# burritojustice/reporter

Measured on AMD Instinct MI355X. Metric: GPS points matched/sec (whole node) at 1/2/4/8 MI355X; % segment-ID agreement vs meili, higher is better.
Workload: dtype f32

## Files before the change

### include/otmatch.h

```cpp
#ifndef OTMATCH_H
#define OTMATCH_H

#include <stddef.h>
#include <stdint.h>

#ifdef __cplusplus
extern "C" {
#endif

#define OTM_OK 0
#define OTM_EINVAL (-1)
#define OTM_EIO (-2)
#define OTM_EDEVICE (-3)
#define OTM_ECONFIG (-4)
#define OTM_EAGAIN (-5)
#define OTM_ENOMEM (-6)

typedef struct otm_engine otm_engine;


int otm_engine_create(const char* cfg_path, const int* devices, int ndev,
                      otm_engine** out);
typedef struct otm_meili_params {
  float sigma_z, beta, max_route_distance_factor, breakage_distance, interpolation_distance;
// ... 231 lines not shown
int otm_attributes_size(otm_engine* eng, int64_t* n_traces, int64_t* n_bytes);
int otm_fetch_attributes(otm_engine* eng, char* dst, int64_t cap, int64_t* body_off, int64_t* n_bytes);
int otm_attributes_device(otm_engine* eng, const char** dev, const int64_t** body_off, int64_t* n_traces,
                          int64_t* n_bytes);
int otm_debug_attr_fixed(double x, int decimals, char* out);

int otm_hist_bind(otm_engine* eng, void* dev_counts, int nbins, float bin_kph);
int otm_hist_bind_ex(otm_engine* eng, void* dev_counts, int nbins, float bin_kph,
                     void* dev_speed_sum);


int otm_flush_body_host(const uint32_t* counts, const uint64_t* speed_sum,
                        const uint64_t* segment_ids, int64_t n_segments,
                        int64_t rows, int nbins, float bin_kph, int rank, int world,
                        char** body, size_t* body_len, int64_t* n_records);
int otm_flush_body_device(otm_engine* eng, const void* dev_counts,
                          const void* dev_speed_sum, int64_t rows, int nbins,
                          float bin_kph, int rank, int world, void* stream,
                          char** body, size_t* body_len, int64_t* n_records);

int otm_window_begin(otm_engine* eng, int nbins, float bin_kph);
int otm_window_flush(otm_engine* eng, char** body, size_t* body_len, int64_t* n_records);
int otm_window_end(otm_engine* eng);

typedef struct otm_pairs_cfg {
  int32_t bucket_s;
  int32_t privacy;
  int64_t origin;
  int64_t max_keys;
} otm_pairs_cfg;
typedef struct otm_pairs_stats {
  int64_t reports;
  int64_t keys;
  int64_t records;
  int64_t suppressed_keys;
  int64_t suppressed_reports;
  int64_t out_of_range;
  int64_t dropped;
} otm_pairs_stats;
int otm_pairs_cfg_check(const otm_pairs_cfg* cfg);
int otm_pairs_begin(otm_engine* eng, const otm_pairs_cfg* cfg);
int otm_pairs_add_reports(otm_engine* eng, int64_t n, const otm_report_rec* recs);
int otm_pairs_flush(otm_engine* eng, char** body, size_t* body_len, otm_pairs_stats* stats);
int otm_pairs_end(otm_engine* eng);
int otm_pairs_info(const otm_engine* eng, otm_pairs_cfg* cfg, int64_t* slots);

int otm_graph_info(const otm_engine* eng, int64_t* n_nodes, int64_t* n_edges,
                   int64_t* n_segments);

int otm_index_info(const otm_engine* eng, float* rmax, int64_t* entries,
                   int32_t* incomplete_rows, float* build_ms);

int otm_index_levels(const otm_engine* eng, float* radii, int64_t* entries, int cap);

int otm_index_tables(const otm_engine* eng, int64_t* slots, int64_t* bytes, int32_t* load_pct);

int otm_grid_info(const otm_engine* eng, double* cell_deg, int32_t* rows, int32_t* cols,
                  int64_t* entries, int32_t* mult);

typedef struct otm_work_counters {
  int64_t points, columns, cells_visited, cell_entries_scanned, candidates;
  int64_t searches, nodes_settled, edges_relaxed, transitions;
  int64_t route_searches, route_nodes_settled, route_edges_relaxed, route_edges;
  int64_t segments_out, reports_out;
} otm_work_counters;
int otm_set_counting(otm_engine* eng, int on);
int otm_get_counters(otm_engine* eng, otm_work_counters* out);

int otm_set_timing(otm_engine* eng, int on);
int otm_get_stage_ms(otm_engine* eng, float* ms, int n);

#define OTM_NUM_KERNELS 18
int otm_get_kernel_ms(otm_engine* eng, float* ms, int n);
const char* otm_kernel_name(int k);

typedef struct otm_spill_stats {
  int32_t cand_wave;
  int32_t trans_online, trans_wave, trans_global;
  int32_t route_online, route_wave, route_global;
  int32_t cand_big, trans_huge, route_huge, attempts;
  int32_t resumed;
} otm_spill_stats;
int otm_get_spill_stats(otm_engine* eng, otm_spill_stats* out);

int otm_debug_fetch(otm_engine* eng, int what, void* dst, size_t bytes,
                    size_t* needed);
int otm_kmax(void);
int otm_debug_py_repr(double d, char* out);
int otm_debug_py_round3(double x, double* out);
int otm_debug_arena_stress(int threads, int rounds);
int otm_debug_last_split(const otm_engine* eng);
const char* otm_runtime_info(void);

typedef struct otm_batcher otm_batcher;
typedef struct otm_batcher_cfg {
  int32_t report_dist;
  int32_t report_count;
  int64_t report_time_s;
  int64_t session_gap_ms;
  int32_t max_batch;
  int32_t json_path;
  int64_t max_pending;
  int32_t threads;
  int32_t reserved;
} otm_batcher_cfg;
void otm_batcher_defaults(otm_batcher_cfg* cfg);
typedef int (*otm_report_fn)(void* ctx, int n, const char* const* reqs, const size_t* lens, char** resps,
                             size_t* resp_lens, int* codes);
int otm_batcher_create(otm_engine* eng, const otm_batcher_cfg* cfg, otm_report_fn fn, void* ctx,
                       otm_batcher** out);
void otm_batcher_destroy(otm_batcher* b);
int otm_batcher_process(otm_batcher* b, int n, const char* const* keys, const size_t* key_lens, const float* lat,
                        const float* lon, const int32_t* accuracy, const int64_t* time, const int64_t* ts_ms);
int otm_batcher_flush(otm_batcher* b);
int otm_batcher_close(otm_batcher* b);
typedef struct otm_forward {
  char* key;
  size_t key_len;
  char* body;
  size_t body_len;
  int64_t seq;
} otm_forward;
int otm_batcher_take(otm_batcher* b, otm_forward* out, int max);
typedef struct otm_batcher_stats {
  int64_t records, clean_ops, close_ops, requests, request_points, match_batches, forwarded;
  int64_t null_batch_in_clean;
  int64_t keys, stored_batches, stored_points;
  int64_t us_enqueue, us_run, us_prepare, us_match, us_apply;
  int64_t raw_messages, raw_dropped, us_format;
  int64_t null_responses;
} otm_batcher_stats;
int otm_batcher_get_stats(const otm_batcher* b, otm_batcher_stats* out);
int otm_batcher_batch(const otm_batcher* b, const char* key, size_t key_len, int max, float* lat, float* lon,
                      int32_t* accuracy, int64_t* time, float* max_separation);

typedef struct otm_formatter otm_formatter;
int otm_formatter_create(const char* spec, otm_formatter** out, char* err, size_t err_len);
void otm_formatter_destroy(otm_formatter* f);
typedef struct otm_formatted {
  int32_t n, n_ok;
  uint8_t* ok;
  int64_t* key_off;
  char* keys;
  float* lat;
  float* lon;
  int32_t* accuracy;
  int64_t* time;
} otm_formatted;
int otm_format(const otm_formatter* f, int32_t n, const char* msgs, const int64_t* off, int nthreads,
               otm_formatted* out);
void otm_formatted_free(otm_formatted* r);
int otm_batcher_process_raw(otm_batcher* b, const otm_formatter* f, int32_t n, const char* msgs,
                            const int64_t* off, const int64_t* ts_ms, int nthreads);

void otm_quantize_decimal6(const float* in, float* out, int64_t n);

typedef struct otm_synth_graph_params {
  double center_lat, center_lon;
  double width_m, height_m;
  double block_m;
  double jitter_m;
  int arterial_every;
  int highway_every;
  double unassoc_frac;
  int complex_every;
  double seg_max_m;
// ... 38 lines not shown
```

### reporter_amd/_lib.py

```python
import ctypes as C
import os

import numpy as np

_HERE = os.path.dirname(os.path.abspath(__file__))
LIB_PATH = os.environ.get("OTM_LIB") or os.path.join(_HERE, "lib", "libotmatch.so")

OTM_OK = 0



class Batch(C.Structure):
    _fields_ = [("n_traces", C.c_int32), ("n_points", C.c_int64), ("trace_off", C.c_void_p), ("lat", C.c_void_p),
                ("lon", C.c_void_p), ("time", C.c_void_p), ("accuracy", C.c_void_p)]


class BatchCompact(C.Structure):
    _fields_ = [("n_traces", C.c_int32), ("n_points", C.c_int64), ("trace_off", C.c_void_p),
                ("time_base", C.c_void_p), ("lat", C.c_void_p), ("lon", C.c_void_p), ("time_delta", C.c_void_p),
                ("accuracy", C.c_void_p)]


class Results(C.Structure):
    _fields_ = [("n_traces", C.c_int32), ("n_segments", C.c_int32), ("n_reports", C.c_int32),
# ... 158 lines not shown
    psz = C.POINTER(C.c_size_t)
    sig = {
        "otm_engine_create": (C.c_int, [C.c_char_p, C.POINTER(C.c_int), C.c_int, pp]),
        "otm_engine_members": (C.c_int, [vp]),
        "otm_config_meili": (C.c_int, [C.c_char_p, vp]),
        "otm_config_queue": (C.c_int, [C.c_char_p, C.POINTER(C.c_float)]),
        "otm_queue_info": (C.c_int, [vp, C.POINTER(C.c_float)]),
        "otm_set_points": (C.c_int, [vp, C.c_int]),
        "otm_points_info": (C.c_int, [vp, C.POINTER(C.c_int)]),
        "otm_fetch_points": (C.c_int, [vp, vp, i64, C.POINTER(i64)]),
        "otm_points_device": (C.c_int, [vp, pp, C.POINTER(i64)]),
        "otm_set_traversals": (C.c_int, [vp, C.c_int]),
        "otm_traversals_info": (C.c_int, [vp, C.POINTER(C.c_int)]),
        "otm_traversals_size": (C.c_int, [vp, C.POINTER(i64), C.POINTER(i64)]),
        "otm_fetch_traversals": (C.c_int, [vp, vp, i64, vp, C.POINTER(i64)]),
        "otm_traversals_device": (C.c_int, [vp, pp, pp, C.POINTER(i64)]),
        "otm_set_scores": (C.c_int, [vp, C.c_int]),
        "otm_scores_info": (C.c_int, [vp, C.POINTER(C.c_int)]),
        "otm_fetch_scores": (C.c_int, [vp, vp, i64, C.POINTER(i64)]),
        "otm_scores_device": (C.c_int, [vp, pp, C.POINTER(i64)]),
        "otm_set_shape": (C.c_int, [vp, C.c_int]),
        "otm_shape_info": (C.c_int, [vp, C.POINTER(C.c_int)]),
        "otm_shape_size": (C.c_int, [vp, C.POINTER(ShapeSizes)]),
        "otm_fetch_shape": (C.c_int, [vp, C.POINTER(ShapeOut)]),
        "otm_shape_device": (C.c_int, [vp, C.POINTER(ShapeOut), C.POINTER(ShapeSizes)]),
        "otm_set_attributes": (C.c_int, [vp, C.c_uint32]),
        "otm_attributes_info": (C.c_int, [vp, C.POINTER(C.c_uint32)]),
        "otm_attributes_size": (C.c_int, [vp, C.POINTER(i64), C.POINTER(i64)]),
        "otm_fetch_attributes": (C.c_int, [vp, vp, i64, vp, C.POINTER(i64)]),
        "otm_attributes_device": (C.c_int, [vp, pp, pp, C.POINTER(i64), C.POINTER(i64)]),
        "otm_debug_attr_fixed": (C.c_int, [C.c_double, C.c_int, C.c_char_p]),
        "otm_request_points": (C.c_int, [C.c_char_p, sz, C.c_int, vp, vp, vp, vp, C.c_int, C.c_char_p, sz]),
        "otm_engine_member": (vp, [vp, C.c_int]),
        "otm_engine_destroy": (None, [vp]),
        "otm_last_error": (C.c_char_p, [vp]),
        "otm_free": (None, [vp]),
        "otm_report": (C.c_int, [vp, C.c_char_p, sz, pp, psz]),
        "otm_report_batch": (C.c_int, [vp, C.c_int, C.POINTER(C.c_char_p), psz, pp, psz, C.POINTER(C.c_int)]),
        "otm_match_json": (C.c_int, [vp, C.c_char_p, sz, pp, psz]),
        "otm_report_segments": (C.c_int, [vp, C.c_char_p, sz, C.c_char_p, sz, pp, psz]),
        "otm_submit": (C.c_int, [vp, C.c_char_p, sz, C.c_uint64]),
        "otm_poll": (C.c_int, [vp, C.POINTER(Result), C.c_int, C.c_int]),
        "otm_submit_batch": (C.c_int, [vp, C.c_int, vp, vp, vp]),
        "otm_encode_request": (C.c_int, [C.c_char_p, C.c_int, vp, vp, vp, vp, pp, psz]),
        "otm_match_soa": (C.c_int, [vp, C.POINTER(Batch), C.POINTER(Results)]),
        "otm_match_compact": (C.c_int, [vp, C.POINTER(BatchCompact), C.POINTER(Results)]),
        "otm_request_arena_alloc": (vp, [sz]),
        "otm_request_arena_release": (C.c_int, [vp]),
        "otm_host_alloc": (vp, [sz]),
        "otm_host_free": (None, [vp]),
        "otm_match_device": (C.c_int, [vp, C.POINTER(Batch), vp]),
        "otm_fetch_results": (C.c_int, [vp, C.POINTER(Results)]),
        "otm_hist_bind": (C.c_int, [vp, vp, C.c_int, C.c_float]),
        "otm_hist_bind_ex": (C.c_int, [vp, vp, C.c_int, C.c_float, vp]),
        "otm_flush_body_host": (C.c_int, [vp, vp, vp, i64, i64, C.c_int, C.c_float, C.c_int, C.c_int, pp, psz,
                                          C.POINTER(i64)]),
        "otm_flush_body_device": (C.c_int, [vp, vp, vp, i64, C.c_int, C.c_float, C.c_int, C.c_int, vp, pp, psz,
                                            C.POINTER(i64)]),
        "otm_window_begin": (C.c_int, [vp, C.c_int, C.c_float]),
        "otm_window_flush": (C.c_int, [vp, pp, psz, C.POINTER(i64)]),
        "otm_window_end": (C.c_int, [vp]),
        "otm_pairs_cfg_check": (C.c_int, [vp]),
        "otm_pairs_begin": (C.c_int, [vp, vp]),
        "otm_pairs_add_reports": (C.c_int, [vp, i64, vp]),
        "otm_pairs_flush": (C.c_int, [vp, pp, psz, vp]),
        "otm_pairs_end": (C.c_int, [vp]),
        "otm_pairs_info": (C.c_int, [vp, vp, C.POINTER(i64)]),
        "otm_report_segments_device": (C.c_int, [vp, C.c_int, C.POINTER(C.c_char_p), psz, C.POINTER(C.c_char_p), psz,
                                                 pp, psz, C.POINTER(C.c_int)]),
        "otm_graph_info": (C.c_int, [vp, C.POINTER(i64), C.POINTER(i64), C.POINTER(i64)]),
        "otm_index_info": (C.c_int, [vp, C.POINTER(C.c_float), C.POINTER(i64), C.POINTER(i32),
                                     C.POINTER(C.c_float)]),
        "otm_index_levels": (C.c_int, [vp, C.POINTER(C.c_float), C.POINTER(i64), C.c_int]),
        "otm_index_tables": (C.c_int, [vp, C.POINTER(C.c_int64), C.POINTER(C.c_int64), C.POINTER(C.c_int32)]),
        "otm_grid_info": (C.c_int, [vp, C.POINTER(C.c_double), C.POINTER(i32), C.POINTER(i32), C.POINTER(i64),
                                    C.POINTER(i32)]),
        "otm_set_counting": (C.c_int, [vp, C.c_int]),
        "otm_get_counters": (C.c_int, [vp, C.POINTER(WorkCounters)]),
        "otm_set_timing": (C.c_int, [vp, C.c_int]),
        "otm_get_stage_ms": (C.c_int, [vp, C.POINTER(C.c_float), C.c_int]),
        "otm_get_kernel_ms": (C.c_int, [vp, C.POINTER(C.c_float), C.c_int]),
        "otm_kernel_name": (C.c_char_p, [C.c_int]),
        "otm_get_spill_stats": (C.c_int, [vp, C.POINTER(SpillStats)]),
        "otm_debug_fetch": (C.c_int, [vp, C.c_int, vp, sz, psz]),
        "otm_kmax": (C.c_int, []),
        "otm_debug_py_repr": (C.c_int, [C.c_double, C.c_char_p]),
        "otm_debug_py_round3": (C.c_int, [C.c_double, C.POINTER(C.c_double)]),
        "otm_debug_arena_stress": (C.c_int, [C.c_int, C.c_int]),
        "otm_debug_last_split": (C.c_int, [vp]),
        "otm_batcher_defaults": (None, [C.POINTER(BatcherCfg)]),
        "otm_batcher_create": (C.c_int, [vp, C.POINTER(BatcherCfg), REPORT_FN, vp, pp]),
        "otm_batcher_destroy": (None, [vp]),
        "otm_batcher_process": (C.c_int, [vp, C.c_int, C.POINTER(C.c_char_p), psz, vp, vp, vp, vp, vp]),
        "otm_batcher_flush": (C.c_int, [vp]),
        "otm_batcher_close": (C.c_int, [vp]),
        "otm_batcher_take": (C.c_int, [vp, C.POINTER(Forward), C.c_int]),
        "otm_batcher_get_stats": (C.c_int, [vp, C.POINTER(BatcherStats)]),
        "otm_batcher_batch": (C.c_int, [vp, C.c_char_p, sz, C.c_int, vp, vp, vp, vp, C.POINTER(C.c_float)]),
        "otm_quantize_decimal6": (None, [vp, vp, C.c_int64]),
        "otm_engine_clone": (C.c_int, [vp, C.POINTER(vp)]),
        "otm_formatter_create": (C.c_int, [C.c_char_p, C.POINTER(vp), C.c_char_p, sz]),
        "otm_formatter_destroy": (None, [vp]),
        "otm_format": (C.c_int, [vp, C.c_int32, vp, vp, C.c_int, C.POINTER(Formatted)]),
        "otm_formatted_free": (None, [C.POINTER(Formatted)]),
        "otm_batcher_process_raw": (C.c_int, [vp, vp, C.c_int32, vp, vp, vp, C.c_int]),
        "otm_synth_graph_defaults": (None, [C.POINTER(SynthGraphParams)]),
        "otm_synth_graph": (C.c_int, [C.POINTER(SynthGraphParams), C.c_char_p]),
        "otm_synth_traces": (C.c_int, [C.c_char_p, C.POINTER(SynthTraceParams), vp, vp, vp, vp, vp, vp, vp]),
        "otm_murmur2": (i32, [C.c_char_p, sz]),
        "otm_synth_true_paths": (i64, [C.c_char_p, C.POINTER(SynthTraceParams), vp, vp, i64]),
        "otm_synth_true_paths_timed": (i64, [C.c_char_p, C.POINTER(SynthTraceParams), vp, vp, vp, i64]),
        "otm_tile_id": (i64, [C.c_int, C.c_double, C.c_double]),
        "otm_tile_file": (C.c_int, [i64, C.c_int, C.c_char_p, C.c_char_p, sz]),
        "otm_tile_files_bbox": (C.c_int, [C.c_double, C.c_double, C.c_double, C.c_double, C.c_char_p, pp, psz]),
        "otm_runtime_info": (C.c_char_p, []),
        "otm_stream_create": (vp, [vp, C.c_int]),
        "otm_stream_destroy": (None, [vp]),
    }
    for name, (res, args) in sig.items():
        if os.environ.get("OTM_LIB") and not hasattr(L, name):
            continue
        fn = getattr(L, name)
        fn.restype = res
        fn.argtypes = args
    return sig


EXPORTED = None


def _bind_torch_hip_runtime():
    try:
        import torch
    except Exception:
        pass


def lib():
    global _lib, EXPORTED
    if _lib is None:
        if not os.path.exists(LIB_PATH):
            raise RuntimeError("libotmatch.so not built (%s); run __graft_entry__.build() or "
                               "`make -C reporter_amd/csrc`" % LIB_PATH)
        _bind_torch_hip_runtime()
        L = C.CDLL(LIB_PATH)
        EXPORTED = sorted(_declare(L).keys())
        _lib = L
    return _lib


def malloc_bytes(b):
    libc = C.CDLL(None)
    libc.malloc.restype = C.c_void_p
    libc.malloc.argtypes = [C.c_size_t]
    p = libc.malloc(len(b) + 1)
    C.memmove(p, b + b"\0", len(b) + 1)
    return p


def last_error():
    msg = lib().otm_last_error(None)
    return msg.decode("utf-8", "replace") if msg else ""


def take(ptr, n):
    s = C.string_at(ptr, n)
# ... 15 lines not shown
```

### reporter_amd/csrc/abi.cpp

```cpp
#include <dlfcn.h>

#include <algorithm>
#include <atomic>
#include <chrono>
#include <cmath>
#include <condition_variable>
#include <cstdio>
#include <cstdlib>
#include <cstring>
#include <deque>
#include <fstream>
#include <exception>
#include <functional>
#include <memory>
#include <mutex>
#include <new>
#include <sstream>
#include <thread>

#include "attrfmt.h"
#include "engine.h"
#include "flush.h"
#include "javastr.h"
#include "json.h"
// ... 2315 lines not shown

int otm_index_tables(const otm_engine* E, int64_t* slots, int64_t* bytes, int32_t* load_pct) {
  if (!E) return fail(OTM_EINVAL, "engine is NULL");
  if (!E->members.empty()) E = E->members[0];
  const int64_t n = E->index_slots + E->index_near_slots;
  if (slots) *slots = n;
  if (bytes) *bytes = n * otm::IDX_SLOT_BYTES + E->index_src_bytes;
  if (load_pct) *load_pct = E->idx.rmax > 0.0f ? E->idx.load_pct : 0;
  return OTM_OK;
}

int otm_index_levels(const otm_engine* E, float* radii, int64_t* entries, int cap) {
  if (!E) return fail(OTM_EINVAL, "engine is NULL");
  if (!E->members.empty()) E = E->members[0];
  int n = 0;
  for (int l = 0; l < otm::NEAR_LEVELS; ++l) {
    if (!(E->idxn[l].rmax > 0.0f)) continue;
    if (n < cap) {
      if (radii) radii[n] = E->idxn[l].rmax;
      if (entries) entries[n] = E->index_near_level_entries[l];
    }
    ++n;
  }
  return n;
}

int otm_grid_info(const otm_engine* E, double* cell_deg, int32_t* rows, int32_t* cols, int64_t* entries,
                  int32_t* mult) {
  if (!E) return fail(OTM_EINVAL, "engine is NULL");
  if (!E->members.empty()) E = E->members[0];
  if (cell_deg) *cell_deg = E->g.cell;
  if (rows) *rows = E->grid_rows;
  if (cols) *cols = E->grid_cols;
  if (entries) *entries = E->grid_entries;
  if (mult) *mult = E->grid_mult;
  return OTM_OK;
}

int otm_set_counting(otm_engine* E, int on) {
  if (!E) return fail(OTM_EINVAL, "engine is NULL");
  for (otm_engine* m : E->members) m->counting = on != 0;
  E->counting = on != 0;
  return OTM_OK;
}

int otm_get_counters(otm_engine* E, otm_work_counters* out) {
  if (!E || !out) return fail(OTM_EINVAL, "bad arguments");
  if (!E->members.empty()) E = E->members[0];
  std::lock_guard<std::mutex> lk(E->mu);
  return otm::engine_counters(E, out) ? fail(OTM_EDEVICE, "counter copy failed") : OTM_OK;
}

int otm_set_timing(otm_engine* E, int on) {
  if (!E) return fail(OTM_EINVAL, "engine is NULL");
  for (otm_engine* m : E->members) m->timing = on != 0;
  E->timing = on != 0;
  return OTM_OK;
}

int otm_get_stage_ms(otm_engine* E, float* ms, int n) {
  if (!E || !ms) return fail(OTM_EINVAL, "bad arguments");
  if (!E->members.empty()) E = E->members[0];
  for (int k = 0; k < n && k < 8; ++k) ms[k] = E->stage_ms[k];
  return OTM_OK;
}

int otm_get_kernel_ms(otm_engine* E, float* ms, int n) {
  if (!E || !ms) return fail(OTM_EINVAL, "bad arguments");
  if (!E->members.empty()) E = E->members[0];
  for (int k = 0; k < n && k < otm::KN_COUNT; ++k) ms[k] = E->kernel_ms[k];
  return OTM_OK;
}

static_assert(OTM_NUM_KERNELS == otm::KN_COUNT, "kernel table");
const char* otm_kernel_name(int k) { return k >= 0 && k < otm::KN_COUNT ? otm::kKernelNames[k] : nullptr; }

int otm_get_spill_stats(otm_engine* E, otm_spill_stats* out) {
  if (!E || !out) return fail(OTM_EINVAL, "bad arguments");
  if (!E->members.empty()) E = E->members[0];
  std::lock_guard<std::mutex> lk(E->mu);
  return otm::engine_spill_stats(E, out) ? fail(OTM_EDEVICE, "spill stats copy failed") : OTM_OK;
}

int otm_debug_fetch(otm_engine* E, int what, void* dst, size_t bytes, size_t* needed) {
  if (!E) return fail(OTM_EINVAL, "engine is NULL");
  if (!E->members.empty()) E = E->members[0];
  std::lock_guard<std::mutex> lk(E->mu);
  std::string err;
  int rc = otm::engine_debug_fetch(E, what, dst, bytes, needed, &err);
  return rc ? fail(rc, err) : OTM_OK;
}

int otm_engine_create(const char* cfg_path, const int* devices, int ndev, otm_engine** out) {
  return guarded([&] { return otm_engine_create_impl(cfg_path, devices, ndev, out); });
}

int otm_report_batch(otm_engine* E, int n, const char* const* reqs, const size_t* lens, char** resps,
                     size_t* resp_lens, int* codes) {
  return guarded([&] { return otm_report_batch_impl(E, n, reqs, lens, resps, resp_lens, codes); });
}

int otm_report_segments_device(otm_engine* E, int n, const char* const* reqs, const size_t* lens,
                               const char* const* match_jsons, const size_t* match_lens, char** resps,
                               size_t* resp_lens, int* codes) {
  return guarded(
      [&] { return otm_report_segments_device_impl(E, n, reqs, lens, match_jsons, match_lens, resps, resp_lens, codes); });
}

int otm_submit(otm_engine* E, const char* req, size_t len, uint64_t tag) {
  return guarded([&] { return otm_submit_impl(E, req, len, tag); });
}

int otm_submit_batch(otm_engine* E, int n, const char* const* reqs, const size_t* lens, const uint64_t* tags) {
  return guarded([&] { return otm_submit_batch_impl(E, n, reqs, lens, tags); });
}

int otm_match_soa(otm_engine* E, const otm_batch* in, otm_results* out) {
  return guarded([&] { return otm_match_soa_impl(E, in, out); });
}

int otm_match_compact(otm_engine* E, const otm_batch_compact* in, otm_results* out) {
  return guarded([&] { return otm_match_compact_impl(E, in, out); });
}

int otm_match_device(otm_engine* E, const otm_batch* in, void* stream) {
  return guarded([&] { return otm_match_device_impl(E, in, stream); });
}

int otm_fetch_results(otm_engine* E, otm_results* out) {
  return guarded([&] { return otm_fetch_results_impl(E, out); });
}

int otm_report(otm_engine* E, const char* req, size_t len, char** resp, size_t* resp_len) {
  return guarded_500(resp, resp_len, [&] { return otm_report_impl(E, req, len, resp, resp_len); });
}

int otm_match_json(otm_engine* E, const char* req, size_t len, char** resp, size_t* resp_len) {
  return guarded_500(resp, resp_len, [&] { return otm_match_json_impl(E, req, len, resp, resp_len); });
}

}
```

### reporter_amd/csrc/engine.cpp

```cpp
#include "engine.h"

#include "flush.h"

#include <algorithm>
#include <chrono>
#include <cmath>
#include <cstdlib>

#include <cstring>

namespace otm {

#define HIPCHK(x)                                                              \
  do {                                                                         \
    hipError_t e_ = (x);                                                       \
    if (e_ != hipSuccess) {                                                    \
      *err = std::string(#x) + ": " + hipGetErrorString(e_);                   \
      return OTM_EDEVICE;                                                      \
    }                                                                          \
  } while (0)

#define TRY(x)                    \
  do {                            \
    if (int rc_ = (x)) return rc_; \
// ... 498 lines not shown
  TRY(bind_grow(w.huge_fr, E->huge_fr, n * 2, err));
  TRY(bind_grow(w.huge_ins, E->huge_ins, n ? (size_t)HUGE_SLOTS * huge_limit(E->huge_log2) : 0, err));
  TRY(bind_grow(w.huge_prev, E->huge_prev, n ? (size_t)HUGE_SLOTS : 0, err));
  if (n && E->huge_ready_log2 != E->huge_log2) {
    E->huge_ready_log2 = E->huge_log2;
    HIPCHK(hipMemsetAsync(w.huge_key, 0xFF, n * sizeof *w.huge_key, E->stream));
    HIPCHK(hipMemsetAsync(w.huge_lab, 0xFF, n * sizeof *w.huge_lab, E->stream));
    HIPCHK(hipMemsetAsync(w.huge_inq, 0, n * sizeof *w.huge_inq, E->stream));
    HIPCHK(hipMemsetAsync(w.huge_prev, 0xFF, (size_t)HUGE_SLOTS * sizeof *w.huge_prev, E->stream));
  }
  return OTM_OK;
}

static int ensure_big(otm_engine* E, DevWork& w, std::string* err) {
  const size_t n = (size_t)BIG_SLOTS * BIG_TABLE_CAP;
  bool fresh;
  TRY(bind_buf(w.big_key, E->big_key, n, err));
  TRY(bind_buf(w.big_lab, E->big_lab, n, err));
  TRY(bind_buf(w.big_inq, E->big_inq, n, err));
  TRY(bind_buf(w.big_fr, E->big_fr, n * 2, err));
  TRY(bind_buf(w.big_ins, E->big_ins, (size_t)BIG_SLOTS * SEARCH_LIMIT, err));
  TRY(bind_buf(w.big_prev, E->big_prev, (size_t)BIG_SLOTS, err, &fresh));
  if (fresh) {
    HIPCHK(hipMemsetAsync(w.big_key, 0xFF, n * sizeof *w.big_key, E->stream));
    HIPCHK(hipMemsetAsync(w.big_lab, 0xFF, n * sizeof *w.big_lab, E->stream));
    HIPCHK(hipMemsetAsync(w.big_inq, 0, n * sizeof *w.big_inq, E->stream));
    HIPCHK(hipMemsetAsync(w.big_prev, 0, (size_t)BIG_SLOTS * sizeof *w.big_prev, E->stream));
  }
  return OTM_OK;
}

static int bind_point_work(otm_engine* E, int64_t NP, int32_t NT, DevWork& w, std::string* err) {
  const size_t Pn = (size_t)NP + 1;
  TRY(bind_buf(w.pt_trace, E->pt_trace, Pn, err));
  TRY(bind_buf(w.is_col, E->is_col, Pn, err));
  TRY(bind_buf(w.prevc, E->prevc, Pn, err));
  TRY(bind_buf(w.nextc, E->nextc, Pn, err));
  TRY(bind_buf(w.gc, E->gc, Pn, err));
  TRY(bind_buf(w.ncand, E->ncand, Pn, err));
  TRY(bind_buf(w.cand_eo, E->cand_eo, Pn * KIN, err));
  TRY(bind_buf(w.cand_em, E->cand_em, Pn * KIN, err));
  TRY(bind_buf(w.cand_xeo, E->cand_xeo, Pn * KX, err));
  TRY(bind_buf(w.cand_xem, E->cand_xem, Pn * KX, err));
  TRY(bind_buf(w.probe, E->probe, Pn, err));
  TRY(bind_buf(w.col_prev, E->col_prev, Pn, err));
  TRY(bind_buf(w.kq_prev, E->kq_prev, Pn, err));
  TRY(bind_buf(w.vmeta, E->vmeta, Pn, err));
  TRY(bind_buf(w.colrec, E->colrec, Pn, err));
  TRY(bind_buf(w.colrec_pos, E->colrec_pos, Pn, err));
  TRY(bind_buf(w.trans_off, E->trans_off, Pn, err));
  TRY(bind_buf(w.bp, E->bp, Pn * KMAX, err));
  TRY(bind_buf(w.state, E->state, Pn, err));
  TRY(bind_buf(w.chosen, E->chosen, Pn, err));
  TRY(bind_buf(w.chain_start, E->chain_start, Pn, err));
  TRY(bind_buf(w.route_dist, E->route_dist, Pn, err));
  TRY(bind_buf(w.ipos, E->ipos, Pn, err));
  TRY(bind_buf(w.path_off, E->path_off, Pn, err));
  TRY(bind_buf(w.path_len, E->path_len, Pn, err));
  TRY(bind_buf(w.trace_err, E->trace_err, (size_t)NT + 1, err));
  TRY(bind_buf(w.spill_list1, E->spill_list1, Pn, err));
  TRY(bind_buf(w.spill_list2, E->spill_list2, Pn, err));
  TRY(bind_buf(w.spill_list3, E->spill_list3, Pn, err));
  TRY(bind_buf(w.counters_i32, E->counters_i32, CTR_WORDS, err));
  TRY(E->snap.ensure(1, err));
  w.snap = &E->snap.p->stage[0][0];
  TRY(bind_buf(w.abort, E->abort_flag, 4, err));
  if (!E->caps_read) {
    E->caps_read = true;
    if (const char* v = std::getenv("OTM_TRANS_CAP")) E->trans_cap = std::max<int64_t>(1, std::atoll(v)), E->caps_pinned = true;
    if (const char* v = std::getenv("OTM_POOL_CAP")) E->pool_cap = (int32_t)std::max(1, std::atoi(v)), E->caps_pinned = true;
  }
  if (!E->caps_pinned) {
    E->trans_cap = std::max<int64_t>(E->trans_cap, (int64_t)Pn * 48 + 4096);
    E->pool_cap = std::max<int32_t>(E->pool_cap, (int32_t)std::min<size_t>(Pn * 8, (size_t)1 << 30));
  }
  TRY(E->scan_tmp.ensure(scan_tmp_bytes(NP > NT ? NP : NT) + 256, err));
  TRY(bind_buf(w.path_pool, E->path_pool, (size_t)E->pool_cap, err));
  w.pool_cap = E->pool_cap;
  w.idx = E->idx;
  for (int l = 0; l < NEAR_LEVELS; ++l) w.idxn[l] = E->idxn[l];
  return OTM_OK;
}

static int bind_order(otm_engine* E, int64_t NP, bool ordered, DevOrder& ord, std::string* err) {
  const size_t Pn = (size_t)NP + 1;
  TRY(bind_buf(ord.tile, E->ord_tile, Pn, err));
  TRY(bind_buf(ord.tile_cnt, E->ord_cnt, ORDER_TILES, err));
  TRY(bind_buf(ord.cursor, E->ord_cursor, ORDER_TILES, err));
  TRY(bind_buf(ord.grp, E->ord_grp, ORDER_GROUPS + 1, err));
  TRY(bind_buf(ord.item, E->ord_item, Pn, err));
  if (!ordered) ord.tile_cnt = nullptr;
  return OTM_OK;
}

static int bind_trans(otm_engine* E, DevWork& w, hipStream_t s, std::string* err) {
  bool fresh;
  TRY(bind_buf(w.trans, E->trans, (size_t)E->trans_cap + 1, err, &fresh));
  if (fresh) HIPCHK(hipMemsetAsync(E->trans.p, 0, E->trans.bytes(), s));
  w.trans_cap = E->trans_cap;
  return OTM_OK;
}

static size_t out_region_cap(const otm_engine* E, int64_t NP) { return 2 * (size_t)NP + (size_t)E->pool_cap + 1; }

static int bind_out(otm_engine* E, int32_t NT, int64_t NP, DevOut& o, std::string* err) {
  const size_t Tn = (size_t)NT + 1, cap = out_region_cap(E, NP);
  TRY(bind_buf(o.traces, E->o_traces, Tn, err));
  TRY(bind_buf(o.seg_cnt, E->o_seg_cnt, Tn, err));
  TRY(bind_buf(o.way_cnt, E->o_way_cnt, Tn, err));
  TRY(bind_buf(o.seg_base, E->seg_ub, Tn, err));
  TRY(bind_buf(o.segments, E->o_segments, cap, err));
  TRY(bind_buf(o.seg_gidx, E->o_seg_gidx, cap, err));
  TRY(bind_buf(o.reports, E->o_reports, cap, err));
  TRY(bind_buf(o.way_ids, E->o_way_ids, cap, err));
  TRY(bind_buf(o.rep_cnt, E->o_rep_cnt, Tn, err));
  return OTM_OK;
}

static int bind_trav(otm_engine* E, int32_t NT, int64_t NP, DevTrav& tv, std::string* err) {
  TRY(bind_buf(tv.rec, E->tv_rec, out_region_cap(E, NP), err));
  TRY(bind_buf(tv.cnt, E->tv_cnt, (size_t)NT + 1, err));
  return OTM_OK;
}

static int bind_scores(otm_engine* E, int32_t NT, int64_t NP, DevScores& sc, std::string* err) {
  const size_t Pn = (size_t)NP + 1;
  TRY(bind_buf(sc.rec, E->scores.dev, Pn, err));
  TRY(bind_buf(sc.alpha, E->sc_alpha, Pn * KIN, err));
  TRY(bind_buf(sc.alpha_x, E->sc_alpha_x, Pn * KX, err));
  TRY(bind_buf(sc.rej, E->sc_rej, (size_t)NT + 2, err));
  sc.rej_n = sc.rej + NT + 1;
  return OTM_OK;
}

static int engine_match_once(otm_engine* E, const DevBatch& b, hipStream_t s, std::string* err,
                             int from = RESUME_ALL) {
  const int64_t NP = b.n_points;
  const int32_t NT = b.n_traces;
  end_records(E, REC_BATCH_BEGINS);
  DevWork w{};
  TRY(bind_point_work(E, NP, NT, w, err));

  DevParams dp = E->dp;
  if (NP < E->small_points) {
    dp.order_mask = 0;
    dp.cand_wave_all = 1;
  }
  {
    const char* ce = std::getenv("OTM_CAND_CHUNK");
    const int ch = ce ? std::atoi(ce) : 64;
    dp.cand_chunk = ch < 1 ? 1 : (ch > 64 ? 64 : ch);
  }
  w.ctr = E->counting ? E->ctr.p : nullptr;
  if (E->counting && from == RESUME_ALL) HIPCHK(hipMemsetAsync(E->ctr.p, 0, sizeof(DevCounters), s));
  Marks mk;
  mk.ev = E->timing ? E->kev : nullptr;
  TRY(bind_order(E, NP, dp.order_mask != 0, w.ord, err));
  if (from == RESUME_ALL) {
    launch_columns(E->g, b, dp, w, s, mk);
    if (dp.order_mask) {
      launch_order(b, w, s, mk);
    } else if (E->timing) {
      mk.begin(KN_ORDER, s);
      mk.end(KN_ORDER, s);
    }
  }
  TRY(ensure_cand(E, w, err));
  if (from <= RESUME_CAND_BIG) launch_candidates(E->g, b, dp, w, s, mk, from);
  if (from <= RESUME_CAND_BIG) {
    launch_links(b, dp, w, s, mk);
    mk.begin(KN_SCAN_TRANS, s);
    scan_i64(w.trans_off, NP, E->scan_tmp.p, E->scan_tmp.cap(), s);
    mk.end(KN_SCAN_TRANS, s);
  }
  TRY(bind_trans(E, w, s, err));
  TRY(ensure_big(E, w, err));
  TRY(ensure_huge(E, w, err));
  if (from <= RESUME_TRANS_HUGE) launch_transitions(E->g, b, dp, w, s, mk, E->trans_lanes, from);
  if (from <= RESUME_TRANS_HUGE) launch_viterbi(b, w, s, mk);
  launch_route(E->g, b, dp, w, s, mk, from);

  if (out_region_cap(E, NP) >= (size_t)INT32_MAX) {
    *err = "batch too large for one launch (segment regions exceed 2^31)";
    return OTM_EINVAL;
  }
  DevOut o{};
  TRY(bind_out(E, NT, NP, o, err));
  {
    otm_engine* H = E->parent ? const_cast<otm_engine*>(E->parent) : E;
    std::lock_guard<std::mutex> lk(H->hist_mu);
    o.hist = H->hist;
    o.speed_sum = H->speed_sum;
    o.nbins = H->nbins;
    o.bin_kph = H->bin_kph;
    o.pairs = H->pairs_tab;
  }
  HIPCHK(hipMemsetAsync(o.seg_base, 0, ((size_t)NT + 1) * sizeof *o.seg_base, s));
  launch_seg_bound(E->g, b, dp, w, o.seg_base, s, mk);
  mk.begin(KN_SEG_SCAN, s);
  scan_i64(o.seg_base, NT, E->scan_tmp.p, E->scan_tmp.cap(), s);
  mk.end(KN_SEG_SCAN, s);
  launch_segments(E->g, b, w, o, s, mk);
  if (E->queue_kph > 0.0f) launch_queue(b, w, o, E->queue_kph, s);
  const uint32_t attr = records_wanted(E, E->attrs) ? E->at_mask : 0;
  end_records(E, REC_BATCH_OUTPUTS);
  if (records_wanted(E, E->points) || (attr & OTM_ATTR_POINTS)) {
    TRY(E->points.dev.ensure((size_t)NP + 1, err));
    launch_points(E->g, b, dp, w, E->points.dev.p, s);
    if (records_wanted(E, E->points)) E->points.n = NP;
  }
  if (records_wanted(E, E->scores) || (attr & OTM_ATTR_SCORES)) {
    DevScores sc{};
    TRY(bind_scores(E, NT, NP, sc, err));
    launch_scores(b, w, sc, s);
    if (records_wanted(E, E->scores)) E->scores.n = NP;
  }
  const bool for_route = records_wanted(E, E->route), for_shape = records_wanted(E, E->shape);
  if (for_route || for_shape || (attr & (OTM_ATTR_EDGES | OTM_ATTR_SHAPE))) {
    DevTrav tv{};
    TRY(bind_trav(E, NT, NP, tv, err));
    HIPCHK(hipMemsetAsync(tv.cnt + NT, 0, sizeof *tv.cnt, s));
    launch_traversals(E->g, b, w, o, tv, s);
    if (for_route) E->tv_T = NT;
    if (for_shape) E->sh_T = NT;
  }
  if (attr) {
    E->at_T = NT;
    E->at_P = NP;
    E->at_batch_mask = attr;
  }
  launch_report(b, E->drc, w, o, s, mk);
  HIPCHK(hipGetLastError());
  E->last_T = NT;
  E->last_P = NP;
  E->last_S = -1;
  E->last_W = -1;
  return OTM_OK;
}

int engine_match(otm_engine* E, const DevBatch& b, hipStream_t s, std::string* err) {
  if (!s) s = E->stream;
  const int64_t NP = b.n_points;
  struct OomGuard {
    otm_engine* E;
    bool huge = false, cand = false;
    ~OomGuard() {
      if (huge) E->huge_final = 0;
      if (cand) E->cand_final = 0;
    }
  } oom{E};
  struct FailGuard {
    otm_engine* E;
    bool ok = false;
    ~FailGuard() {
      if (!ok) end_records(E, REC_BATCH_FAILED);
    }
  } failed{E};
  int from = RESUME_ALL;
  DevWork grown{};
  E->last_resumes = 0;
  for (int attempt = 0;; ++attempt) {
    TRY(engine_match_once(E, b, s, err, from));
    TRY(E->h_status.ensure(1, err));
    BatchStatus* dst = &E->snap.p->status;
    launch_status(E->abort_flag.p, E->trans_off.p + NP, E->counters_i32.p, dst, s);
    HIPCHK(hipMemcpyAsync(E->h_status.p, dst, sizeof(BatchStatus), hipMemcpyDeviceToHost, s));
    HIPCHK(wait_batch(E, s, NP));
    const BatchStatus st = *E->h_status.p;
    const int32_t ab = st.abort;
    const int64_t ttotal = st.ttotal;
    E->last_trans = ttotal;
    E->last_attempts = attempt + 1;
    if (!ab) break;
    if (attempt == 16) {
      *err = "batch capacities could not be sized";
      return OTM_EDEVICE;
    }
    if (ttotal > E->trans_cap) E->trans_cap = ttotal + ttotal / 4 + 4096;
    if (st.grow & GROW_HUGE) {
      const int32_t next = E->huge_log2 ? E->huge_log2 + 2 : 19;
      const int32_t prev = E->huge_log2;
      if (next > max_log2("OTM_HUGE_MAX_LOG2", HUGE_MAX_LOG2)) {
        E->huge_final = 1;
      } else {
        E->huge_log2 = next;
        if (ensure_huge(E, grown, err) != OTM_OK) {
          E->huge_log2 = prev;
          E->huge_final = 1;
          oom.huge = true;
          E->huge_ready_log2 = 0;
          err->clear();
        }
      }
    }
    if (st.grow & GROW_CAND) {
      const int32_t next = E->cand_log2 ? E->cand_log2 + 2 : 13;
      const int32_t prev = E->cand_log2;
      if (next > max_log2("OTM_CAND_MAX_LOG2", CAND_MAX_LOG2)) {
        E->cand_final = 1;
      } else {
        E->cand_log2 = next;
        if (ensure_cand(E, grown, err) != OTM_OK) {
          E->cand_log2 = prev;
          E->cand_final = 1;
          oom.cand = true;
          err->clear();
        }
      }
    }
    if (st.pool_over)
      E->pool_cap = (int32_t)std::min<size_t>((size_t)st.pool_used * 2 + 1024, (size_t)INT32_MAX / 2);
    const char* nr = std::getenv("OTM_NO_RESUME");
    const bool whole = ttotal > E->trans_cap || st.pool_over || !(st.grow & (GROW_HUGE | GROW_CAND)) ||
                       (nr && *nr && *nr != '0');
    from = whole ? RESUME_ALL
                 : (st.grow & GROW_CAND) ? RESUME_CAND_BIG : (st.route_huge ? RESUME_ROUTE_HUGE : RESUME_TRANS_HUGE);
    if (from != RESUME_ALL) {
      const SnapId snap = from == RESUME_CAND_BIG ? SNAP_AFTER_CAND
                                                  : (from == RESUME_TRANS_HUGE ? SNAP_AFTER_TRANS : SNAP_AFTER_ROUTE);
      int32_t* ctr = E->counters_i32.p;
      HIPCHK(hipMemcpyAsync(ctr, E->snap.p->stage[snap], CTR_STAGE_WORDS * sizeof(int32_t),
                            hipMemcpyDeviceToDevice, s));
      HIPCHK(hipMemsetAsync(ctr + CTR_GROW_HUGE, 0, 4, s));
      HIPCHK(hipMemsetAsync(ctr + CTR_GROW_CAND, 0, 4, s));
      HIPCHK(hipMemsetAsync(E->abort_flag.p, 0, 4, s));
      E->last_resumes += 1;
    }
  }
  if (E->timing) {
    HIPCHK(hipEventSynchronize(E->kev[2 * KN_REPORT + 1]));
    for (int k = 0; k < KN_COUNT; ++k)
      HIPCHK(hipEventElapsedTime(&E->kernel_ms[k], E->kev[2 * k], E->kev[2 * k + 1]));
    const int first[8] = {KN_COLUMNS, KN_ORDER, KN_LINKS, KN_TRANS_INDEX, KN_VITERBI, KN_ROUTE_INDEX, KN_SEG_BOUND,
                          KN_SEG_WRITE};
    const int last[8] = {KN_COLUMNS, KN_CAND_WAVE, KN_SCAN_TRANS, KN_TRANS_GLOBAL, KN_VITERBI, KN_ROUTE_GLOBAL,
                         KN_SEG_SCAN, KN_REPORT};
    for (int k = 0; k < 8; ++k) {
      E->stage_ms[k] = 0.0f;
      for (int q = first[k]; q <= last[k]; ++q) E->stage_ms[k] += E->kernel_ms[q];
    }
  }
  failed.ok = true;
  return OTM_OK;
}

static hipError_t big_copy(void* dst, const void* src, size_t n, hipMemcpyKind k, hipStream_t s) {
  return hipMemcpyAsync(dst, src, n, k, s);
}

static int validate_offsets(int32_t NT, const int64_t* trace_off, int64_t n_points, std::string* err) {
  const int64_t NP = trace_off[NT];
  if (trace_off[0] != 0 || NP < 0 || (n_points && n_points != NP)) {
    *err = "batch trace_off inconsistent with n_points";
    return OTM_EINVAL;
  }
  for (int32_t t = 0; t < NT; ++t)
    if (trace_off[t + 1] < trace_off[t]) {
      *err = "batch trace_off not monotonic";
      return OTM_EINVAL;
    }
  return OTM_OK;
}

int engine_match_host(otm_engine* E, const otm_batch* in, std::string* err) {
  const int32_t NT = in->n_traces;
  if (NT < 0 || !in->trace_off) {
    *err = "invalid batch";
    return OTM_EINVAL;
  }
  TRY(validate_offsets(NT, in->trace_off, in->n_points, err));
  const int64_t NP = in->trace_off[NT];
  DevBatch b;
  b.n_traces = NT;
  b.n_points = NP;
  TRY(bind_buf(b.trace_off, E->in_off, (size_t)NT + 1, err));
  TRY(bind_buf(b.lat, E->in_lat, (size_t)NP, err));
  TRY(bind_buf(b.lon, E->in_lon, (size_t)NP, err));
  TRY(bind_buf(b.time, E->in_time, (size_t)NP, err));
  TRY(bind_buf(b.acc, E->in_acc, (size_t)NP, err));
  hipStream_t s = E->stream;
  const size_t b_off = ((size_t)NT + 1) * 8, b_pt = (size_t)NP * 4, b_tm = (size_t)NP * 8;
  if (NP <= (int64_t)1 << 18) {
    const size_t total = b_off + b_tm + 3 * b_pt;
    TRY(E->h_in.ensure(total, err));
    TRY(E->in_blob.ensure(total, err));
    char* h = E->h_in.p;
    std::memcpy(h, in->trace_off, b_off);
    if (NP) {
      std::memcpy(h + b_off, in->time, b_tm);
      std::memcpy(h + b_off + b_tm, in->lat, b_pt);
      std::memcpy(h + b_off + b_tm + b_pt, in->lon, b_pt);
      std::memcpy(h + b_off + b_tm + 2 * b_pt, in->accuracy, b_pt);
    }
    HIPCHK(hipMemcpyAsync(E->in_blob.p, h, total, hipMemcpyHostToDevice, s));
    const char* d = E->in_blob.p;
    b.trace_off = (const int64_t*)d;
    b.time = (const double*)(d + b_off);
    b.lat = (const float*)(d + b_off + b_tm);
    b.lon = (const float*)(d + b_off + b_tm + b_pt);
    b.acc = (const float*)(d + b_off + b_tm + 2 * b_pt);
    return engine_match(E, b, s, err);
  }
  const hipMemcpyKind h2d = hipMemcpyHostToDevice;
  HIPCHK(hipMemcpyAsync(E->in_off.p, in->trace_off, b_off, hipMemcpyHostToDevice, s));
  HIPCHK(big_copy(E->in_lat.p, in->lat, b_pt, h2d, s));
  HIPCHK(big_copy(E->in_lon.p, in->lon, b_pt, h2d, s));
  HIPCHK(big_copy(E->in_time.p, in->time, b_tm, h2d, s));
// ... 1310 lines not shown
```

### reporter_amd/csrc/engine.h

```cpp
#pragma once
#include <atomic>
#include <hip/hip_runtime.h>

#include <condition_variable>
#include <deque>
#include <memory>
#include <mutex>
#include <string>
#include <thread>
#include <vector>

#include "buffers.h"
#include "flush.h"
#include "kernels.h"
#include "otm_internal.h"
#include "otmatch.h"

struct ReqSlab {
  char* base = nullptr;
  size_t cap = 0;
  bool pinned = false;
};

namespace otm {
// ... 51 lines not shown
template <class Rec>
struct BatchRecords {
  bool on = false;
  int64_t n = -1;
  DevBuf<Rec> dev;
  PinBuf<Rec> pin;
  std::vector<Rec> joined;
  int64_t joined_n = -1;
};
}

struct otm_engine {
  ~otm_engine() {
    if (members.empty() && device >= 0) (void)hipSetDevice(device);
  }
  const otm_engine* parent = nullptr;
  std::vector<otm_engine*> members;
  const otm_engine* group = nullptr;
  struct MemberPool* member_pool = nullptr;
  std::vector<otm_trace_result> g_traces;
  std::vector<otm_segment> g_segs;
  std::vector<otm_report_rec> g_reps;
  std::vector<int64_t> g_ways;
  int device = -1;
  std::atomic<int> n_clones{0};
  hipStream_t stream = nullptr;
  hipEvent_t sync_ev = nullptr;
  bool spin_waits = false;
  otm::HostGraph host;
  otm::DevGraph g{};
  std::vector<void*> graph_allocs;
  float index_rmax = -1.0f;
  int64_t small_points = 0;
  int trans_lanes = 8;
  int grid_mult = 0;
  float queue_kph = 0.0f;
  int32_t grid_rows = 0, grid_cols = 0;
  int64_t grid_entries = 0;
  otm::DevIndex idx{};
  otm::DevIndex idxn[otm::NEAR_LEVELS]{};
  std::vector<float> index_near_m;
  bool index_near_set = false;
  int64_t index_near_level_entries[otm::NEAR_LEVELS]{};
  int64_t index_entries = 0;
  int64_t index_slots = 0;
  int64_t index_near_slots = 0;
  int64_t index_src_bytes = 0;
  int32_t index_incomplete_rows = 0;
  float index_build_ms = 0.0f;
  otm::MatchConfig mc;
  otm::ReportConfig rc;
  otm::DevParams dp{};
  otm::DevReportCfg drc{};
  std::mutex mu;

  otm::DevBuf<int64_t> in_off;
  otm::DevBuf<float> in_lat, in_lon, in_acc;
  otm::DevBuf<double> in_time;
  otm::DevBuf<char> in_blob;
  otm::PinBuf<char> h_in;
  otm::DevBuf<int32_t> pt_trace, prevc, nextc, ncand, col_prev, kq_prev, colrec_pos, state, path_off, path_len, path_pool,
      trace_err, spill_list1, spill_list2, spill_list3, counters_i32, abort_flag;
  otm::DevBuf<uint8_t> is_col, vmeta, bp, chain_start;
  otm::DevBuf<float> gc, cand_em, cand_xem, trans, route_dist, ipos;
  otm::DevBuf<int2> cand_eo, cand_xeo, chosen;
  otm::DevBuf<float4> probe;
  otm::DevBuf<int4> colrec;
  otm::DevBuf<int64_t> trans_off;
  otm::DevBuf<otm::SnapBuf> snap;
  otm::DevBuf<char> scan_tmp;
  otm::PinBuf<otm::BatchStatus> h_status;
  otm::DevBuf<otm::DevCounters> ctr, ctr_save;
  int64_t trans_cap = 0;
  bool caps_read = false, caps_pinned = false;
  otm::DevBuf<uint32_t> big_key, big_inq, big_fr, big_ins, huge_key, huge_inq, huge_fr, huge_ins, cbig_key;
  otm::DevBuf<unsigned long long> big_lab, huge_lab, cbig_val, cbig_skey;
  otm::DevBuf<int32_t> big_prev, huge_prev;
  int32_t huge_log2 = 0;
  int32_t huge_ready_log2 = 0;
  int32_t cand_log2 = 0;
  int32_t huge_final = 0, cand_final = 0;
  int32_t last_attempts = 0;
  int32_t last_resumes = 0;
  otm::DevBuf<uint16_t> ord_tile;
  otm::DevBuf<int32_t> ord_cnt, ord_cursor, ord_grp, ord_item;
  otm::DevBuf<otm_trace_result> o_traces;
  otm::DevBuf<int32_t> o_seg_cnt, o_way_cnt, o_rep_cnt, o_seg_gidx;
  otm::DevBuf<int64_t> seg_ub, o_way_ids;
  otm::DevBuf<otm_segment> o_segments;
  otm::DevBuf<otm_report_rec> o_reports;
  otm::DevBuf<char> rs_blob;
  otm::DevBuf<int32_t> f_seg_off, f_way_off, f_rep_off;
  otm::DevBuf<otm_segment> f_segs;
  otm::DevBuf<int64_t> f_ways;
  otm::DevBuf<otm_report_rec> f_reps;
  otm::DevBuf<otm_trace_result> f_traces;
  otm::PinBuf<otm_trace_result> h_traces;
  otm::PinBuf<otm_segment> h_segs;
  otm::PinBuf<otm_report_rec> h_reps_dense;
  otm::PinBuf<int64_t> h_ways;
  otm::PinBuf<int32_t> h_tot;
  bool counting = false;
  std::mutex hist_mu;
  uint32_t* hist = nullptr;
  unsigned long long* speed_sum = nullptr;
  int nbins = 0;
  float bin_kph = 5.0f;
  int32_t last_T = 0;
  int64_t last_P = 0;
  int32_t last_S = 0, last_W = 0;
  int64_t last_trans = 0;
  int32_t pool_cap = 0;
  otm::PinBuf<char> h_req;
  otm::DevBuf<unsigned char> d_req;
  otm::DevBuf<int64_t> req_cnt;
  otm::DevBuf<uint8_t> req_ok;
  otm::PinBuf<uint8_t> h_req_ok;
  otm::DevBuf<float> req_lat, req_lon, req_acc;
  otm::DevBuf<double> req_time;
  int32_t req_read = 0;
  hipStream_t req_copy = nullptr;
  double t_read_done = 0.0;
  hipStream_t req_shared = nullptr;
  std::vector<hipEvent_t> req_ev;
  size_t req_piece = 0;
  otm::DevBuf<char> resp_hdr, resp_seg, resp_rep, resp_blob;
  otm::DevBuf<int32_t> resp_hlen, resp_slen, resp_rlen;
  otm::DevBuf<int64_t> resp_blen;
  otm::DevBuf<uint8_t> resp_host;
  otm::PinBuf<char> h_resp, h_resp_meta;
  otm::DevBuf<char> flush_slots, flush_blob;
  otm::DevBuf<int64_t> flush_len;
  otm::DevBuf<otm::FlushMeta> flush_meta;
  otm::PinBuf<char> h_flush, h_flush_meta;
  std::mutex win_mu;
  bool win_open = false;
  int win_nbins = 0;
  float win_bin_kph = 0.0f;
  void* win_counts = nullptr;
  void* win_sums = nullptr;
  otm::DevBuf<uint32_t> win_peer_counts;
  otm::DevBuf<unsigned long long> win_peer_sums;
  bool pairs_open = false;
  otm_pairs_cfg pairs_cfg{};
  otm::PairTab pairs_tab{};
  otm::DevBuf<unsigned long long> pairs_ckey, pairs_skey, pm_key, pm_ctr, pp_key;
  otm::DevBuf<uint32_t> pairs_cidx, pairs_sidx;
  otm::DevBuf<char> pairs_sort_tmp, pairs_meta;
  otm::DevBuf<otm::PairIn> pairs_in;
  otm::DevBuf<otm::PairVal> pm_val, pp_val;
  std::vector<std::pair<uint64_t, int32_t>> pairs_rows;
  bool timing = false;
  hipEvent_t kev[2 * otm::KN_COUNT] = {};
  float kernel_ms[otm::KN_COUNT] = {};
  float stage_ms[8] = {};
  struct Pending {
    uint64_t tag;
    const char* p;
    size_t len;
    std::shared_ptr<ReqSlab> slab;
    size_t run_left;
    uint64_t sub;
  };
  uint64_t n_subs = 0;
  std::mutex qmu;
  std::condition_variable qcv;
// ... 94 lines not shown
```

### reporter_amd/csrc/kernels.h

```cpp
#pragma once
#include <hip/hip_runtime.h>

#include <cstddef>
#include <cstdint>

#include "otmatch.h"
#include "pairs.h"

namespace otm {

constexpr int KMAX = 32;
constexpr int KIN = 8;
static_assert(KIN == 4 || KIN == 8, "inline blocks of 4 or 8 slots (whole 16-B emission pieces)");
constexpr int KX = KMAX - KIN;
constexpr int MAX_HITS = 256;
constexpr int SEARCH_LIMIT = 98304;
constexpr int LDS_TABLE_CAP = 256;
constexpr int LDS_TABLE_LIMIT = 192;
constexpr int BIG_TABLE_LOG2 = 17;
constexpr int BIG_TABLE_CAP = 1 << BIG_TABLE_LOG2;
#ifndef OTM_BIG_SLOTS
#define OTM_BIG_SLOTS 512
#endif
constexpr int BIG_SLOTS = OTM_BIG_SLOTS;
// ... 57 lines not shown
  IdxRow node;
  int32_t from;
  int32_t len;
  int32_t pad[(OTM_SRC_REC_BYTES - 40) / 4];
};
static_assert(sizeof(SrcRec) == OTM_SRC_REC_BYTES && (OTM_SRC_REC_BYTES == 48 || OTM_SRC_REC_BYTES == 64),
              "source records of 48 or 64 bytes");
struct DevIndex {
  float rmax;
  uint32_t cmax;
  const IdxRow* row;
  const SrcRec* src;
  const uint4* slot;
  int load_pct;
};
constexpr int IDX_SLOT_BYTES = 16;
constexpr float INDEX_RMAX_CAP = 200000.0f;
constexpr uint32_t NODE_KEY = 0x80000000u;
constexpr uint32_t NONE_PRED = 0xFFFFFFFFu;
constexpr int NEAR_LEVELS = 3;
#ifndef OTM_INDEX_NEAR_FRACS
#define OTM_INDEX_NEAR_FRACS {0.45f}
#endif
#ifndef OTM_INDEX_NEAR_MIN_GB
#define OTM_INDEX_NEAR_MIN_GB 16.0
#endif
constexpr int INDEX_BUILD_LOG2 = 11;
constexpr int INDEX_BUILD_CAP = 1 << INDEX_BUILD_LOG2;
constexpr int INDEX_BUILD_LIMIT = 1536;
__host__ __device__ inline uint32_t index_cost_bound(float B) { return (uint32_t)floor((double)B * 64.0); }

constexpr int ORDER_CAND = 1, ORDER_TRANS = 2, ORDER_ROUTE = 4;
constexpr int TURN_TABLE = 181;
constexpr uint32_t TURN_UNITS_MAX = 0xFFFFFFu;
constexpr uint32_t NO_TURNS = 0xFFFFFFFFu;
struct DevParams {
  float sigma_z, beta, factor, breakage, interp, search_radius, max_search_radius, gps_accuracy;
  const uint32_t* turn_units;
  int max_candidates;
  int order_mask;
  int cand_wave_all;
  int cand_chunk;
};

struct DevReportCfg {
  int n_report, n_transition;
  int64_t report_levels[16];
  int64_t transition_levels[16];
  double threshold_sec;
};

struct DevBatch {
  int32_t n_traces;
  int64_t n_points;
  const int64_t* trace_off;
  const float *lat, *lon;
  const double* time;
  const float* acc;
};

struct DevCounters {
  unsigned long long points, columns, cells_visited, cell_entries_scanned, candidates;
  unsigned long long searches, nodes_settled, edges_relaxed, transitions;
  unsigned long long route_searches, route_nodes_settled, route_edges_relaxed, route_edges;
  unsigned long long segments_out, reports_out;
};

enum CtrSlot : int {
  CTR_UNUSED = 0,
  CTR_POOL_USED = 1,
  CTR_POOL_OVER = 2,
  CTR_SEARCH_GLOBAL = 3,
  CTR_INDEX_MISS = 4,
  CTR_CAND_WAVE = 5,
  CTR_TRANS_WIDE = 6,
  CTR_SEG_LARGE = 8,
  CTR_VIT_16 = 20,
  CTR_TRANS_HUGE = 21,
  CTR_ROUTE_HUGE = 22,
  CTR_GROW_HUGE = 23,
  CTR_CAND_BIG = 24,
  CTR_GROW_CAND = 25,
  CTR_VIT_WAVE = 26,
};
constexpr int CTR_STAGE_WORDS = 16;
constexpr int CTR_ZEROED_WORDS = 32;
constexpr int CTR_WORDS = 64;
enum SnapId : int { SNAP_AFTER_CAND = 0, SNAP_AFTER_TRANS = 1, SNAP_AFTER_ROUTE = 2, SNAP_COUNT = 3 };
constexpr int ctr_list(CtrSlot c) {
  switch (c) {
    case CTR_INDEX_MISS: case CTR_CAND_WAVE: case CTR_SEG_LARGE: case CTR_VIT_16: return 1;
    case CTR_SEARCH_GLOBAL: case CTR_TRANS_WIDE: case CTR_VIT_WAVE: return 2;
    case CTR_TRANS_HUGE: case CTR_ROUTE_HUGE: case CTR_CAND_BIG: return 3;
    default: return 0;
  }
}
constexpr bool ctr_per_stage(CtrSlot c) { return c >= 0 && c < CTR_STAGE_WORDS; }
constexpr bool ctr_per_batch(CtrSlot c) { return c >= CTR_STAGE_WORDS && c < CTR_ZEROED_WORDS; }
static_assert(ctr_per_stage(CTR_UNUSED) && ctr_per_stage(CTR_POOL_USED) && ctr_per_stage(CTR_POOL_OVER) &&
                  ctr_per_stage(CTR_SEARCH_GLOBAL) && ctr_per_stage(CTR_INDEX_MISS) && ctr_per_stage(CTR_CAND_WAVE) &&
                  ctr_per_stage(CTR_TRANS_WIDE) && ctr_per_stage(CTR_SEG_LARGE),
              "per-stage slots lie in the snapshot range");
static_assert(ctr_per_batch(CTR_VIT_16) && ctr_per_batch(CTR_TRANS_HUGE) && ctr_per_batch(CTR_ROUTE_HUGE) &&
                  ctr_per_batch(CTR_GROW_HUGE) && ctr_per_batch(CTR_CAND_BIG) && ctr_per_batch(CTR_GROW_CAND) &&
                  ctr_per_batch(CTR_VIT_WAVE),
              "per-batch slots lie past the snapshot range, within what K1 zeroes");

struct DevWork {
  int32_t* pt_trace;
  uint8_t* is_col;
  int32_t* prevc;
  int32_t* nextc;
  float* gc;
  int32_t* ncand;
  float4* probe;
  int2* cand_eo;
  float* cand_em;
  int2* cand_xeo;
  float* cand_xem;
  int32_t* col_prev;
  int32_t* kq_prev;
  uint8_t* vmeta;
  int64_t* trans_off;
  float* trans;
  uint8_t* bp;
  int32_t* state;
  int2* chosen;
  uint8_t* chain_start;
  float* route_dist;
  float* ipos;
  int32_t* path_off;
  int32_t* path_len;
  int32_t* path_pool;
  int32_t pool_cap;
  int32_t* trace_err;
  int32_t* spill_list1;
  int32_t* spill_list2;
  int32_t* snap;
  int32_t* counters_i32;
  int32_t* abort;
  int64_t trans_cap;
  int4* colrec;
  int32_t* colrec_pos;
  DevIndex idx;
  DevIndex idxn[NEAR_LEVELS];
  DevOrder ord;
  uint32_t* big_key;
  unsigned long long* big_lab;
  uint32_t* big_inq;
  uint32_t* big_fr;
  uint32_t* big_ins;
  int32_t* big_prev;
  uint32_t* huge_key;
  unsigned long long* huge_lab;
  uint32_t* huge_inq;
  uint32_t* huge_fr;
  uint32_t* huge_ins;
  int32_t* huge_prev;
  int32_t huge_log2;
  int32_t huge_final;
  uint32_t* cbig_key;
  unsigned long long* cbig_val;
  unsigned long long* cbig_skey;
  int32_t cand_log2;
  int32_t cand_final;
  int32_t* spill_list3;
  DevCounters* ctr;
};
struct SpillRef {
  int32_t* list;
  int32_t* count;
};
template <CtrSlot C>
__host__ __device__ __forceinline__ int32_t* spill_list(const DevWork& w) {
  constexpr int L = ctr_list(C);
  static_assert(L != 0, "this slot counts no list");
  return L == 1 ? w.spill_list1 : (L == 2 ? w.spill_list2 : w.spill_list3);
}
template <CtrSlot C>
__host__ __device__ __forceinline__ SpillRef spill_of(const DevWork& w) {
  return SpillRef{spill_list<C>(w), w.counters_i32 + C};
}

struct DevOut {
  otm_trace_result* traces;
  int32_t* seg_cnt;
  int32_t* way_cnt;
  int32_t* rep_cnt;
  int64_t* seg_base;
  otm_segment* segments;
  int32_t* seg_gidx;
  int64_t* way_ids;
  otm_report_rec* reports;
  uint32_t* hist;
  unsigned long long* speed_sum;
  int nbins;
  float bin_kph;
  PairTab pairs;
};

struct DevTrav {
  otm_traversal* rec;
  int64_t* cnt;
};

struct DevShape {
  const int64_t* trav_off;
  int64_t* vtx_off;
  int64_t* poly_off;
  otm_shape_vertex* vtx;
  otm_shape_span* span;
  char* poly;
};

enum KernelId {
  KN_COLUMNS,
  KN_ORDER,
  KN_CAND_LANE,
  KN_CAND_WAVE,
  KN_LINKS,
  KN_SCAN_TRANS,
  KN_TRANS_INDEX,
  KN_TRANS_WIDE,
  KN_TRANS_WAVE,
  KN_TRANS_GLOBAL,
  KN_VITERBI,
  KN_ROUTE_INDEX,
  KN_ROUTE_WAVE,
  KN_ROUTE_GLOBAL,
  KN_SEG_BOUND,
  KN_SEG_SCAN,
  KN_SEG_WRITE,
  KN_REPORT,
  KN_COUNT
};
extern const char* const kKernelNames[KN_COUNT];
struct Marks {
  hipEvent_t* ev = nullptr;
  void begin(int k, hipStream_t s) const {
    if (ev) (void)hipEventRecord(ev[2 * k], s);
  }
  void end(int k, hipStream_t s) const {
    if (ev) (void)hipEventRecord(ev[2 * k + 1], s);
  }
};

void launch_columns(const DevGraph& g, const DevBatch& b, const DevParams& p, DevWork& w, hipStream_t s,
                    const Marks& mk);
enum Resume { RESUME_ALL = 0, RESUME_CAND_BIG = 1, RESUME_TRANS_HUGE = 2, RESUME_ROUTE_HUGE = 3 };
void launch_candidates(const DevGraph& g, const DevBatch& b, const DevParams& p, DevWork& w, hipStream_t s,
                       const Marks& mk, int from = RESUME_ALL);
void launch_links(const DevBatch& b, const DevParams& p, DevWork& w, hipStream_t s, const Marks& mk);
void launch_transitions(const DevGraph& g, const DevBatch& b, const DevParams& p, DevWork& w, hipStream_t s,
                        const Marks& mk, int sub, int from = RESUME_ALL);
void launch_viterbi(const DevBatch& b, DevWork& w, hipStream_t s, const Marks& mk);
void launch_route(const DevGraph& g, const DevBatch& b, const DevParams& p, DevWork& w, hipStream_t s,
                  const Marks& mk, int from = RESUME_ALL);
void launch_segments(const DevGraph& g, const DevBatch& b, DevWork& w, DevOut& o, hipStream_t s, const Marks& mk);
void launch_queue(const DevBatch& b, DevWork& w, DevOut& o, float kph, hipStream_t s);
void launch_points(const DevGraph& g, const DevBatch& b, const DevParams& p, DevWork& w, otm_matched_point* out,
                   hipStream_t s);
void launch_traversals(const DevGraph& g, const DevBatch& b, DevWork& w, DevOut& o, const DevTrav& tv, hipStream_t s);
void launch_trav_compact(int32_t n_traces, const int64_t* seg_base, const int64_t* off, const otm_traversal* reg,
                         otm_traversal* dst, hipStream_t s);
struct DevScores {
  otm_point_score* rec;
  float* alpha;
  float* alpha_x;
  int32_t* rej;
  int32_t* rej_n;
};
void launch_scores(const DevBatch& b, DevWork& w, const DevScores& sc, hipStream_t s);
void launch_shape(const DevGraph& g, int32_t n_traces, const int64_t* seg_base, const DevTrav& tv, const DevShape& sh,
                  bool write, hipStream_t s);
void launch_report(const DevBatch& b, const DevReportCfg& rc, DevWork& w, DevOut& o, hipStream_t s, const Marks& mk);
void launch_order(const DevBatch& b, DevWork& w, hipStream_t s, const Marks& mk);
void launch_seg_bound(const DevGraph& g, const DevBatch& b, const DevParams& p, DevWork& w, int64_t* tb, hipStream_t s,
                      const Marks& mk);
void launch_compact(int32_t n_traces, const DevOut& o, const int32_t* seg_off, const int32_t* way_off,
                    const int32_t* rep_off, otm_segment* segs_out, int64_t* ways_out, otm_report_rec* reps_out,
                    otm_trace_result* traces_out,
                    hipStream_t s);
void launch_index_build(const DevGraph& g, const uint32_t* turn_units, uint32_t cmax, int32_t* row_cnt,
                        const IdxRow* rows, uint4* slot, bool write, hipStream_t s);
int index_load_fast();
int index_load_dense();
void launch_row_sizes(const int32_t* row_cnt, int64_t* row_sizes, int32_t n, int pct, hipStream_t s);
constexpr int32_t GROW_HUGE = 1, GROW_CAND = 2;
struct BatchStatus {
  int32_t abort, grow;
  int64_t ttotal;
  int32_t pool_used, pool_over;
  int32_t route_huge;
};
struct SnapBuf {
  int32_t stage[SNAP_COUNT][CTR_STAGE_WORDS];
  BatchStatus status;
};
static_assert(offsetof(SnapBuf, status) == 192 && sizeof(SnapBuf) == 192 + 32, "snapshot buffer layout");
void launch_expand_compact(const int64_t* trace_off, const int64_t* tbase, const int32_t* dt, const int16_t* acc16,
                           double* time, float* acc, int32_t n_traces, hipStream_t s);
void launch_status(const int32_t* abort, const int64_t* ttotal, const int32_t* counters, BatchStatus* out,
                   hipStream_t s);
void launch_row_pack(const int32_t* row_cnt, const int64_t* row_off, IdxRow* rows, int32_t n, hipStream_t s);
void launch_src_pack(const DevGraph& g, const IdxRow* rows, SrcRec* src, hipStream_t s);
size_t req_sparse_slots(int32_t n, size_t bytes);
void launch_req_read(const unsigned char* blob, const int64_t* off, int32_t r0, int32_t r1, int32_t n, int64_t* cnt,
                     uint8_t* ok, const DevBatch& sparse, hipStream_t s);
void launch_req_compact(const int64_t* off, int32_t n, const int64_t* pre, const uint8_t* ok, const DevBatch& sparse,
                        const DevBatch& out, int64_t* trace_off, hipStream_t s);
constexpr int RESP_HDR_SLOT = 512;
constexpr int RESP_SEG_SLOT = 320;
constexpr int RESP_REP_SLOT = 192;
struct RespIn {
  int32_t nt, ns, nr;
  const otm_trace_result* traces;
  const otm_segment* segs;
  const int64_t* ways;
  const otm_report_rec* reps;
};
struct RespWork {
  char *hdr, *seg, *rep;
  int32_t *hlen, *slen, *rlen;
  int64_t* blen;
  uint8_t* host;
};
size_t resp_seg_scratch(int32_t ns, int32_t nw);
void launch_resp_items(const RespIn& in, const RespWork& w, hipStream_t s);
void launch_resp_len(const RespIn& in, const RespWork& w, hipStream_t s);
void launch_resp_copy(const RespIn& in, const RespWork& w, const int64_t* boff, char* blob, hipStream_t s);
struct DevAttr {
  uint32_t mask;
  int32_t n_traces;
  int64_t n_points, n_trav;
  const int32_t* pt_trace;
  const otm_matched_point* pts;
  const otm_point_score* scores;
  const otm_traversal* trav;
  const int64_t* trav_off;
  const otm_shape_span* span;
  const char* poly;
  const int64_t* poly_off;
  int64_t* pt_off;
  int64_t* item_off;
  int64_t* body_off;
  char* blob;
};
void launch_attr_pt_off(const DevAttr& a, hipStream_t s);
void launch_attr_items(const DevAttr& a, bool write, hipStream_t s);
void launch_attr_frame(const DevAttr& a, bool write, hipStream_t s);
void scan_i64(int64_t* d, int64_t n, void* tmp, size_t tmp_bytes, hipStream_t s);
constexpr int FETCH_SCAN_MAX = 1 << 16;
void launch_fetch_scan(int32_t n, const int32_t* c0, const int32_t* c1, const int32_t* c2, int32_t* o0, int32_t* o1,
                       int32_t* o2, hipStream_t s);
void scan_i32(int32_t* d, int64_t n, void* tmp, size_t tmp_bytes, hipStream_t s);
size_t scan_tmp_bytes(int64_t n);

}
```

### reporter_amd/csrc/kernels.hip

```cpp
#include <hip/hip_runtime.h>

#include <algorithm>
#include <cstdlib>
#include <type_traits>

#include <hipcub/hipcub.hpp>

#include "kernels.h"
#include "otmatch.h"

namespace otm {

namespace {

#define MPD_F 111319.4954833f
constexpr uint32_t EMPTY = 0xFFFFFFFFu;
constexpr unsigned long long LAB_NONE = ~0ull;
constexpr int TB = 64;
__device__ __forceinline__ void wave_sync() {
  __builtin_amdgcn_wave_barrier();
  asm volatile("" ::: "memory");
}

__device__ __forceinline__ float cos_deg(float deg) {
// ... 126 lines not shown
                                        float& sqd, float& off_out) {
  bool at_end;
  project(g, e, k, lat, lon, ls, sqd, off_out, at_end);
}
__device__ __forceinline__ float probe_radius(const DevParams& P, float acc) {
  const float a = acc > 0.0f ? acc : P.gps_accuracy;
  const float r = a > P.search_radius ? a : P.search_radius;
  return r < P.max_search_radius ? r : P.max_search_radius;
}

__device__ __forceinline__ uint32_t fbits(float f) { return __float_as_uint(f); }
__device__ __forceinline__ float bitsf(uint32_t u) { return __uint_as_float(u); }
__device__ __forceinline__ uint32_t hash32(uint32_t x) { return x * 2654435761u; }

__device__ __forceinline__ void cadd(unsigned long long* c, unsigned long long v) {
  if (c && v) atomicAdd(c, v);
}

__device__ __forceinline__ int2 crec(const DevWork& w, int64_t p, int j) {
  return j < KIN ? w.cand_eo[p * KIN + j] : w.cand_xeo[p * KX + (j - KIN)];
}
__device__ __forceinline__ float cemis(const DevWork& w, int64_t p, int j) {
  return j < KIN ? w.cand_em[p * KIN + j] : w.cand_xem[p * KX + (j - KIN)];
}
__device__ __forceinline__ void cput(const DevWork& w, int64_t p, int j, int32_t e, float off, float em) {
  if (j < KIN) {
    w.cand_eo[p * KIN + j] = make_int2(e, __float_as_int(off));
    w.cand_em[p * KIN + j] = em;
  } else {
    w.cand_xeo[p * KX + (j - KIN)] = make_int2(e, __float_as_int(off));
    w.cand_xem[p * KX + (j - KIN)] = em;
  }
}

__device__ __forceinline__ uint32_t turn_deg(uint32_t hin, uint32_t hout) {
  int d = (int)hout - (int)hin;
  d += d < 0 ? 360 : 0;
  return (uint32_t)(d <= 180 ? d : 360 - d);
}
__device__ __forceinline__ float trans_cost(uint32_t units, float r, float gcv, float beta) {
  units = units > TURN_UNITS_MAX ? TURN_UNITS_MAX : units;
  const float tc = (float)units * 0.015625f;
  const float diff = fabsf(r - gcv);
  return (tc + diff) / beta;
}

constexpr uint32_t NO_HEAD = 0xFFFFu;
__device__ __forceinline__ bool cand_node(float off) { return off == 0.0f; }
__device__ __forceinline__ int32_t src_node(const DevGraph& g, int32_t e, float off) {
  return cand_node(off) ? g.e_from[e] : g.e_to[e];
}
__device__ __forceinline__ float src_start(const DevGraph& g, int32_t e, float off) {
  return cand_node(off) ? 0.0f : g.e_len[e] - off;
}
__device__ __forceinline__ uint32_t src_head(const DevGraph& g, int32_t e, float off) {
  return cand_node(off) ? NO_HEAD : (uint32_t)g.e_head_in[e];
}
__device__ __forceinline__ uint32_t dst_head(const DevGraph& g, int32_t e, float off) {
  return cand_node(off) ? NO_HEAD : (uint32_t)g.e_head_out[e];
}
__device__ __forceinline__ bool same_edge_step(int32_t ei, float oi, int32_t ej, float oj) {
  return ei == ej && (oj >= oi || (!cand_node(oj) && !cand_node(oi)));
}
__device__ __forceinline__ float same_edge_dist(float oi, float oj) { return oj >= oi ? oj - oi : 0.0f; }
__device__ __forceinline__ uint32_t turn_units(const uint32_t* TU, uint32_t hin, uint32_t hout) {
  return (hin == NO_HEAD || hout == NO_HEAD) ? 0u : TU[turn_deg(hin, hout)];
}

__device__ __forceinline__ int wave_incl_scan(int v, int lane) {
#pragma unroll
  for (int o = 1; o < 64; o <<= 1) {
    int n = __shfl_up(v, o, 64);
    if (lane >= o) v += n;
  }
  return v;
}

__device__ __forceinline__ void fold_snap(DevWork& w, int k, bool reset) {
  for (int t = 0; t < CTR_STAGE_WORDS; ++t) {
    w.snap[CTR_STAGE_WORDS * k + t] = w.counters_i32[t];
    if (reset) w.counters_i32[t] = 0;
  }
}
template <CtrSlot C>
__device__ __forceinline__ void spill_push(const DevWork& w, int32_t p) {
  const SpillRef s = spill_of<C>(w);
  s.list[atomicAdd(s.count, 1)] = p;
}
__device__ __forceinline__ bool trans_over_cap(const DevBatch& b, const DevWork& w) {
  if (w.trans_off[b.n_points] <= w.trans_cap) return false;
  *w.abort = 1;
  return true;
}

__device__ __forceinline__ int hilbert_d(int x, int y) {
  int d = 0;
  for (int sft = ORDER_SIDE / 2; sft > 0; sft >>= 1) {
    const int rx = (x & sft) > 0;
    const int ry = (y & sft) > 0;
    d += sft * sft * ((3 * rx) ^ ry);
    if (ry == 0) {
      if (rx == 1) {
        x = ORDER_SIDE - 1 - x;
        y = ORDER_SIDE - 1 - y;
      }
      const int tmp = x;
      x = y;
      y = tmp;
    }
  }
  return d;
}

__device__ __forceinline__ int tile_of(const DevGraph& g, float lat, float lon) {
  int ty = (int)((lat - g.bb_lat0) * g.bb_inv_h);
  int tx = (int)((lon - g.bb_lon0) * g.bb_inv_w);
  ty = ty < 0 ? 0 : (ty >= ORDER_SIDE ? ORDER_SIDE - 1 : ty);
  tx = tx < 0 ? 0 : (tx >= ORDER_SIDE ? ORDER_SIDE - 1 : tx);
  return hilbert_d(tx, ty);
}

struct AggMatch {
  int leader;
  int rank;
  int count;
};
__device__ __forceinline__ AggMatch agg_match(int key, bool active) {
  const int lane = threadIdx.x & 63;
  unsigned long long pending = __ballot(active);
  AggMatch m{lane, 0, 0};
  while (pending) {
    const int leader = __ffsll((long long)pending) - 1;
    const int k = __shfl(key, leader, 64);
    const unsigned long long grp = __ballot(((pending >> lane) & 1ull) && key == k);
    if ((grp >> lane) & 1ull) {
      m.leader = leader;
      m.rank = (int)__popcll(grp & ((1ull << lane) - 1ull));
      m.count = (int)__popcll(grp);
    }
    pending &= ~grp;
  }
  return m;
}
__device__ __forceinline__ int wave_agg_slot(int32_t* ctr, int key, bool active) {
  const AggMatch m = agg_match(key, active);
  int base = 0;
  if (active && m.leader == (int)(threadIdx.x & 63)) base = atomicAdd(&ctr[key], m.count);
  return __shfl(base, m.leader, 64) + m.rank;
}
__device__ __forceinline__ void wave_agg_count(int32_t* ctr, int key, bool active) {
  const AggMatch m = agg_match(key, active);
  if (active && m.leader == (int)(threadIdx.x & 63)) atomicAdd(&ctr[key], m.count);
}

__global__ __launch_bounds__(1024) void k_order_plan(const int32_t* tile_cnt, int32_t* cursor, int32_t* grp) {
  __shared__ int32_t part[1024];
  __shared__ int32_t cut[ORDER_GROUPS + 1];
  constexpr int PER = ORDER_TILES / 1024;
  const int tid = threadIdx.x;
  int32_t v[PER], sum = 0;
  for (int k = 0; k < PER; ++k) {
    v[k] = tile_cnt[tid * PER + k];
    sum += v[k];
  }
  part[tid] = sum;
  if (tid <= ORDER_GROUPS) cut[tid] = 0x7fffffff;
  __syncthreads();
  for (int o = 1; o < 1024; o <<= 1) {
    const int32_t x = tid >= o ? part[tid - o] : 0;
    __syncthreads();
    part[tid] += x;
    __syncthreads();
  }
  const int32_t total = part[1023];
  int32_t run = part[tid] - sum;
  int32_t prev_start = tid == 0 ? -1 : run - tile_cnt[tid * PER - 1];
  for (int k = 0; k < PER; ++k) {
    cursor[tid * PER + k] = run;
    for (int gi = 1; gi < ORDER_GROUPS; ++gi) {
      const int64_t want = ((int64_t)total * gi + ORDER_GROUPS - 1) / ORDER_GROUPS;
      if (run >= want && prev_start < want) cut[gi] = run;
    }
    prev_start = run;
    run += v[k];
  }
  __syncthreads();
  if (tid == 0) {
    grp[0] = 0;
    int32_t prev = 0;
    for (int gi = 1; gi < ORDER_GROUPS; ++gi) {
      const int32_t c = cut[gi] > total ? total : cut[gi];
      prev = c > prev ? c : prev;
      grp[gi] = prev;
    }
    grp[ORDER_GROUPS] = total;
  }
}

__global__ __launch_bounds__(256) void k_order_scatter(DevBatch b, DevWork w, const uint16_t* tile, int32_t* cursor,
                                                       int32_t* item) {
  for (int64_t p0 = (int64_t)blockIdx.x * 256; p0 < b.n_points; p0 += (int64_t)gridDim.x * 256) {
    const int64_t p = p0 + threadIdx.x;
    const bool col = p < b.n_points && w.is_col[p];
    const int t = col ? (int)tile[p] : 0;
    const int pos = wave_agg_slot(cursor, t, col);
    if (col) item[pos] = (int32_t)p;
    if (col && w.colrec_pos) w.colrec_pos[p] = pos;
  }
}

#ifndef OTM_COL_PTS
#define OTM_COL_PTS 256
#endif
constexpr int COL_PTS = OTM_COL_PTS;
__global__ __launch_bounds__(TB) void k_columns(DevGraph g, DevBatch b, DevParams P, DevWork w) {
  __shared__ float sLat[COL_PTS], sLon[COL_PTS], sGc[COL_PTS];
  __shared__ int32_t sPrev[COL_PTS];
  __shared__ uint8_t sCol[COL_PTS];
  const int lane = threadIdx.x;
  if (blockIdx.x == 0) {
    if (lane < CTR_ZEROED_WORDS) w.counters_i32[lane] = 0;
    if (lane == 0) *w.abort = 0;
  }
  for (int32_t t = blockIdx.x; t < b.n_traces; t += gridDim.x) {
    const int64_t a = b.trace_off[t], e = b.trace_off[t + 1];
    const int n = (int)(e - a);
    int ncols = 0;
    if (n > COL_PTS) {
      if (lane == 0) {
        int64_t last = -1;
        for (int64_t p = a; p < e; ++p) {
          float gcv = 0.0f;
          if (last >= 0) gcv = gc_dist(b.lat[last], b.lon[last], b.lat[p], b.lon[p]);
          const bool col = last < 0 || gcv >= P.interp;
          w.is_col[p] = col ? 1 : 0;
          w.gc[p] = col ? gcv : 0.0f;
          w.prevc[p] = (int32_t)last;
          if (col) {
            last = p;
            ++ncols;
            if (w.ord.tile_cnt) {
              const int tl = tile_of(g, b.lat[p], b.lon[p]);
              w.ord.tile[p] = (uint16_t)tl;
              atomicAdd(&w.ord.tile_cnt[tl], 1);
            }
          }
        }
      }
      for (int64_t p = a + lane; p < e; p += TB) {
        w.probe[p] = make_float4(b.lat[p], b.lon[p], b.acc[p], 0.0f);
        w.pt_trace[p] = t;
        w.ncand[p] = 0;
        w.route_dist[p] = 0.0f;
        w.ipos[p] = -1.0f;
        w.nextc[p] = -1;
      }
    } else {
      for (int pl = lane; pl < n; pl += TB) {
        sLat[pl] = b.lat[a + pl];
        sLon[pl] = b.lon[a + pl];
      }
      __syncthreads();
      bool near = false;
      for (int pl = lane; pl < n; pl += TB) {
        const float d = pl > 0 ? gc_dist(sLat[pl - 1], sLon[pl - 1], sLat[pl], sLon[pl]) : 0.0f;
        sGc[pl] = d;
        near = near || (pl > 0 && !(d >= P.interp));
      }
      __syncthreads();
      if (__ballot(near) == 0ull) {
        for (int pl = lane; pl < n; pl += TB) {
          sCol[pl] = 1;
          sPrev[pl] = pl > 0 ? (int32_t)(a + pl - 1) : -1;
        }
        ncols = n;
      } else if (lane == 0) {
        int last = -1;
        for (int pl = 0; pl < n; ++pl) {
          float gcv = 0.0f;
          if (last >= 0) gcv = last == pl - 1 ? sGc[pl] : gc_dist(sLat[last], sLon[last], sLat[pl], sLon[pl]);
          const bool col = last < 0 || gcv >= P.interp;
          sCol[pl] = col ? 1 : 0;
          sGc[pl] = col ? gcv : 0.0f;
          sPrev[pl] = last >= 0 ? (int32_t)(a + last) : -1;
          if (col) {
            last = pl;
            ++ncols;
          }
        }
      }
      __syncthreads();
      for (int c0 = 0; c0 < n; c0 += TB) {
        const int pl = c0 + lane;
        const bool in = pl < n;
        const bool col = in && sCol[pl];
        if (in) {
          const int64_t p = a + pl;
          w.probe[p] = make_float4(sLat[pl], sLon[pl], b.acc[p], 0.0f);
          w.pt_trace[p] = t;
          w.is_col[p] = sCol[pl];
          w.gc[p] = sGc[pl];
          w.prevc[p] = sPrev[pl];
          w.ncand[p] = 0;
          w.route_dist[p] = 0.0f;
          w.ipos[p] = -1.0f;
          w.nextc[p] = -1;
        }
        if (w.ord.tile_cnt) {
          const int tl = col ? tile_of(g, sLat[pl], sLon[pl]) : 0;
          if (col) w.ord.tile[a + pl] = (uint16_t)tl;
          wave_agg_count(w.ord.tile_cnt, tl, col);
        }
      }
      __syncthreads();
    }
    if (lane == 0) {
      w.trace_err[t] = 0;
      if (w.ctr) {
        cadd(&w.ctr->points, (unsigned long long)n);
        cadd(&w.ctr->columns, (unsigned long long)ncols);
      }
    }
  }
}

struct ItemRange {
  int64_t i0, i1, stride;
  bool ordered;
};
__device__ __forceinline__ ItemRange item_range(const DevWork& w, const DevBatch& b, bool ordered, int per_block) {
  ItemRange r;
  r.ordered = ordered;
  const int tid = per_block > 1 ? (int)threadIdx.x : 0;
  if (ordered) {
    const int grp = blockIdx.x % ORDER_GROUPS;
    r.i0 = w.ord.grp[grp] + (int64_t)(blockIdx.x / ORDER_GROUPS) * per_block + tid;
    r.i1 = w.ord.grp[grp + 1];
    r.stride = (int64_t)(gridDim.x / ORDER_GROUPS) * per_block;
  } else {
    r.i0 = (int64_t)blockIdx.x * per_block + tid;
    r.i1 = b.n_points;
    r.stride = (int64_t)gridDim.x * per_block;
  }
  return r;
}

constexpr int HCAP = 512;
constexpr uint32_t NODE_ENT = 0x80000000u;
#ifndef OTM_CAND_LANE_CAP
#define OTM_CAND_LANE_CAP 8
#endif
constexpr int CAND_LANE_CAP = OTM_CAND_LANE_CAP;
#ifndef OTM_CAND_TB
#define OTM_CAND_TB 256
#endif
#ifndef OTM_CAND_WAVES
#define OTM_CAND_WAVES 8
#endif
constexpr int CAND_TB = OTM_CAND_TB;
#ifndef OTM_CAND_INFL
#define OTM_CAND_INFL 2
#endif
constexpr int CAND_INFL = OTM_CAND_INFL;
#ifndef OTM_SNAP_B
#define OTM_SNAP_B 2
#endif
constexpr int SNAP_B = OTM_SNAP_B;
__device__ __forceinline__ void wave_cadd(unsigned long long* c, unsigned long long v) {
  for (int o = 32; o > 0; o >>= 1) v += __shfl_xor(v, o, 64);
  if ((threadIdx.x & 63) == 0 && v) atomicAdd(c, v);
}

template <bool CTR>
__global__ __launch_bounds__(CAND_TB, OTM_CAND_WAVES) void k_cand_lane(DevGraph g, DevBatch b, DevParams P, DevWork w) {
  __shared__ uint32_t sE[CAND_LANE_CAP * CAND_TB];
  __shared__ float sQ[CAND_LANE_CAP * CAND_TB];
  uint32_t* E = sE + threadIdx.x;
  float* Q = sQ + threadIdx.x;
  static_assert(CAND_LANE_CAP <= 8 && CAND_LANE_CAP % SNAP_B == 0, "3-bit slots; whole snap steps");
  constexpr int S = CAND_TB;
  unsigned long long c_cells = 0, c_ent = 0, c_cand = 0;
  const ItemRange R = item_range(w, b, (P.order_mask & ORDER_CAND) != 0, CAND_TB);
  for (int64_t it = R.i0; it < R.i1; it += R.stride) {
    const int64_t p = R.ordered ? (int64_t)w.ord.item[it] : it;
    if (!R.ordered && !w.is_col[p]) continue;
    if (P.cand_wave_all) {
      spill_push<CTR_CAND_WAVE>(w, (int32_t)p);
      continue;
    }
    const float4 pr = w.probe[p];
    const float lat = pr.x, lon = pr.y;
    const float r = probe_radius(P, pr.z);
    const float r2 = r * r;
    const float ls = MPD_F * cos_deg(lat);
    const float dlat = r / MPD_F;
    const float dlon = r / ls;
    const double la_lo = ((double)lat - (double)dlat - g.lat0) / g.cell;
    const double la_hi = ((double)lat + (double)dlat - g.lat0) / g.cell;
    const double lo_lo = ((double)lon - (double)dlon - g.lon0) / g.cell;
    const double lo_hi = ((double)lon + (double)dlon - g.lon0) / g.cell;
// ... 273 lines not shown
    const float dlat = r / MPD_F;
    const float dlon = r / ls;
    const double la_lo = ((double)lat - (double)dlat - g.lat0) / g.cell;
    const double la_hi = ((double)lat + (double)dlat - g.lat0) / g.cell;
    const double lo_lo = ((double)lon - (double)dlon - g.lon0) / g.cell;
    const double lo_hi = ((double)lon + (double)dlon - g.lon0) / g.cell;
    const double R = g.grid_rows, Cn = g.grid_cols;
    int r0 = 0, r1 = -1, c0 = 0, c1 = -1;
    if (!(la_hi < 0.0 || lo_hi < 0.0 || la_lo >= R || lo_lo >= Cn)) {
      r0 = la_lo < 0.0 ? 0 : (int)floor(la_lo);
      r1 = la_hi >= R ? (int)R - 1 : (int)floor(la_hi);
      c0 = lo_lo < 0.0 ? 0 : (int)floor(lo_lo);
      c1 = lo_hi >= Cn ? (int)Cn - 1 : (int)floor(lo_hi);
    }
    const int ncols = c1 - c0 + 1;
    const int ncells = (r1 - r0 + 1) * ncols;
    for (int i = lane; i < hcap; i += TB) {
      Mem<BIG>::st(&hkey[i], (uint32_t)EMPTY);
      Mem<BIG>::st(&hval[i], (unsigned long long)LAB_NONE);
    }
    if (lane == 0) {
      s_count = 0;
      s_over = 0;
      s_n = 0;
    }
    __syncthreads();
    unsigned long long scanned = 0;
    for (int cb = 0; cb < ncells; cb += TB) {
      const int c = cb + lane;
      int cnt = 0;
      int64_t cs = 0;
      if (c < ncells) {
        const int rr = r0 + c / ncols, cc = c0 + c % ncols;
        const size_t cidx = (size_t)rr * (size_t)g.grid_cols + (size_t)cc;
        cs = g.cell_off[cidx];
        cnt = (int)(g.cell_off[cidx + 1] - cs);
      }
      const int incl = wave_incl_scan(cnt, lane);
      const int total = __shfl(incl, 63, 64);
      cexcl[lane] = incl - cnt;
      cstart[lane] = cs;
      __syncthreads();
      const int nc_here = min(TB, ncells - cb);
      for (int gi = lane; gi < total; gi += TB) {
        int lo = 0, hi = nc_here - 1;
        while (lo < hi) {
          const int mid = (lo + hi + 1) >> 1;
          if (cexcl[mid] <= gi) lo = mid;
          else hi = mid - 1;
        }
        const int64_t q = cstart[lo] + (gi - cexcl[lo]);
        const uint32_t ent = g.cell_ent[q];
        const float4 G = g.ent_geo[q];
        const int32_t e = (int32_t)(ent >> 4), k = (int32_t)(ent & 15u);
        const float sqd = seg_sqdist(G.x, G.y, G.z, G.w, lat, lon, ls);
        if (!(sqd <= r2)) continue;
        uint32_t slot = hash32((uint32_t)e) >> (32 - hlog2);
        bool placed = false;
        for (int probe = 0; probe < hcap; ++probe) {
          const uint32_t old = atomicCAS(&hkey[slot], EMPTY, (uint32_t)e);
          if (old == EMPTY) {
            if (atomicAdd(&s_count, 1) >= max_hits) s_over = 1;
            placed = true;
            break;
          }
          if (old == (uint32_t)e) {
            placed = true;
            break;
          }
          slot = (slot + 1) & (uint32_t)(hcap - 1);
        }
        if (!placed) {
          s_over = 1;
          continue;
        }
        atomicMin(&hval[slot], ((unsigned long long)fbits(sqd) << 32) | (unsigned long long)k);
      }
      scanned += (unsigned long long)total;
      __syncthreads();
    }
    if (s_over) {
      if (lane == 0) {
        if (!BIG) {
          spill_push<CTR_CAND_BIG>(w, (int32_t)p);
        } else if (w.cand_final) {
          w.ncand[p] = 0;
          atomicCAS(&w.trace_err[w.pt_trace[p]], 0, OTM_TERR_CAND_OVERFLOW);
        } else {
          w.ncand[p] = 0;
          w.counters_i32[CTR_GROW_CAND] = 1;
          *w.abort = 1;
        }
      }
      __syncthreads();
      continue;
    }
    for (int i = lane; i < hcap; i += TB) {
      const uint32_t hk = Mem<BIG>::ld(&hkey[i]);
      if (hk != EMPTY) {
        const unsigned long long hv = Mem<BIG>::ld(&hval[i]);
        const int idx = atomicAdd(&s_n, 1);
        Mem<BIG>::st(&skey[idx],
                     (hv & 0xFFFFFFFF00000000ull) | ((unsigned long long)hk << 5) | ((hv & 15ull) << 1));
      }
    }
    __syncthreads();
    for (int i = lane; i < hcap; i += TB) {
      Mem<BIG>::st(&hkey[i], (uint32_t)EMPTY);
      Mem<BIG>::st(&hval[i], (unsigned long long)LAB_NONE);
    }
    if (lane == 0) s_count = 0;
    __syncthreads();
    const int n0 = s_n;
    for (int idx = lane; idx < n0; idx += TB) {
      const unsigned long long key = Mem<BIG>::ld(&skey[idx]);
      const int32_t e = (int32_t)(((uint32_t)key) >> 5);
      float sqd, off;
      bool at_end;
      const ProjIn pin = proj_load(g, e, (int32_t)((key >> 1) & 15ull));
      proj_calc(pin, lat, lon, ls, sqd, off, at_end);
      const int32_t v = snap_rep(pin, off, at_end);
      if (v < 0) {
        Mem<BIG>::st(&skey[idx], key | 1ull);
        atomicAdd(&s_count, 1);
      } else {
        Mem<BIG>::st(&skey[idx], (unsigned long long)LAB_NONE);
        const uint32_t rep = (uint32_t)v;
        uint32_t slot = hash32(rep) >> (32 - hlog2);
        while (true) {
          const uint32_t old = atomicCAS(&hkey[slot], EMPTY, rep);
          if (old == EMPTY || old == rep) break;
          slot = (slot + 1) & (uint32_t)(hcap - 1);
        }
        atomicMin(&hval[slot], (key & 0xFFFFFFFF00000000ull) | (unsigned long long)idx);
      }
    }
    __syncthreads();
    for (int i = lane; i < hcap; i += TB) {
      const uint32_t hk = Mem<BIG>::ld(&hkey[i]);
      if (hk != EMPTY) {
        const unsigned long long hv = Mem<BIG>::ld(&hval[i]);
        Mem<BIG>::st(&skey[(int)(hv & 0xFFFFFFFFull)], (hv & 0xFFFFFFFF00000000ull) | ((unsigned long long)hk << 5));
        atomicAdd(&s_count, 1);
      }
    }
    __syncthreads();
    const int ns = n0;
    const int n = s_count;
    int N = 1;
    while (N < ns) N <<= 1;
    for (int i = ns + lane; i < N; i += TB) Mem<BIG>::st(&skey[i], (unsigned long long)LAB_NONE);
    __syncthreads();
    for (int kk = 2; kk <= N; kk <<= 1) {
      for (int j = kk >> 1; j > 0; j >>= 1) {
        for (int i = lane; i < N; i += TB) {
          const int ixj = i ^ j;
          if (ixj > i) {
            const unsigned long long x = Mem<BIG>::ld(&skey[i]), y = Mem<BIG>::ld(&skey[ixj]);
            const bool up = (i & kk) == 0;
            if ((x > y) == up) {
              Mem<BIG>::st(&skey[i], y);
              Mem<BIG>::st(&skey[ixj], x);
            }
          }
        }
        __syncthreads();
      }
    }
    const int K = n < P.max_candidates ? n : P.max_candidates;
    if (lane < K) {
      const unsigned long long key = Mem<BIG>::ld(&skey[lane]);
      const int32_t e = (int32_t)(((uint32_t)key) >> 5);
      float sqd = bitsf((uint32_t)(key >> 32)), off = 0.0f;
      if (key & 1ull) project(g, e, (int32_t)((key >> 1) & 15ull), lat, lon, ls, sqd, off);
      const float ds = (2.0f * P.sigma_z) * P.sigma_z;
      cput(w, p, lane, e, off, sqd / ds);
    } else if (lane < KIN) {
      cput(w, p, lane, -1, 0.0f, INFINITY);
    }
    if (lane == 0) {
      w.ncand[p] = K;
      if (w.ctr) {
        cadd(&w.ctr->cells_visited, (unsigned long long)ncells);
        cadd(&w.ctr->cell_entries_scanned, scanned);
        cadd(&w.ctr->candidates, (unsigned long long)K);
      }
    }
    __syncthreads();
  }
}

__global__ __launch_bounds__(256) void k_links(DevBatch b, DevParams P, DevWork w) {
  const int64_t p = (int64_t)blockIdx.x * blockDim.x + threadIdx.x;
  if (p > b.n_points) return;
  if (p == b.n_points) {
    w.trans_off[p] = 0;
    fold_snap(w, SNAP_AFTER_CAND, true);
    return;
  }
  int32_t cp = -1, kq = 0;
  int64_t cnt = 0;
  if (w.is_col[p]) {
    const int32_t q = w.prevc[p];
    if (q >= 0 && p - q > 1) w.nextc[q] = (int32_t)p;
    if (q >= 0 && w.ncand[p] > 0 && w.ncand[q] > 0 && w.gc[p] <= P.breakage) {
      cp = q;
      kq = w.ncand[q];
      cnt = (int64_t)kq * (int64_t)w.ncand[p];
    }
  }
  w.col_prev[p] = cp;
  w.kq_prev[p] = kq;
  w.trans_off[p] = cnt;
  if (w.colrec && (P.order_mask & ORDER_TRANS) && w.is_col[p])
    w.colrec[w.colrec_pos[p]] = make_int4((int32_t)p, cp, kq | (w.ncand[p] << 8), __float_as_int(w.gc[p]));
  w.vmeta[p] = (uint8_t)((w.is_col[p] ? (w.ncand[p] | 0x40) : 0) | (cp >= 0 ? 0x80 : 0));
}

__global__ void k_status(const int32_t* abort, const int64_t* ttotal, const int32_t* counters, BatchStatus* out) {
  if (threadIdx.x == 0) {
    out->abort = *abort;
    out->grow = (counters[CTR_GROW_HUGE] != 0 ? GROW_HUGE : 0) | (counters[CTR_GROW_CAND] != 0 ? GROW_CAND : 0);
    out->ttotal = *ttotal;
    out->pool_used = counters[CTR_POOL_USED];
    out->pool_over = counters[CTR_POOL_OVER];
    out->route_huge = counters[CTR_ROUTE_HUGE];
  }
}

struct Table {
  uint32_t* key;
  unsigned long long* lab;
  uint32_t* inq;
  uint32_t* fr0;
  uint32_t* fr1;
  int cap_log2;
  int limit;
  uint32_t* ins = nullptr;
  int32_t* prev = nullptr;
};

struct SearchShared {
  int nfr, nnext, count, over;
};

template <bool BIG>
__device__ __forceinline__ int table_find(const Table& T, uint32_t v) {
  const uint32_t mask = (1u << T.cap_log2) - 1u;
  uint32_t slot = hash32(v) >> (32 - T.cap_log2);
  for (int i = 0; i <= (int)mask; ++i) {
    const uint32_t k = Mem<BIG>::ld(&T.key[slot]);
    if (k == v) return (int)slot;
    if (k == EMPTY) return -1;
    slot = (slot + 1) & mask;
  }
  return -1;
}

template <bool BIG>
__device__ __forceinline__ void ta_relax(const Table& T, SearchShared& S, uint32_t* nxt, uint32_t key,
                                         unsigned long long nl) {
  const uint32_t mask = (1u << T.cap_log2) - 1u;
  uint32_t slot = hash32(key) >> (32 - T.cap_log2);
  int found = -1;
  for (int i = 0; i <= (int)mask; ++i) {
    const uint32_t old = atomicCAS(&T.key[slot], EMPTY, key);
    if (old == EMPTY) {
      const int c = atomicAdd(&S.count, 1);
      if (c >= T.limit) S.over = 1;
      else if (BIG) Mem<true>::st(&T.ins[c], slot);
      found = (int)slot;
      break;
    }
    if (old == key) {
      found = (int)slot;
      break;
    }
    slot = (slot + 1) & mask;
  }
  if (found < 0) {
    S.over = 1;
    return;
  }
  const unsigned long long old = atomicMin(&T.lab[found], nl);
  if (!(key & NODE_KEY) && nl < old && (uint32_t)(old >> 32) != (uint32_t)(nl >> 32)) {
    if (atomicExch(&T.inq[found], 1u) == 0u) {
      const int idx = atomicAdd(&S.nnext, 1);
      Mem<BIG>::st(&nxt[idx], (uint32_t)found);
    }
  }
}

template <bool BIG>
__device__ int ta_search(const DevGraph& g, const uint32_t* TU, const Table& T, SearchShared& S, int32_t u,
                         uint32_t hin, uint32_t cmax, int lane) {
  const int cap = 1 << T.cap_log2;
  const int pc = BIG ? Mem<true>::ld(T.prev) : -1;
  if (pc < 0) {
    for (int i = lane; i < cap; i += TB) {
      Mem<BIG>::st(&T.key[i], EMPTY);
      Mem<BIG>::st(&T.lab[i], LAB_NONE);
      Mem<BIG>::st(&T.inq[i], 0u);
    }
  } else {
    for (int i = lane; i < pc; i += TB) {
      const uint32_t sl = Mem<true>::ld(&T.ins[i]);
      Mem<BIG>::st(&T.key[sl], EMPTY);
      Mem<BIG>::st(&T.lab[sl], LAB_NONE);
      Mem<BIG>::st(&T.inq[sl], 0u);
// ... 309 lines not shown
    base = (int64_t)blockIdx.x * NS;
    end = w.counters_i32[CTR_TRANS_WIDE];
    stride = (int64_t)gridDim.x * NS;
  } else if (ordered) {
    const int grp = blockIdx.x % ORDER_GROUPS;
    base = w.ord.grp[grp] + (int64_t)(blockIdx.x / ORDER_GROUPS) * NS;
    end = w.ord.grp[grp + 1];
    stride = (int64_t)(gridDim.x / ORDER_GROUPS) * NS;
  } else {
    base = (int64_t)blockIdx.x * NS;
    end = b.n_points;
    stride = (int64_t)gridDim.x * NS;
  }
  for (; base < end; base += stride) {
    const int64_t it = base + sg;
    bool act = it < end;
    int64_t p = 0;
    int32_t q = -1;
    int Kp = 0, Kq = 0;
    float gcv = 0.0f;
    int64_t toff = 0;
    if (act && ordered && w.colrec) {
      const int4 A = w.colrec[it];
      p = A.x;
      toff = w.trans_off[p];
      q = A.y;
      Kq = A.z & 255;
      Kp = A.z >> 8;
      gcv = __int_as_float(A.w);
    } else if (act) {
      p = LIST ? (int64_t)spill_list<CTR_TRANS_WIDE>(w)[it] : (ordered ? (int64_t)w.ord.item[it] : it);
      q = w.col_prev[p];
      Kq = w.kq_prev[p];
      Kp = w.ncand[p];
      gcv = w.gc[p];
      toff = w.trans_off[p];
    }
    act = act && q >= 0;
    const float bound = P.factor * gcv;
    const uint32_t cq = index_cost_bound(bound);
    const bool idx_ok = X.rmax > 0.0f && cq <= X.cmax;
    const SrcRec* xsrc = X.src;
    const uint4* xslot = X.slot;
#pragma unroll
    for (int l = NEAR_LEVELS - 1; l >= 0; --l) {
      if (w.idxn[l].rmax > 0.0f && cq <= w.idxn[l].cmax) {
        xsrc = w.idxn[l].src;
        xslot = w.idxn[l].slot;
      }
    }
    const bool wide = WIDE && act && idx_ok && (Kp > KC || Kq > KC);
    if (wide && sl == 0) spill_push<CTR_TRANS_WIDE>(w, (int32_t)p);
    act = act && !wide;
    bool bad = act && (!idx_ok || Kp > KC || Kq > KC);
    for (int k = sl; k < KC; k += S) {
      if (act && k < Kp) {
        const int2 c = crec(w, p, k);
        const int32_t e = c.x;
        const float o = __int_as_float(c.y);
        const uint32_t key = dst_key(g, e, o);
        tg[sg][k ^ swz] = make_int4(e, __float_as_int(o), (int)key, (int)idx_hash(key));
      }
      if (act && k < Kq) {
        const int2 c = crec(w, q, k);
        const int32_t e = c.x;
        const float o = __int_as_float(c.y);
        IdxRow R{};
        int32_t lenb;
        if (idx_ok) {
          R = src_row(xsrc, e, cand_node(o));
          lenb = xsrc[e].len;
        } else {
          lenb = g.e_fl[e].y;
        }
        const float start = cand_node(o) ? 0.0f : __int_as_float(lenb) - o;
        sr[sg][k ^ swz] = make_int4(e, __float_as_int(o), __float_as_int(start), w.ctr ? (int)src_head(g, e, o) : 0);
        if (idx_ok) {
          rq[sg][k ^ swz] = R;
          bad = bad || R.cnt < 0;
        }
      }
    }
    const bool spill = (__ballot(bad) & smask) != 0ull;
    if (spill && act && sl == 0) spill_push<CTR_INDEX_MISS>(w, (int32_t)p);
    act = act && !spill;
    const int npair_g = act ? Kq * Kp : 0;
    if (sl == 0) {
      const unsigned long long xs = (unsigned long long)xslot;
      cr[sg][0] = make_int4((int)(uint32_t)toff, (int)(uint32_t)((unsigned long long)toff >> 32),
                            act ? (Kp | Kq << 8 | 1 << 16) : 0, __float_as_int(gcv));
      cr[sg][1] = make_int4(__float_as_int(bound), (int)cq, (int)(uint32_t)xs, (int)(uint32_t)(xs >> 32));
    }
    wave_sync();
    {
      int pre[NS], total = 0;
#pragma unroll
      for (int c = 0; c < NS; ++c) {
        pre[c] = total;
        total += __builtin_amdgcn_readlane(npair_g, c * S);
      }
      unsigned long long ntr = 0;
      for (int f = lane; f < total; f += TB) {
        int c = 0, pc = 0;
#pragma unroll
        for (int k = 1; k < NS; ++k) {
          if (f >= pre[k]) {
            c = k;
            pc = pre[k];
          }
        }
        const int idx = f - pc;
        const int cz = S == 8 ? ((c >> 1) & 1) * 4 : (c & 1) * 8;
        const int4 C0 = cr[c][0], C1 = cr[c][1];
        const int kp = C0.z & 255;
        const float gcv_c = __int_as_float(C0.w), bound_c = __int_as_float(C1.x);
        const uint32_t cq_c = (uint32_t)C1.y;
        const uint4* xslot_c = (const uint4*)word64(C1.z, C1.w);
        const int64_t toff_c = (int64_t)word64(C0.x, C0.y);
        const int i = idx / kp, j = idx - (idx / kp) * kp;
        const int4 T = tg[c][j ^ cz], Sx = sr[c][i ^ cz];
        const uint32_t key = (uint32_t)T.z;
        const int32_t ej = T.x, ei = Sx.x;
        const float oj = __int_as_float(T.y), oi = __int_as_float(Sx.y), si = __int_as_float(Sx.z);
        float r = 0.0f;
        bool ok = true;
        uint32_t units = 0;
        if (same_edge_step(ei, oi, ej, oj)) {
          r = same_edge_dist(oi, oj);
        } else {
          const IdxRow R = rq[c][i ^ cz];
          uint4 sv = make_uint4(EMPTY, 0u, 0u, 0u);
          if (R.cnt > 0) {
            uint32_t h = idx_slot0((uint32_t)T.w, R);
            sv = xslot_c[R.off + h];
            uint4 s1 = xslot_c[R.off + h + 1];
            if (sv.x != key && sv.x != EMPTY) {
              sv = s1;
              h = h + 1u;
              while (sv.x != key && sv.x != EMPTY) {
                h = idx_next(h, R);
                sv = xslot_c[R.off + h];
              }
            }
          }
          if (R.cnt > 0 && sv.x == key && idx_slot_cost(sv) <= cq_c) {
            const float sd = si + bitsf(sv.z);
            r = sd + oj;
            units = idx_slot_units(sv);
          } else {
            ok = false;
          }
        }
        float cost = INFINITY;
        if (ok && r <= bound_c) {
          cost = trans_cost(units, r, gcv_c, P.beta);
          ++ntr;
        }
        w.trans[toff_c + idx] = cost;
      }
      if (w.ctr) {
        const int4 C0 = cr[sg][0], C1 = cr[sg][1];
        if (C0.z >> 16)
          count_searches((C0.z >> 8) & 255, (uint32_t)C1.y, (const uint4*)word64(C1.z, C1.w));
        c_trans += ntr;
      }
    }
    wave_sync();
  }
  if (w.ctr) {
    for (int sh = 32; sh > 0; sh >>= 1) {
      c_search += __shfl_xor(c_search, sh, 64);
      c_settled += __shfl_xor(c_settled, sh, 64);
      c_relaxed += __shfl_xor(c_relaxed, sh, 64);
      c_trans += __shfl_xor(c_trans, sh, 64);
    }
    if (lane == 0) {
      cadd(&w.ctr->searches, c_search);
      cadd(&w.ctr->nodes_settled, c_settled);
      cadd(&w.ctr->edges_relaxed, c_relaxed);
      cadd(&w.ctr->transitions, c_trans);
    }
  }
}

#ifndef OTM_ROUTE_WAVES
#define OTM_ROUTE_WAVES 1
#endif
__global__ __launch_bounds__(256, OTM_ROUTE_WAVES) void k_route_index(DevGraph g, DevBatch b, DevParams P, DevWork w) {
  if (*w.abort) return;
  const DevIndex& X = w.idx;
  unsigned long long c_search = 0, c_settled = 0, c_relaxed = 0, c_edges = 0;
  const ItemRange R = item_range(w, b, (P.order_mask & ORDER_ROUTE) != 0, 256);
  const bool rec = R.ordered && w.colrec && (P.order_mask & ORDER_TRANS);
  for (int64_t it = R.i0; it < R.i1; it += R.stride) {
    int64_t p;
    int32_t q = -1;
    float gcv = 0.0f;
    if (rec) {
      const int4 A = w.colrec[it];
      p = A.x;
      q = A.y;
      gcv = __int_as_float(A.w);
    } else {
      p = R.ordered ? (int64_t)w.ord.item[it] : it;
    }
    if (!R.ordered && !w.is_col[p]) continue;
    w.route_dist[p] = 0.0f;
    w.path_len[p] = 0;
    w.path_off[p] = 0;
    const int2 cq0 = w.chosen[q >= 0 ? q : p];
    if (w.state[p] < 0 || w.chain_start[p]) continue;
    if (!rec) {
      q = w.col_prev[p];
      gcv = w.gc[p];
    }
    const int2 ci = rec ? cq0 : w.chosen[q], cj = w.chosen[p];
    const int32_t ei = ci.x, ej = cj.x;
    const float oi = __int_as_float(ci.y), oj = __int_as_float(cj.y);
    if (same_edge_step(ei, oi, ej, oj)) {
      w.route_dist[p] = same_edge_dist(oi, oj);
      continue;
    }
    const float bound = P.factor * gcv;
    const uint32_t cq = index_cost_bound(bound);
    IdxRow Rw{};
    int64_t sv = -1;
    uint4 lab{};
    int lvl = -1;
#pragma unroll
    for (int l = NEAR_LEVELS - 1; l >= 0; --l)
      if (w.idxn[l].rmax > 0.0f && cq <= w.idxn[l].cmax) lvl = l;
    const DevIndex& Xc = lvl >= 0 ? w.idxn[lvl] : X;
    int32_t leni = 0;
    if (X.rmax > 0.0f && cq <= X.cmax) {
      Rw = src_row(Xc.src, ei, cand_node(oi));
      leni = Xc.src[ei].len;
      sv = idx_find(Xc.slot, Rw, dst_key(g, ej, oj), lab);
    }
    if (sv < 0 || idx_slot_cost(lab) > cq) {
      spill_push<CTR_INDEX_MISS>(w, (int32_t)p);
      continue;
    }
    int len = 0;
    for (int32_t ps = idx_slot_pred(lab); ps >= 0 && len <= Rw.cnt; ps = idx_slot_pred(Xc.slot[Rw.off + ps])) ++len;
    const int off = len ? atomicAdd(&w.counters_i32[CTR_POOL_USED], len) : 0;
    if (off + len > w.pool_cap) {
      w.counters_i32[CTR_POOL_OVER] = 1;
      *w.abort = 1;
      w.path_len[p] = -1;
    } else {
      int k = len;
      for (int32_t ps = idx_slot_pred(lab); ps >= 0 && k > 0;) {
        const uint4 sl = Xc.slot[Rw.off + ps];
        w.path_pool[off + (--k)] = (int32_t)sl.x;
        ps = idx_slot_pred(sl);
      }
      w.path_off[p] = off;
      w.path_len[p] = len;
    }
    const float start = cand_node(oi) ? 0.0f : __int_as_float(leni) - oi;
    const float sd = start + bitsf(lab.z);
    w.route_dist[p] = sd + oj;
    if (w.ctr) {
      unsigned long long st = 0, rl = 0;
      for (int64_t k = 0; k < (int64_t)Rw.cap; ++k) {
        const uint4 sl = Xc.slot[Rw.off + k];
        if (sl.x == EMPTY || (sl.x & NODE_KEY) || idx_slot_cost(sl) > cq) continue;
        ++st;
        if ((unsigned long long)idx_slot_cost(sl) + g.e_len64[sl.x] <= cq) {
          const int32_t v = g.e_to[sl.x];
          rl += (unsigned long long)(g.out_off[v + 1] - g.out_off[v]);
        }
      }
      ++c_search;
      c_settled += st;
      c_relaxed += rl;
      c_edges += (unsigned long long)len;
    }
  }
  if (w.ctr) {
    cadd(&w.ctr->route_searches, c_search);
    cadd(&w.ctr->route_nodes_settled, c_settled);
    cadd(&w.ctr->route_edges_relaxed, c_relaxed);
    cadd(&w.ctr->route_edges, c_edges);
  }
}

template <int TIER>
__device__ __forceinline__ Table tier_table(const DevWork& w, uint32_t* lkey, unsigned long long* llab, uint32_t* linq,
                                            uint32_t* lfr0, uint32_t* lfr1) {
  if (TIER == 1) {
    const size_t base = (size_t)blockIdx.x * BIG_TABLE_CAP;
    return Table{w.big_key + base, w.big_lab + base, w.big_inq + base, w.big_fr + 2 * base,
                 w.big_fr + 2 * base + BIG_TABLE_CAP, BIG_TABLE_LOG2, SEARCH_LIMIT,
                 w.big_ins + (size_t)blockIdx.x * SEARCH_LIMIT, w.big_prev + blockIdx.x};
  }
  if (TIER == 2) {
    const size_t cap = (size_t)1 << w.huge_log2;
    const size_t base = (size_t)blockIdx.x * cap;
    const int lim = huge_limit(w.huge_log2);
    return Table{w.huge_key + base, w.huge_lab + base, w.huge_inq + base, w.huge_fr + 2 * base,
                 w.huge_fr + 2 * base + cap, w.huge_log2, lim, w.huge_ins + (size_t)blockIdx.x * lim,
                 w.huge_prev + blockIdx.x};
  }
  return Table{lkey, llab, linq, lfr0, lfr1, 8, LDS_TABLE_LIMIT};
}
__device__ __forceinline__ bool huge_unready(DevWork& w, int64_t nwork, const int32_t* list) {
  if (nwork <= 0 || w.huge_log2 > 0) return false;
  if (w.huge_final) {
    for (int64_t it = (int64_t)blockIdx.x * blockDim.x + threadIdx.x; it < nwork; it += (int64_t)gridDim.x * blockDim.x)
      atomicCAS(&w.trace_err[w.pt_trace[list[it]]], 0, OTM_TERR_SEARCH_OVERFLOW);
  } else if (blockIdx.x == 0 && threadIdx.x == 0) {
    w.counters_i32[CTR_GROW_HUGE] = 1;
    *w.abort = 1;
  }
  return true;
}
__device__ __forceinline__ void huge_overflow(DevWork& w, int64_t p) {
  if (w.huge_final) {
    atomicCAS(&w.trace_err[w.pt_trace[p]], 0, OTM_TERR_SEARCH_OVERFLOW);
  } else {
    w.counters_i32[CTR_GROW_HUGE] = 1;
    *w.abort = 1;
// ... 470 lines not shown
    __syncthreads();
    for (int pl = lane; pl < n; pl += TB) {
      const int st = sState[pl];
      const int cs = sCs[pl];
      w.state[a + pl] = st;
      w.chain_start[a + pl] = (uint8_t)cs;
      if (st >= 0) {
        w.chosen[a + pl] = crec(w, a + pl, st);
      }
    }
    __syncthreads();
  }
}

__device__ __forceinline__ int wave_max_i(int v) {
#pragma unroll
  for (int o = 32; o > 0; o >>= 1) {
    const int x = __shfl_xor(v, o, 64);
    v = x > v ? x : v;
  }
  return v;
}
#ifndef OTM_VG8_WAVES
#define OTM_VG8_WAVES 4
#endif
#ifndef OTM_VG8_U
#define OTM_VG8_U 8
#endif
#ifndef OTM_VG_CHUNK
#define OTM_VG_CHUNK 4
#endif
constexpr int VG_PTS = 128;
constexpr uint8_t VG_COL = 1, VG_CS = 2, VG_END = 4;
template <int G>
__global__ __launch_bounds__(TB, G == 8 ? OTM_VG8_WAVES : 3) void k_viterbi_g(DevBatch b, DevWork w, const int32_t* list,
                                                                const int32_t* list_n, int32_t* rej, int32_t* rej_n,
                                                                int snap) {
  static_assert(G == 8 || G == 16, "8 or 16 lanes per trace");
  constexpr int NT = TB / G;
  constexpr int U = G == 8 ? OTM_VG8_U : 16;
  constexpr int VT = U * G;
  constexpr int CH = OTM_VG_CHUNK;
  static_assert(CH <= G, "a chunk's metadata is one byte per lane");
  if (snap && blockIdx.x == 0 && threadIdx.x == 0) fold_snap(w, SNAP_AFTER_TRANS, true);
  if (*w.abort) return;
  __shared__ float sT[NT][VT + G];
  __shared__ float sE[NT][CH * G + G];
  __shared__ uint8_t sBp[NT][VG_PTS * G / 2 + 4];
  __shared__ uint8_t sFl[NT][VG_PTS];
  __shared__ __attribute__((aligned(16))) float sP[NT][G];
  const int lane = threadIdx.x;
  const int g = lane / G, j = lane % G, gb = g * G;
  const unsigned long long gmask = (1ull << G) - 1ull;
  const int32_t ntr = list ? *list_n : b.n_traces;
  for (int32_t tb = blockIdx.x * NT; tb < ntr; tb += gridDim.x * NT) {
    const int32_t it = tb + g;
    bool act = it < ntr;
    const int32_t t = act ? (list ? list[it] : it) : 0;
    int64_t a = 0;
    int n = 0;
    int64_t t0 = 0;
    if (act) {
      a = b.trace_off[t];
      n = (int)(b.trace_off[t + 1] - a);
      t0 = w.trans_off[a];
      if (w.trace_err[t] != 0) {
        for (int pl = j; pl < n; pl += G) {
          w.state[a + pl] = -1;
          w.chain_start[a + pl] = 0;
        }
        act = false;
      }
    }
    bool take = act && n <= VG_PTS;
    if (take) {
      bool wide = false;
      for (int pl = j; pl < n; pl += G) {
        const int vm = w.vmeta[a + pl];
        wide = wide || ((vm & 0x40) && (vm & 0x3F) > G);
      }
      take = ((__ballot(wide) >> gb) & gmask) == 0ull;
    }
    if (act && !take) {
      if (j == 0) rej[atomicAdd(rej_n, 1)] = t;
      act = false;
    }
    if (!act) n = 0;
    const int nch = (wave_max_i(n) + CH - 1) / CH;
    for (int pl = j; pl < n; pl += G) sFl[g][pl] = 0;
    const int nl = n > 0 ? n - 1 : 0;
    auto ld_meta = [&](int c) {
      const int pl = c * CH + j;
      return (int)w.vmeta[a + (pl < nl ? pl : nl)];
    };
    auto ld_range = [&](int c, int64_t& lo, int64_t& hi) {
      const int p0 = c * CH < n ? c * CH : n, p1 = c * CH + CH < n ? c * CH + CH : n;
      lo = w.trans_off[a + p0];
      hi = w.trans_off[a + p1];
    };
    float pTa[U], pEa[CH], pTb[U], pEb[CH];
    auto ld_data = [&](int c, int m, int lo, int hi, float (&pT)[U], float (&pE)[CH]) {
      (void)m;
#pragma unroll
      for (int u = 0; u < U; ++u) {
        const int f = lo + u * G + j;
        pT[u] = w.trans[t0 + (f < hi ? f : lo)];
      }
#pragma unroll
      for (int k = 0; k < CH; ++k) {
        const int pl = c * CH + k < nl ? c * CH + k : nl;
        pE[k] = j < KIN ? w.cand_em[(a + pl) * KIN + j] : w.cand_xem[(a + pl) * KX + (j - KIN)];
      }
    };
    int m0 = ld_meta(0), m1 = ld_meta(1), m2 = ld_meta(2), m3 = ld_meta(3);
    int64_t lo0, hi0, lo1, hi1, lo2, hi2, lo3, hi3;
    ld_range(0, lo0, hi0);
    ld_range(1, lo1, hi1);
    ld_range(2, lo2, hi2);
    ld_range(3, lo3, hi3);
    ld_data(0, m0, (int)(lo0 - t0), (int)(hi0 - t0), pTa, pEa);
    ld_data(1, m1, (int)(lo1 - t0), (int)(hi1 - t0), pTb, pEb);
    float prev = INFINITY;
    sP[g][j] = INFINITY;
    bool open = false;
    int last = -1, lastK = 0;
    int acc = 0;
    auto end_chain = [&]() {
      float bv = j < lastK ? prev : INFINITY;
      int bi = j;
#pragma unroll
      for (int o = G / 2; o > 0; o >>= 1) {
        const float ov = __shfl_xor(bv, o, G);
        const int oi = __shfl_xor(bi, o, G);
        if (ov < bv || (ov == bv && oi < bi)) {
          bv = ov;
          bi = oi;
        }
      }
      if (j == 0) sFl[g][last] = (uint8_t)(sFl[g][last] | VG_END | (bi << 3));
    };
    auto stage = [&](const float (&pT)[U], const float (&pE)[CH]) {
#pragma unroll
      for (int u = 0; u < U; ++u) sT[g][u * G + j] = pT[u];
#pragma unroll
      for (int k = 0; k < CH; ++k) sE[g][k * G + j] = pE[k];
    };
    auto chunk = [&](int c, int m_c, int lo_c, int hi_c) {
      const bool big = hi_c - lo_c > VT;
      for (int k = 0; k < CH; ++k) {
        const int pl = c * CH + k;
        const int mk = __shfl(m_c, gb + k, TB);
        const bool on = pl < n && (mk & 0x40);
        const int Kp = mk & 0x3F;
        if (on && Kp == 0) {
          if (open) end_chain();
          open = false;
        }
        const bool col = on && Kp > 0;
        const bool link = col && open && (mk & 0x80);
        const int to = acc;
        if (link) acc += lastK * Kp;
        const int jj = j < Kp ? j : 0;
        const float em = sE[g][k * G + jj];
        int tb = to - lo_c;
        if (__ballot(big && link) != 0ull) {
          if (big) {
            tb = 0;
// ... 137 lines not shown
template <int I0>
__device__ __forceinline__ void vr_load(const float* Tm, const int Kp, float (&tv)[16]) {
#pragma unroll
  for (int u = 0; u < 4; ++u) tv[I0 + u] = Tm[(I0 + u) * Kp];
}
template <int I0>
__device__ __forceinline__ void vr_four(const int pbits, const float (&tv)[16], float& best, int& bi) {
  float v0 = __int_as_float(__builtin_amdgcn_update_dpp(0, pbits, 0x150 + I0 + 0, 0xF, 0xF, false)) + tv[I0 + 0];
  float v1 = __int_as_float(__builtin_amdgcn_update_dpp(0, pbits, 0x150 + I0 + 1, 0xF, 0xF, false)) + tv[I0 + 1];
  float v2 = __int_as_float(__builtin_amdgcn_update_dpp(0, pbits, 0x150 + I0 + 2, 0xF, 0xF, false)) + tv[I0 + 2];
  float v3 = __int_as_float(__builtin_amdgcn_update_dpp(0, pbits, 0x150 + I0 + 3, 0xF, 0xF, false)) + tv[I0 + 3];
  int i0 = __float_as_int(v0), i1 = __float_as_int(v1), i2 = __float_as_int(v2), i3 = __float_as_int(v3);
  asm("" : "+v"(i0));
  asm("" : "+v"(i1));
  asm("" : "+v"(i2));
  asm("" : "+v"(i3));
  const int m = min(min(i0, i1), min(i2, i3));
  int fu = 3;
  fu = i2 == m ? 2 : fu;
  fu = i1 == m ? 1 : fu;
  fu = i0 == m ? 0 : fu;
  const bool lt = m < __float_as_int(best);
  best = lt ? __int_as_float(m) : best;
  bi = lt ? I0 + fu : bi;
}
__global__ __launch_bounds__(TB, OTM_VR_WAVES) void k_viterbi_row(DevBatch b, DevWork w, int32_t* rej, int32_t* rej_n,
                                                                  int win, int fast, int snap) {
  constexpr int G = 16, NT = TB / G;
  constexpr int CH = OTM_VR_CH, U = OTM_VR_U;
  constexpr int VT = U * G;
  constexpr int VTA = VT > G * G ? VT : G * G;
  constexpr int RS = VTA + G;
  static_assert(CH >= 1 && CH <= G && U >= 4 && U % 4 == 0, "chunk knobs");
  static_assert(RS % 4 == 0, "a row's window is staged by 16-byte stores");
  if (snap && blockIdx.x == 0 && threadIdx.x == 0) fold_snap(w, SNAP_AFTER_TRANS, true);
  if (*w.abort) return;
  __shared__ __attribute__((aligned(16))) float sT[NT * RS + G * G];
  __shared__ __attribute__((aligned(8))) uint8_t sBp[NT][VR_PTS * G / 2];
  __shared__ __attribute__((aligned(8))) uint8_t sFl[NT][VR_PTS];
  __shared__ __attribute__((aligned(16))) uint32_t sM[NT][VR_PTS + G];
  const int lane = threadIdx.x;
  const int g = lane / G, j = lane % G, gb = g * G;
  for (int f = lane; f < NT * RS + G * G; f += TB) sT[f] = INFINITY;
  float* const sTg = sT + g * RS;
  const int32_t ntr = b.n_traces;
  for (int32_t tb0 = blockIdx.x * NT; tb0 < ntr; tb0 += gridDim.x * NT) {
    const int32_t t = tb0 + g;
    bool act = t < ntr;
    int64_t a = 0, t0 = 0;
    int n = 0;
    if (act) {
      a = b.trace_off[t];
      n = (int)(b.trace_off[t + 1] - a);
      if (w.trace_err[t] != 0) {
        for (int pl = j; pl < n; pl += G) {
          w.state[a + pl] = -1;
          w.chain_start[a + pl] = 0;
        }
        act = false;
      }
      if (n <= 0) act = false;
    }
    bool take = act && n <= VR_PTS;
    if (take) {
      t0 = w.trans_off[a];
      int vm[VR_PTS / G + 1];
      int64_t to[VR_PTS / G + 1];
#pragma unroll
      for (int u = 0; u <= VR_PTS / G; ++u) {
        const int pl = u * G + j;
        vm[u] = w.vmeta[a + (pl < n ? pl : n - 1)];
        to[u] = w.trans_off[a + (pl < n ? pl : n)];
      }
      bool wide = false;
#pragma unroll
      for (int u = 0; u <= VR_PTS / G; ++u) {
        const int pl = u * G + j;
        if (pl < n) wide = wide || ((vm[u] & 0x40) && (vm[u] & 0x3F) > G);
        if (pl <= n) sM[g][pl] = (uint32_t)(pl < n ? vm[u] : 0) | ((uint32_t)(to[u] - t0) << 8);
      }
      take = ((__ballot(wide) >> gb) & 0xFFFFull) == 0ull;
    }
    if (act && !take) {
      if (j == 0) rej[atomicAdd(rej_n, 1)] = t;
      act = false;
    }
    if (!act) n = 0;
    const int nch = __builtin_amdgcn_readfirstlane((wave_max_i(n) + CH - 1) / CH);
    for (int pl = j; pl < ((n + 3) & ~3); pl += G) {
      const uint32_t m = sM[g][pl];
      sFl[g][pl] = (uint8_t)(pl < n && (m & 0x40u) && (m & 0x3Fu) ? VG_COL : 0);
    }
    wave_sync();
    const int nl = n > 0 ? n - 1 : 0;
    auto rng_end = [&](int c) {
      const int p1 = c * CH + CH < n ? c * CH + CH : n;
      return act ? (int)(sM[g][p1] >> 8) : 0;
    };
    const float* const ep = j < KIN ? w.cand_em + a * KIN + j : w.cand_xem + a * KX + (j - KIN);
    const int es = j < KIN ? KIN : KX;
    vr_f4 pT[U / 4];
    float pE[CH];
    auto ld_data = [&](int c, int lo, int hi) {
      const int64_t f0 = t0 + lo;
      if (__ballot(f0 + VT > w.trans_cap) == 0ull) {
        const float* const tp = w.trans + (f0 + 4 * j);
#pragma unroll
        for (int q = 0; q < U / 4; ++q) pT[q] = *(const vr_f4*)(tp + q * 4 * G);
      } else {
#pragma unroll
        for (int q = 0; q < U / 4; ++q) {
#pragma unroll
          for (int e = 0; e < 4; ++e) {
            const int f = lo + q * 4 * G + 4 * j + e;
            pT[q][e] = w.trans[t0 + (f < hi ? f : lo)];
          }
        }
      }
#pragma unroll
      for (int k = 0; k < CH; ++k) {
        const int pl = c * CH + k < nl ? c * CH + k : nl;
        pE[k] = ep[pl * es];
      }
    };
    int lo_n = 0, hi_n = rng_end(0);
    ld_data(0, lo_n, hi_n);
    float prev = INFINITY;
    bool open = false;
    int last = 0, lastK = 0;
    auto end_chain = [&]() {
      float bv = j < lastK ? prev : INFINITY;
      int bi = j;
#pragma unroll
      for (int o = G / 2; o > 0; o >>= 1) {
        const float ov = __shfl_xor(bv, o, G);
        const int oi = __shfl_xor(bi, o, G);
        if (ov < bv || (ov == bv && oi < bi)) {
          bv = ov;
          bi = oi;
        }
      }
      if (j == 0) sFl[g][last] = (uint8_t)(sFl[g][last] | VG_END | (bi << 3));
    };
    for (int c = 0; c < nch; ++c) {
      const int lo_c = lo_n, hi_c = hi_n;
#pragma unroll
      for (int q = 0; q < U / 4; ++q) *(vr_f4a*)(sTg + q * 4 * G + 4 * j) = pT[q];
      float em_c[CH];
      uint32_t mw[CH];
#pragma unroll
      for (int k = 0; k < CH; ++k) {
        em_c[k] = pE[k];
        mw[k] = sM[g][c * CH + k];
      }
      wave_sync();
      lo_n = hi_c;
      hi_n = rng_end(c + 1);
      ld_data(c + 1, lo_n, hi_n);
      const bool big = hi_c - lo_c > win;
#pragma unroll
      for (int k = 0; k < CH; ++k) {
        const int pl = c * CH + k;
        const int mk = (int)(mw[k] & 0xFFu);
        const bool on = pl < n && (mk & 0x40);
        const int Kp = mk & 0x3F;
        const bool col = on && Kp > 0;
        const bool link = col && open && (mk & 0x80);
// ... 549 lines not shown
    const int hn = __shfl_up((int)head, d, 64);
    if (lane >= d) {
      if (!head) v = vn > v ? vn : v;
      head = head || hn != 0;
    }
  }
  if (!head) v = carry > v ? carry : v;
  return v;
}

struct StateStep {
  int32_t pts;
  uint32_t f;
  int32_t ei, ej;
  float oi, oj;
  int32_t plen, poff;
  double ta, tb;
  float rd;
  __device__ int pl() const { return pts & 0xFFFF; }
  __device__ int lp() const { return pts >> 16; }
  __device__ bool cs() const { return f & 1u; }
  __device__ bool last() const { return f & 2u; }
  __device__ bool step() const { return f & 4u; }
  __device__ bool same() const { return f & 8u; }
};
template <class SP>
__device__ __forceinline__ StateStep state_step(const DevWork& w, const DevBatch& b, int64_t a, const SP& S, int k,
                                                int ns) {
  StateStep r;
  const int pl = S.sidx[k];
  const int nx = k + 1 < ns ? S.sidx[k + 1] : pl;
  const int pv = k > 0 ? S.sidx[k - 1] : pl;
  const int64_t p = a + pl;
  const bool csp = w.chain_start[p] != 0;
  const bool csn = w.chain_start[a + nx] != 0;
  const int2 cj = w.chosen[p];
  const int2 cv = w.chosen[a + pv];
  const int32_t pln = w.path_len[p], pof = w.path_off[p];
  const double tp = b.time[p], tv = b.time[a + pv];
  r.rd = w.route_dist[p];
  const bool last = k == ns - 1 || csn;
  const bool step = !csp && k > 0;
  const int lp = step ? pv : pl;
  r.pts = pl | (lp << 16);
  r.ej = cj.x;
  r.oj = __int_as_float(cj.y);
  const int2 ci = step ? cv : cj;
  r.ei = ci.x;
  r.oi = __int_as_float(ci.y);
  const bool same = step && same_edge_step(r.ei, r.oi, r.ej, r.oj);
  r.f = (csp ? 1u : 0u) | (last ? 2u : 0u) | (step ? 4u : 0u) | (same ? 8u : 0u);
  const bool leaves = step && !same;
  r.plen = leaves ? (pln > 0 ? pln : 0) : 0;
  r.poff = leaves ? pof : 0;
  r.tb = tp;
  r.ta = step ? tv : tp;
  return r;
}

template <int PT, int TR>
__global__ __launch_bounds__(TB, (PT <= 128 ? 4 : 2)) void k_segments(DevGraph g, DevBatch b, DevWork w, DevOut o, const int32_t* list,
                                                 const int32_t* list_n, int32_t* spill, int32_t* spill_n) {
  if (*w.abort) return;
  __shared__ SegParT<PT, TR> S;
  const int lane = threadIdx.x;
  const unsigned long long lt = (1ull << lane) - 1ull;
  const int32_t nwork = list ? *list_n : b.n_traces;
  SEGP_DECL
  for (int32_t it = blockIdx.x; it < nwork; it += gridDim.x) {
    SEGP_START
    const int32_t t = list ? list[it] : it;
    const int64_t a = b.trace_off[t];
    const int n = (int)(b.trace_off[t + 1] - a);
    const int32_t base = (int32_t)o.seg_base[t];
    if (w.trace_err[t] != 0) {
      if (lane == 0) {
        o.seg_cnt[t] = 0;
        o.way_cnt[t] = 0;
      }
      continue;
    }
    if (n > PT) {
      if (lane == 0) {
        if (spill) spill[atomicAdd(spill_n, 1)] = t;
        else segments_trace<true>(g, w, o, t, n, base, SegSrcGlobal{&g, &b, &w, a});
      }
      continue;
    }
    constexpr int NCH = (PT + TB - 1) / TB;
    bool stv[NCH];
#pragma unroll
    for (int c = 0; c < NCH; ++c) {
      const int pl = c * TB + lane;
      const bool in = pl < n;
      const uint8_t ic = in ? w.is_col[a + pl] : (uint8_t)0;
      const int32_t sv = in ? w.state[a + pl] : -1;
      stv[c] = ic && sv >= 0;
    }
    int ns = 0;
#pragma unroll
    for (int c = 0; c < NCH; ++c) {
      const unsigned long long m = __ballot(stv[c]);
      if (stv[c]) S.sidx[ns + __popcll(m & lt)] = (int16_t)(c * TB + lane);
      ns += __popcll(m);
    }
    wave_sync();
    SEGP_MARK(1)
    StateStep rs[NCH];
#pragma unroll
    for (int c = 0; c < NCH; ++c)
      if (c * TB + lane < ns) rs[c] = state_step(w, b, a, S, c * TB + lane, ns);
    float elen[NCH];
#pragma unroll
    for (int c = 0; c < NCH; ++c) elen[c] = 0.0f;
    int c_chain = 0, c_open = -1, c_base = 0;
#pragma unroll
    for (int c = 0; c < NCH; ++c) {
      if (c * TB >= ns) break;
      const int k = c * TB + lane;
      const bool valid = k < ns;
      int cs = 0, opener = -1, nem = 0;
      if (valid) {
        const StateStep& r = rs[c];
        cs = r.cs() ? 1 : 0;
        if (r.cs() || !r.same()) opener = k;
        if (!r.cs() && !r.same()) elen[c] = rec_len(edge_rec(g, r.ei));
        nem = (r.step() && !r.same() ? (cand_node(r.oi) ? 0 : 1) + r.plen : 0) +
              (r.last() && !r.cs() && !cand_node(r.oj) ? 1 : 0);
      }
      const int ch = c_chain + wave_incl_scan(cs, lane);
      int lo = wave_incl_max(opener, lane);
      lo = lo > c_open ? lo : c_open;
      const int inc = wave_incl_scan(nem, lane);
      if (valid) {
        S.chain[k] = (int16_t)(ch - 1);
        S.lopen[k] = (int16_t)lo;
        S.tbase[k] = c_base + inc - nem;
      }
      c_chain = __shfl(ch, 63, 64);
      c_open = __shfl(lo, 63, 64);
      c_base += __shfl(inc, 63, 64);
    }
    const int nt = c_base;
    wave_sync();
    SEGP_MARK(2)
    if (nt > TR) {
      if (lane == 0) {
        if (spill) spill[atomicAdd(spill_n, 1)] = t;
        else segments_trace<true>(g, w, o, t, n, base, SegSrcGlobal{&g, &b, &w, a});
      }
      wave_sync();
      continue;
    }
#pragma unroll
    for (int c = 0; c < NCH; ++c) {
      const int k = c * TB + lane;
      if (k >= ns) continue;
      const StateStep& r = rs[c];
      int slot = S.tbase[k];
      if (r.step() && !r.same()) {
        if (!cand_node(r.oi)) S.t_edge[slot++] = -1;
        for (int i = 0; i < r.plen; ++i) S.t_edge[slot++] = -2 - (r.poff + i);
      }
      if (r.last() && !r.cs() && !cand_node(r.oj)) S.t_edge[slot] = -1;
    }
    wave_sync();
    SEGP_MARK(3)
    {
      constexpr int NTC = (TR + TB - 1) / TB;
      int32_t pe[NTC];
#pragma unroll
      for (int c = 0; c < NTC; ++c) {
        const int s = c * TB + lane;
        const int32_t v = s < nt ? S.t_edge[s] : -1;
        pe[c] = v <= -2 ? w.path_pool[-2 - v] : -1;
      }
#pragma unroll
      for (int c = 0; c < NTC; ++c) {
        const int s = c * TB + lane;
        if (pe[c] >= 0) {
          S.t_edge[s] = pe[c];
          S.t_off1[s] = rec_len(edge_rec(g, pe[c]));
        }
      }
    }
    wave_sync();
    SEGP_MARK(4)
#pragma unroll
    for (int c = 0; c < NCH; ++c) {
      const int k = c * TB + lane;
      if (k >= ns) continue;
      const StateStep& r = rs[c];
      if (r.cs()) {
        S.o_t0[k] = r.tb;
        S.o_off0[k] = r.oj;
        S.o_sh0[k] = (int16_t)r.pl();
      } else if (!r.same()) {
        const float start = cand_node(r.oi) ? 0.0f : elen[c] - r.oi;
        const int s0 = S.tbase[k] + (cand_node(r.oi) ? 0 : 1);
        float dd = 0.0f;
        for (int i = 0; i < r.plen; ++i) dd = dd + S.t_off1[s0 + i];
        const float x = start + dd;
        double t0;
        int sh;
        step_bound(b, w, a, r.lp(), r.pl(), r.rd, r.ta, r.tb, x, t0, sh);
        S.o_t0[k] = t0;
        S.o_off0[k] = 0.0f;
        S.o_sh0[k] = (int16_t)sh;
      }
    }
    wave_sync();
    SEGP_MARK(5)
#pragma unroll
    for (int c = 0; c < NCH; ++c) {
      const int k = c * TB + lane;
      if (k >= ns) continue;
      const StateStep& r = rs[c];
      int slot = S.tbase[k];
      const int16_t chk = S.chain[k];
      if (r.step() && !r.same()) {
        const float Rd = r.rd;
        const double ta = r.ta, tb = r.tb;
        const float el = elen[c];
        const float start = cand_node(r.oi) ? 0.0f : el - r.oi;
        if (!cand_node(r.oi)) {
          const int jo = S.lopen[k - 1];
          S.t_edge[slot] = r.ei;
          S.t_off0[slot] = S.o_off0[jo];
          S.t_t0[slot] = S.o_t0[jo];
          S.t_sh0[slot] = S.o_sh0[jo];
          S.t_off1[slot] = el;
          double t1;
// ... 1267 lines not shown
          int k = j - o_ex;
          double la, lo;
          if (o_cs && k == 0) {
            shape_coord(g, o_s0, o_m, o_b, la, lo);
          } else {
            k -= o_cs;
            if (k < o_nint) {
              la = (double)g.s_lat[o_s0 + o_i0 + k];
              lo = (double)g.s_lon[o_s0 + o_i0 + k];
            } else {
              shape_coord(g, o_s0, o_m, o_z, la, lo);
            }
          }
          qlat = (int32_t)rint(la * 1e6);
          qlon = (int32_t)rint(lo * 1e6);
        }
        int plat = __shfl_up(qlat, 1, 64), plon = __shfl_up(qlon, 1, 64);
        if (lane == 0) {
          plat = c_lat;
          plon = c_lon;
        }
        const int dla = qlat - plat, dlo = qlon - plon;
        const uint32_t za = ((uint32_t)dla << 1) ^ (uint32_t)(dla >> 31);
        const uint32_t zb = ((uint32_t)dlo << 1) ^ (uint32_t)(dlo >> 31);
        const int na = 1 + (31 - __clz((int)(za | 1u))) / 5, nb = 1 + (31 - __clz((int)(zb | 1u))) / 5;
        const int nby = act ? na + nb : 0;
        const int binc = wave_incl_scan(nby, lane);
        if (WRITE && act) {
          const int64_t vi = c_v + j, bp = c_b + binc - nby;
          if (vi < vcap) ((int2*)sh.vtx)[vb + vi] = make_int2(qlat, qlon);
          if (bp + nby <= pcap) shape_put(shape_put(sh.poly + pb + bp, za, na), zb, nb);
        }
        const int last = (total - v0 < TB ? total - v0 : TB) - 1;
        c_lat = __shfl(qlat, last, 64);
        c_lon = __shfl(qlon, last, 64);
        c_b += __shfl(binc, 63, 64);
      }
      c_v += total;
    }
    if (!WRITE && lane == 0) {
      sh.vtx_off[t] = c_v;
      sh.poly_off[t] = c_b;
    }
  }
}

int grid_for(int64_t n, int per_block, int cap) {
  int64_t g = (n + per_block - 1) / per_block;
  if (g < 1) g = 1;
  return (int)(g > cap ? cap : g);
}

constexpr int WAVE_GRID_CAP = 256 * 64;
#ifndef OTM_TRANS_GRID_CAP
#define OTM_TRANS_GRID_CAP 65536
#endif
constexpr int TRANS_GRID_CAP = OTM_TRANS_GRID_CAP;

}

void launch_fetch_scan(int32_t n, const int32_t* c0, const int32_t* c1, const int32_t* c2, int32_t* o0, int32_t* o1,
                       int32_t* o2, hipStream_t s) {
  hipLaunchKernelGGL(k_fetch_scan, dim3(1), dim3(1024), 0, s, n, c0, c1, c2, o0, o1, o2);
}


const char* const kKernelNames[KN_COUNT] = {
    "k_columns",       "spatial_order",  "k_cand_lane",    "k_candidates",     "k_links",         "scan_trans_off",  "k_trans_sub",
    "k_trans_wide",    "k_transitions",  "k_transitions_big", "k_viterbi",      "k_route_index",
    "k_route",         "k_route_big",    "k_seg_bound",      "scan_seg_bound",  "k_segments",       "k_report"};

namespace {
constexpr int SPILL_GRID = 4096;
#ifndef OTM_WIDE_GRID
#define OTM_WIDE_GRID 8192
#endif
constexpr int WIDE_GRID = OTM_WIDE_GRID;
}

#define TIMED(k, launch) \
  do {                   \
    mk.begin(k, s);      \
    launch;              \
    mk.end(k, s);        \
  } while (0)

void launch_columns(const DevGraph& g, const DevBatch& b, const DevParams& p, DevWork& w, hipStream_t s,
                    const Marks& mk) {
  if (w.ord.tile_cnt) (void)hipMemsetAsync(w.ord.tile_cnt, 0, ORDER_TILES * 4, s);
  TIMED(KN_COLUMNS, hipLaunchKernelGGL(k_columns, dim3(grid_for(b.n_traces, 1, WAVE_GRID_CAP)), dim3(TB), 0, s, g,
                                       b, p, w));
}
static int order_grid(int64_t n, int per_block, int cap) {
  const int64_t per_group = (n + ORDER_GROUPS - 1) / ORDER_GROUPS;
  int64_t gb = (per_group + per_group / 4 + per_block - 1) / per_block;
  if (gb < 1) gb = 1;
  int64_t gtot = gb * ORDER_GROUPS;
  if (gtot > cap) gtot = cap / ORDER_GROUPS * ORDER_GROUPS;
  return (int)gtot;
}

void launch_order(const DevBatch& b, DevWork& w, hipStream_t s, const Marks& mk) {
  mk.begin(KN_ORDER, s);
  hipLaunchKernelGGL(k_order_plan, dim3(1), dim3(1024), 0, s, w.ord.tile_cnt, w.ord.cursor, w.ord.grp);
  hipLaunchKernelGGL(k_order_scatter, dim3(grid_for(b.n_points, 256, 8192)), dim3(256), 0, s, b, w, w.ord.tile,
                     w.ord.cursor, w.ord.item);
  mk.end(KN_ORDER, s);
}

void launch_candidates(const DevGraph& g, const DevBatch& b, const DevParams& p, DevWork& w, hipStream_t s,
                       const Marks& mk, int from) {
  if (from < RESUME_CAND_BIG) {
    if (w.ctr)
      TIMED(KN_CAND_LANE, hipLaunchKernelGGL(k_cand_lane<true>, dim3(order_grid(b.n_points, CAND_TB, 1 << 30)),
                                             dim3(CAND_TB), 0, s, g, b, p, w));
    else
      TIMED(KN_CAND_LANE, hipLaunchKernelGGL(k_cand_lane<false>, dim3(order_grid(b.n_points, CAND_TB, 1 << 30)),
                                             dim3(CAND_TB), 0, s, g, b, p, w));
  }
  mk.begin(KN_CAND_WAVE, s);
#ifndef OTM_CAND_WAVE_GRID
#define OTM_CAND_WAVE_GRID 4096
#endif
  if (from < RESUME_CAND_BIG)
    hipLaunchKernelGGL(k_candidates<false>, dim3(OTM_CAND_WAVE_GRID), dim3(TB), 0, s, g, b, p, w);
  hipLaunchKernelGGL(k_candidates<true>, dim3(CAND_BIG_SLOTS), dim3(TB), 0, s, g, b, p, w);
  mk.end(KN_CAND_WAVE, s);
}
void launch_links(const DevBatch& b, const DevParams& p, DevWork& w, hipStream_t s, const Marks& mk) {
  TIMED(KN_LINKS, hipLaunchKernelGGL(k_links, dim3(grid_for(b.n_points + 1, 256, 1 << 30)), dim3(256), 0, s, b, p,
                                     w));
}
__global__ __launch_bounds__(256) void k_expand_compact(const int64_t* trace_off, const int64_t* tbase,
                                                        const int32_t* dt, const int16_t* acc16, double* time,
                                                        float* acc, int32_t n_traces) {
  const int wv = threadIdx.x >> 6, lane = threadIdx.x & 63;
  for (int64_t t = (int64_t)blockIdx.x * 4 + wv; t < n_traces; t += (int64_t)gridDim.x * 4) {
    const int64_t a = trace_off[t], e = trace_off[t + 1], base = tbase[t];
    for (int64_t i = a + lane; i < e; i += 64) {
      time[i] = (double)(base + (int64_t)dt[i]);
      acc[i] = (float)acc16[i];
    }
  }
}
void launch_expand_compact(const int64_t* trace_off, const int64_t* tbase, const int32_t* dt, const int16_t* acc16,
                           double* time, float* acc, int32_t n_traces, hipStream_t s) {
  if (n_traces <= 0) return;
  hipLaunchKernelGGL(k_expand_compact, dim3(grid_for(((int64_t)n_traces + 3) / 4, 1, 1 << 20)), dim3(256), 0, s,
                     trace_off, tbase, dt, acc16, time, acc, n_traces);
}
void launch_status(const int32_t* abort, const int64_t* ttotal, const int32_t* counters, BatchStatus* out,
                   hipStream_t s) {
  hipLaunchKernelGGL(k_status, dim3(1), dim3(64), 0, s, abort, ttotal, counters, out);
}
void launch_transitions(const DevGraph& g, const DevBatch& b, const DevParams& p, DevWork& w, hipStream_t s,
                        const Marks& mk, int sub, int from) {
  if (from >= RESUME_TRANS_HUGE) {
    mk.begin(KN_TRANS_GLOBAL, s);
    hipLaunchKernelGGL(k_transitions<2>, dim3(HUGE_SLOTS), dim3(TB), 0, s, g, b, p, w);
    mk.end(KN_TRANS_GLOBAL, s);
    return;
  }
  const int per = TB / sub;
  const int grid = order_grid((b.n_points + per - 1) / per, 1, TRANS_GRID_CAP);
  if (sub == 8) {
    TIMED(KN_TRANS_INDEX, hipLaunchKernelGGL((k_trans_sub<8, false>), dim3(grid), dim3(TB), 0, s, g, b, p, w));
    TIMED(KN_TRANS_WIDE, hipLaunchKernelGGL((k_trans_sub<16, true>), dim3(WIDE_GRID), dim3(TB), 0, s, g, b, p, w));
  } else {
    TIMED(KN_TRANS_INDEX, hipLaunchKernelGGL((k_trans_sub<16, false>), dim3(grid), dim3(TB), 0, s, g, b, p, w));
    mk.begin(KN_TRANS_WIDE, s);
    mk.end(KN_TRANS_WIDE, s);
  }
  TIMED(KN_TRANS_WAVE, hipLaunchKernelGGL(k_transitions<0>, dim3(SPILL_GRID), dim3(TB), 0, s, g, b, p, w));
  mk.begin(KN_TRANS_GLOBAL, s);
  hipLaunchKernelGGL(k_transitions<1>, dim3(BIG_SLOTS), dim3(TB), 0, s, g, b, p, w);
  hipLaunchKernelGGL(k_transitions<2>, dim3(HUGE_SLOTS), dim3(TB), 0, s, g, b, p, w);
  mk.end(KN_TRANS_GLOBAL, s);
}
void launch_viterbi(const DevBatch& b, DevWork& w, hipStream_t s, const Marks& mk) {
  const char* fe = std::getenv("OTM_VIT_FORM");
  const int forced = fe ? std::atoi(fe) : 0;
  constexpr int gmin = 32768;
  constexpr int rmin = 4096;
  const int form = forced ? forced : (b.n_traces >= gmin ? 8 : (b.n_traces >= rmin ? 4 : 64));
  const SpillRef to_16 = spill_of<CTR_VIT_16>(w), to_wave = spill_of<CTR_VIT_WAVE>(w);
  if (form == 4) {
    const char* we = std::getenv("OTM_VR_WIN");
    const int vt = OTM_VR_U * 16;
    int win = we ? std::atoi(we) : vt;
    win = win < 0 ? 0 : (win > vt ? vt : win);
    const char* fa = std::getenv("OTM_VR_FAST");
    const int fast = fa ? (std::atoi(fa) != 0 ? 1 : 0) : 1;
    mk.begin(KN_VITERBI, s);
    hipLaunchKernelGGL(k_viterbi_row, dim3(grid_for(b.n_traces, TB / 16, WAVE_GRID_CAP)), dim3(TB), 0, s, b, w,
                       to_wave.list, to_wave.count, win, fast, 1);
    hipLaunchKernelGGL(k_viterbi, dim3(grid_for(b.n_traces, 1, WAVE_GRID_CAP)), dim3(TB), 0, s, b, w,
                       (const int32_t*)to_wave.list, (const int32_t*)to_wave.count, 0);
    mk.end(KN_VITERBI, s);
    return;
  }
  if (form == 64) {
    TIMED(KN_VITERBI, hipLaunchKernelGGL(k_viterbi, dim3(grid_for(b.n_traces, 1, WAVE_GRID_CAP)), dim3(TB), 0, s, b,
                                         w, (const int32_t*)nullptr, (const int32_t*)nullptr, 1));
    return;
  }
  int32_t* l8 = to_16.list;
  int32_t* n8 = to_16.count;
  int32_t* l16 = to_wave.list;
  int32_t* n16 = to_wave.count;
  mk.begin(KN_VITERBI, s);
  if (form == 16) {
    hipLaunchKernelGGL(k_viterbi_g<16>, dim3(grid_for(b.n_traces, TB / 16, WAVE_GRID_CAP)), dim3(TB), 0, s, b, w,
                       (const int32_t*)nullptr, (const int32_t*)nullptr, l16, n16, 1);
  } else {
    hipLaunchKernelGGL(k_viterbi_g<8>, dim3(grid_for(b.n_traces, TB / 8, WAVE_GRID_CAP)), dim3(TB), 0, s, b, w,
                       (const int32_t*)nullptr, (const int32_t*)nullptr, l8, n8, 1);
    hipLaunchKernelGGL(k_viterbi_g<16>, dim3(grid_for(b.n_traces, TB / 16, WAVE_GRID_CAP)), dim3(TB), 0, s, b, w,
                       (const int32_t*)l8, (const int32_t*)n8, l16, n16, 0);
  }
  hipLaunchKernelGGL(k_viterbi, dim3(grid_for(b.n_traces / 64 + 1, 1, 1024)), dim3(TB), 0, s, b, w,
                     (const int32_t*)l16, (const int32_t*)n16, 0);
  mk.end(KN_VITERBI, s);
}
void launch_route(const DevGraph& g, const DevBatch& b, const DevParams& p, DevWork& w, hipStream_t s,
                  const Marks& mk, int from) {
  if (from >= RESUME_ROUTE_HUGE) {
    mk.begin(KN_ROUTE_GLOBAL, s);
    hipLaunchKernelGGL(k_route<2>, dim3(HUGE_SLOTS), dim3(TB), 0, s, g, b, p, w);
    mk.end(KN_ROUTE_GLOBAL, s);
    return;
  }
  TIMED(KN_ROUTE_INDEX, hipLaunchKernelGGL(k_route_index, dim3(order_grid(b.n_points, 256, 1 << 30)), dim3(256), 0,
                                           s, g, b, p, w));
  TIMED(KN_ROUTE_WAVE, hipLaunchKernelGGL(k_route<0>, dim3(SPILL_GRID), dim3(TB), 0, s, g, b, p, w));
  mk.begin(KN_ROUTE_GLOBAL, s);
  hipLaunchKernelGGL(k_route<1>, dim3(BIG_SLOTS), dim3(TB), 0, s, g, b, p, w);
  hipLaunchKernelGGL(k_route<2>, dim3(HUGE_SLOTS), dim3(TB), 0, s, g, b, p, w);
  mk.end(KN_ROUTE_GLOBAL, s);
}
void launch_segments(const DevGraph& g, const DevBatch& b, DevWork& w, DevOut& o, hipStream_t s, const Marks& mk) {
  const dim3 grid(grid_for(b.n_traces, 1, WAVE_GRID_CAP));
  const SpillRef large = spill_of<CTR_SEG_LARGE>(w);
  int32_t* lst = large.list;
  int32_t* cnt = large.count;
  mk.begin(KN_SEG_WRITE, s);
  hipLaunchKernelGGL((k_segments<SEGP_PTS_S, SEGP_TRAV_S>), grid, dim3(TB), 0, s, g, b, w, o, (const int32_t*)nullptr,
                     (const int32_t*)nullptr, lst, cnt);
  hipLaunchKernelGGL((k_segments<SEGP_PTS, SEGP_TRAV>), dim3(grid_for(b.n_traces, 1, 2048)), dim3(TB), 0, s, g, b, w,
                     o, (const int32_t*)lst, (const int32_t*)cnt, (int32_t*)nullptr, (int32_t*)nullptr);
  mk.end(KN_SEG_WRITE, s);
}
void launch_queue(const DevBatch& b, DevWork& w, DevOut& o, float kph, hipStream_t s) {
  hipLaunchKernelGGL(k_queue, dim3(grid_for(b.n_traces, 1, WAVE_GRID_CAP)), dim3(TB), 0, s, b, w, o, kph);
}
void launch_points(const DevGraph& g, const DevBatch& b, const DevParams& p, DevWork& w, otm_matched_point* out,
                   hipStream_t s) {
  hipLaunchKernelGGL(k_points, dim3(grid_for(b.n_traces, 1, WAVE_GRID_CAP)), dim3(TB), 0, s, g, b, p, w, out);
}
void launch_scores(const DevBatch& b, DevWork& w, const DevScores& sc, hipStream_t s) {
  if (b.n_traces <= 0 || b.n_points <= 0) return;
  const char* fe = std::getenv("OTM_SCORE_FORM");
  const int forced = fe ? std::atoi(fe) : 0;
  constexpr int rmin = 4096;
  const int form = forced == 1 || forced == 4 ? forced : (b.n_traces >= rmin ? 4 : 1);
  if (form == 1) {
    hipLaunchKernelGGL(k_scores<64>, dim3(grid_for(b.n_traces, 1, WAVE_GRID_CAP)), dim3(TB), 0, s, b, w, sc,
                       (const int32_t*)nullptr, (const int32_t*)nullptr, (int32_t*)nullptr, (int32_t*)nullptr);
    return;
  }
  (void)hipMemsetAsync(sc.rej_n, 0, sizeof *sc.rej_n, s);
  hipLaunchKernelGGL(k_scores<16>, dim3(grid_for(b.n_traces, TB / 16, WAVE_GRID_CAP)), dim3(TB), 0, s, b, w, sc,
                     (const int32_t*)nullptr, (const int32_t*)nullptr, sc.rej, sc.rej_n);
  hipLaunchKernelGGL(k_scores<64>, dim3(grid_for(b.n_traces, 1, WAVE_GRID_CAP)), dim3(TB), 0, s, b, w, sc,
                     (const int32_t*)sc.rej, (const int32_t*)sc.rej_n, (int32_t*)nullptr, (int32_t*)nullptr);
}
void launch_traversals(const DevGraph& g, const DevBatch& b, DevWork& w, DevOut& o, const DevTrav& tv, hipStream_t s) {
  hipLaunchKernelGGL(k_traversals, dim3(grid_for(b.n_traces, 1, WAVE_GRID_CAP)), dim3(TB), 0, s, g, b, w, o, tv);
}
void launch_trav_compact(int32_t n_traces, const int64_t* seg_base, const int64_t* off, const otm_traversal* reg,
                         otm_traversal* dst, hipStream_t s) {
  hipLaunchKernelGGL(k_trav_compact, dim3(grid_for(n_traces, 1, WAVE_GRID_CAP)), dim3(TB), 0, s, n_traces, seg_base, off,
                     reg, dst);
}
void launch_shape(const DevGraph& g, int32_t n_traces, const int64_t* seg_base, const DevTrav& tv, const DevShape& sh,
                  bool write, hipStream_t s) {
  const dim3 grid(grid_for(n_traces, 1, WAVE_GRID_CAP));
  if (write)
    hipLaunchKernelGGL(k_shape<true>, grid, dim3(TB), 0, s, g, n_traces, seg_base, tv, sh);
  else
    hipLaunchKernelGGL(k_shape<false>, grid, dim3(TB), 0, s, g, n_traces, seg_base, tv, sh);
}
void launch_seg_bound(const DevGraph& g, const DevBatch& b, const DevParams& p, DevWork& w, int64_t* tb, hipStream_t s,
                      const Marks& mk) {
  TIMED(KN_SEG_BOUND, hipLaunchKernelGGL(k_seg_bound, dim3(grid_for(b.n_points + 1, 256, 1 << 30)), dim3(256), 0, s,
                                         g, b, p, w, tb));
}
void launch_compact(int32_t n_traces, const DevOut& o, const int32_t* seg_off, const int32_t* way_off,
                    const int32_t* rep_off, otm_segment* segs_out, int64_t* ways_out, otm_report_rec* reps_out,
                    otm_trace_result* traces_out, hipStream_t s) {
  hipLaunchKernelGGL(k_compact, dim3(grid_for(n_traces, 1, WAVE_GRID_CAP)), dim3(TB), 0, s, n_traces, o, seg_off, way_off,
                     rep_off, segs_out, ways_out, reps_out, traces_out);
}
void launch_report(const DevBatch& b, const DevReportCfg& rc, DevWork& w, DevOut& o, hipStream_t s,
                   const Marks& mk) {
  constexpr int tb = 16;
  if (b.n_traces <= REPW_MAX_TRACES)
    TIMED(KN_REPORT, hipLaunchKernelGGL(k_report_wave, dim3(grid_for(b.n_traces, 1, WAVE_GRID_CAP)), dim3(TB), 0, s,
                                        b, rc, w, o, 0));
  else
    TIMED(KN_REPORT, hipLaunchKernelGGL(k_report, dim3(grid_for(b.n_traces, tb, 1 << 30)), dim3(tb), 0, s, b, rc, w,
                                        o, 0));
}
#undef TIMED

void launch_index_build(const DevGraph& g, const uint32_t* turn_units, uint32_t cmax, int32_t* row_cnt,
                        const IdxRow* rows, uint4* slot, bool write, hipStream_t s) {
  const int grid = grid_for((int64_t)g.n_edges + g.n_nodes, 1, 256 * 16);
  if (write)
    hipLaunchKernelGGL(k_index_build<true>, dim3(grid), dim3(TB), 0, s, g, turn_units, cmax, row_cnt, rows, slot);
  else
    hipLaunchKernelGGL(k_index_build<false>, dim3(grid), dim3(TB), 0, s, g, turn_units, cmax, row_cnt, rows, slot);
}
int index_load_fast() { return IDX_LOAD_FAST; }
int index_load_dense() { return IDX_LOAD_DENSE; }
void launch_row_sizes(const int32_t* row_cnt, int64_t* row_sizes, int32_t n, int pct, hipStream_t s) {
  hipLaunchKernelGGL(k_row_sizes, dim3(grid_for((int64_t)n + 1, 256, 1 << 30)), dim3(256), 0, s, row_cnt, row_sizes,
                     n, pct);
}
void launch_row_pack(const int32_t* row_cnt, const int64_t* row_off, IdxRow* rows, int32_t n, hipStream_t s) {
  hipLaunchKernelGGL(k_row_pack, dim3(grid_for((int64_t)n, 256, 1 << 30)), dim3(256), 0, s, row_cnt, row_off, rows, n);
}
void launch_src_pack(const DevGraph& g, const IdxRow* rows, SrcRec* src, hipStream_t s) {
// ... 19 lines not shown
```

### reporter_amd/engine.py

```python
import ctypes as C
import json
import os
import tempfile

import numpy as np

from . import _lib
from ._lib import lib, take


class OtmError(RuntimeError):
    pass


def _check(rc):
    if rc != _lib.OTM_OK:
        raise OtmError("libotmatch error %d: %s" % (rc, _lib.last_error()))


def write_config(path, graph_path, index_radius_m=None, grid_mult=None, trans_lanes=None, index_near_m=None,
                 queue_speed_kph=None, **meili):
    otm = {"graph": os.path.abspath(graph_path)}
    if index_radius_m is not None:
        otm["index_radius_m"] = index_radius_m
# ... 402 lines not shown

    def scores_device(self):
        return self._records_device("otm_scores_device")

    def set_shape(self, on):
        self._set_switch("otm_set_shape", on)

    def shape_info(self):
        return self._switch_info("otm_shape_info")

    def shape(self):
        z = _lib.ShapeSizes()
        _check(lib().otm_shape_size(self.h, C.byref(z)))
        vtx = np.zeros(z.n_vertices, dtype=_lib.SHAPE_VERTEX_DTYPE)
        spans = np.zeros(z.n_traversals, dtype=_lib.SHAPE_SPAN_DTYPE)
        poly = np.zeros(z.n_bytes, dtype=np.uint8)
        offs = [np.zeros(z.n_traces + 1, dtype=np.int64) for _ in range(3)]
        dst = _lib.ShapeOut(vtx.ctypes.data if len(vtx) else None, len(vtx), offs[0].ctypes.data,
                            spans.ctypes.data if len(spans) else None, len(spans), offs[1].ctypes.data,
                            poly.ctypes.data if len(poly) else None, len(poly), offs[2].ctypes.data)
        _check(lib().otm_fetch_shape(self.h, C.byref(dst)))
        return vtx, offs[0], spans, offs[1], poly.tobytes(), offs[2]

    def shape_device(self):
        dev, z = _lib.ShapeOut(), _lib.ShapeSizes()
        _check(lib().otm_shape_device(self.h, C.byref(dev), C.byref(z)))
        return dev, z

    def set_attributes(self, mask):
        mask = _lib.ATTR_ALL if mask is True else int(mask or 0)
        _check(lib().otm_set_attributes(self.h, mask))

    def attributes_info(self):
        m = C.c_uint32()
        _check(lib().otm_attributes_info(self.h, C.byref(m)))
        return m.value

    def attributes(self):
        nt, nb = C.c_int64(), C.c_int64()
        _check(lib().otm_attributes_size(self.h, C.byref(nt), C.byref(nb)))
        blob = np.zeros(nb.value, dtype=np.uint8)
        off = np.zeros(nt.value + 1, dtype=np.int64)
        _check(lib().otm_fetch_attributes(self.h, blob.ctypes.data if nb.value else None, nb.value, off.ctypes.data,
                                          C.byref(nb)))
        return blob.tobytes(), off

    def attributes_device(self):
        dev, off, nt, nb = C.c_void_p(), C.c_void_p(), C.c_int64(), C.c_int64()
        _check(lib().otm_attributes_device(self.h, C.byref(dev), C.byref(off), C.byref(nt), C.byref(nb)))
        return dev.value or 0, off.value or 0, nt.value, nb.value

    def set_counting(self, on):
        _check(lib().otm_set_counting(self.h, 1 if on else 0))

    def counters(self):
        c = _lib.WorkCounters()
        _check(lib().otm_get_counters(self.h, C.byref(c)))
        return {n: getattr(c, n) for n in _lib.COUNTER_NAMES}

    def set_timing(self, on):
        _check(lib().otm_set_timing(self.h, 1 if on else 0))

    STAGES = ("columns", "candidates", "links_scan", "transitions", "viterbi", "route", "segment_bound",
              "segments_report")

    def stage_ms(self):
        ms = (C.c_float * 8)()
        _check(lib().otm_get_stage_ms(self.h, ms, 8))
        return dict(zip(self.STAGES, list(ms)))

    def kernel_ms(self):
        n = 0
        while lib().otm_kernel_name(n):
            n += 1
        ms = (C.c_float * n)()
        _check(lib().otm_get_kernel_ms(self.h, ms, n))
        return {lib().otm_kernel_name(k).decode(): ms[k] for k in range(n)}

    def spill_stats(self):
        st = _lib.SpillStats()
        _check(lib().otm_get_spill_stats(self.h, C.byref(st)))
        return {n: getattr(st, n) for n, _ in _lib.SpillStats._fields_ if n != "pad"}

    _DEBUG = {"ncand": (0, np.int32), "cand_edge": (1, np.int32), "cand_off": (2, np.float32),
              "cand_emis": (3, np.float32), "trans_off": (4, np.int64), "trans": (5, np.float32),
              "state": (6, np.int32), "col_prev": (7, np.int32), "route_dist": (8, np.float32),
              "gc": (9, np.float32), "ipos": (10, np.float32),
              "in_trace_off": (11, np.int64), "in_lat": (12, np.float32), "in_lon": (13, np.float32),
              "in_time": (14, np.float64), "in_acc": (15, np.float32),
              "chain_start": (16, np.uint8), "is_col": (17, np.uint8),
              "order_item": (18, np.int32), "order_tile": (19, np.uint16), "order_grp": (20, np.int32)}

    def debug(self, name):
        what, dt = self._DEBUG[name]
        need = C.c_size_t()
        _check(lib().otm_debug_fetch(self.h, what, None, 0, C.byref(need)))
        out = np.zeros(need.value // np.dtype(dt).itemsize, dtype=dt)
        _check(lib().otm_debug_fetch(self.h, what, out.ctypes.data, out.nbytes, None))
        return out


def report_segments(body, match_output, engine=None):
    b = body.encode("utf-8") if isinstance(body, str) else body
    m = match_output.encode("utf-8") if isinstance(match_output, str) else match_output
    out = C.c_void_p()
    n = C.c_size_t()
    code = lib().otm_report_segments(engine.h if engine is not None else None, b, len(b), m, len(m), C.byref(out),
                                     C.byref(n))
    return code, take(out, n.value).decode("utf-8")


def encode_request(uuid, lat, lon, time, accuracy):
    lat = np.ascontiguousarray(lat, dtype=np.float32)
    lon = np.ascontiguousarray(lon, dtype=np.float32)
    tm = np.ascontiguousarray(time, dtype=np.int64)
    acc = np.ascontiguousarray(accuracy, dtype=np.int32)
    out = C.c_void_p()
    n = C.c_size_t()
    ub = uuid if isinstance(uuid, bytes) else uuid.encode("utf-8")
    _check(lib().otm_encode_request(ub, len(lat), lat.ctypes.data, lon.ctypes.data,
                                    tm.ctypes.data, acc.ctypes.data, C.byref(out), C.byref(n)))
    return take(out, n.value)


def murmur2_partition(key, n):
    b = key.encode("utf-8") if isinstance(key, str) else key
    return (lib().otm_murmur2(b, len(b)) & 0x7fffffff) % n
```

Before: 1.734 billion.

## Skip idle spill-tier kernel launches adaptively and fold memsets into kernels

Adds an adaptive tier mechanism. After a few consecutive batches in which a fallback tier (big candidates, online transitions and routes, viterbi lists, large segments) saw no work, those kernel launches are skipped. If a dormant tier is needed, the device raises a wake bit and aborts, and the batch is retried with that tier re-enabled. It also drops separate memsets and the status D2H copy by zeroing seg_base and ord_cnt inside existing kernels and having k_status write directly to host memory. The aim is to cut per-batch launch and dispatch overhead, at the cost of occasional retried batches and more complex retry logic.

```diff
diff --git a/include/otmatch.h b/include/otmatch.h
--- a/include/otmatch.h
+++ b/include/otmatch.h
@@ -337,6 +337,13 @@
   int32_t resumed;
 } otm_spill_stats;
 int otm_get_spill_stats(otm_engine* eng, otm_spill_stats* out);
+
+#define OTM_TIER_CAND_BIG 1
+#define OTM_TIER_TRANS_ONLINE 2
+#define OTM_TIER_ROUTE_ONLINE 4
+#define OTM_TIER_VIT_LISTS 8
+#define OTM_TIER_SEG_LARGE 16
+int otm_get_tiers(otm_engine* eng, int32_t* dormant_mask, int32_t* dispatches);
 
 int otm_debug_fetch(otm_engine* eng, int what, void* dst, size_t bytes,
                     size_t* needed);
diff --git a/reporter_amd/_lib.py b/reporter_amd/_lib.py
--- a/reporter_amd/_lib.py
+++ b/reporter_amd/_lib.py
@@ -264,6 +264,7 @@
         "otm_get_kernel_ms": (C.c_int, [vp, C.POINTER(C.c_float), C.c_int]),
         "otm_kernel_name": (C.c_char_p, [C.c_int]),
         "otm_get_spill_stats": (C.c_int, [vp, C.POINTER(SpillStats)]),
+        "otm_get_tiers": (C.c_int, [vp, C.POINTER(C.c_int32), C.POINTER(C.c_int32)]),
         "otm_debug_fetch": (C.c_int, [vp, C.c_int, vp, sz, psz]),
         "otm_kmax": (C.c_int, []),
         "otm_debug_py_repr": (C.c_int, [C.c_double, C.c_char_p]),
diff --git a/reporter_amd/csrc/abi.cpp b/reporter_amd/csrc/abi.cpp
--- a/reporter_amd/csrc/abi.cpp
+++ b/reporter_amd/csrc/abi.cpp
@@ -2421,6 +2421,19 @@
   return otm::engine_spill_stats(E, out) ? fail(OTM_EDEVICE, "spill stats copy failed") : OTM_OK;
 }
 
+static_assert(OTM_TIER_CAND_BIG == otm::TIER_CAND_BIG && OTM_TIER_TRANS_ONLINE == otm::TIER_TRANS_ONLINE &&
+                  OTM_TIER_ROUTE_ONLINE == otm::TIER_ROUTE_ONLINE && OTM_TIER_VIT_LISTS == otm::TIER_VIT_LISTS &&
+                  OTM_TIER_SEG_LARGE == otm::TIER_SEG_LARGE,
+              "tier group bits");
+int otm_get_tiers(otm_engine* E, int32_t* dormant_mask, int32_t* dispatches) {
+  if (!E) return fail(OTM_EINVAL, "engine is NULL");
+  if (!E->members.empty()) E = E->members[0];
+  std::lock_guard<std::mutex> lk(E->mu);
+  if (dormant_mask) *dormant_mask = E->tier_dormant;
+  if (dispatches) *dispatches = E->last_dispatches;
+  return OTM_OK;
+}
+
 int otm_debug_fetch(otm_engine* E, int what, void* dst, size_t bytes, size_t* needed) {
   if (!E) return fail(OTM_EINVAL, "engine is NULL");
   if (!E->members.empty()) E = E->members[0];
diff --git a/reporter_amd/csrc/engine.cpp b/reporter_amd/csrc/engine.cpp
--- a/reporter_amd/csrc/engine.cpp
+++ b/reporter_amd/csrc/engine.cpp
@@ -604,10 +604,12 @@
   return OTM_OK;
 }
 
-static int bind_order(otm_engine* E, int64_t NP, bool ordered, DevOrder& ord, std::string* err) {
+static int bind_order(otm_engine* E, int64_t NP, bool ordered, DevOrder& ord, hipStream_t s, std::string* err) {
   const size_t Pn = (size_t)NP + 1;
+  bool fresh;
   TRY(bind_buf(ord.tile, E->ord_tile, Pn, err));
-  TRY(bind_buf(ord.tile_cnt, E->ord_cnt, ORDER_TILES, err));
+  TRY(bind_buf(ord.tile_cnt, E->ord_cnt, ORDER_TILES, err, &fresh));
+  if (fresh) HIPCHK(hipMemsetAsync(E->ord_cnt.p, 0, E->ord_cnt.bytes(), s));
   TRY(bind_buf(ord.cursor, E->ord_cursor, ORDER_TILES, err));
   TRY(bind_buf(ord.grp, E->ord_grp, ORDER_GROUPS + 1, err));
   TRY(bind_buf(ord.item, E->ord_item, Pn, err));
@@ -674,17 +676,24 @@
     dp.cand_chunk = ch < 1 ? 1 : (ch > 64 ? 64 : ch);
   }
   w.ctr = E->counting ? E->ctr.p : nullptr;
-  if (E->counting && from == RESUME_ALL) HIPCHK(hipMemsetAsync(E->ctr.p, 0, sizeof(DevCounters), s));
+  w.dormant = E->tier_dormant;
+  E->last_dispatches = 0;
+  if (E->counting && from == RESUME_ALL) {
+    HIPCHK(hipMemsetAsync(E->ctr.p, 0, sizeof(DevCounters), s));
+    E->last_dispatches += 1;
+  }
   Marks mk;
   mk.ev = E->timing ? E->kev : nullptr;
-  TRY(bind_order(E, NP, dp.order_mask != 0, w.ord, err));
+  mk.dispatches = &E->last_dispatches;
+  TRY(bind_order(E, NP, dp.order_mask != 0, w.ord, s, err));
   if (from == RESUME_ALL) {
-    launch_columns(E->g, b, dp, w, s, mk);
+    int64_t* seg_base = nullptr;
+    TRY(bind_buf(seg_base, E->seg_ub, (size_t)NT + 1, err));
+    launch_columns(E->g, b, dp, w, seg_base, s, mk);
     if (dp.order_mask) {
       launch_order(b, w, s, mk);
-    } else if (E->timing) {
-      mk.begin(KN_ORDER, s);
-      mk.end(KN_ORDER, s);
+    } else {
+      mk.skip(KN_ORDER, s);
     }
   }
   TRY(ensure_cand(E, w, err));
@@ -693,6 +702,7 @@
     launch_links(b, dp, w, s, mk);
     mk.begin(KN_SCAN_TRANS, s);
     scan_i64(w.trans_off, NP, E->scan_tmp.p, E->scan_tmp.cap(), s);
+    mk.count(2);
     mk.end(KN_SCAN_TRANS, s);
   }
   TRY(bind_trans(E, w, s, err));
@@ -717,10 +727,10 @@
     o.bin_kph = H->bin_kph;
     o.pairs = H->pairs_tab;
   }
-  HIPCHK(hipMemsetAsync(o.seg_base, 0, ((size_t)NT + 1) * sizeof *o.seg_base, s));
   launch_seg_bound(E->g, b, dp, w, o.seg_base, s, mk);
   mk.begin(KN_SEG_SCAN, s);
   scan_i64(o.seg_base, NT, E->scan_tmp.p, E->scan_tmp.cap(), s);
+  mk.count(2);
   mk.end(KN_SEG_SCAN, s);
   launch_segments(E->g, b, w, o, s, mk);
   if (E->queue_kph > 0.0f) launch_queue(b, w, o, E->queue_kph, s);
@@ -760,8 +770,28 @@
   return OTM_OK;
 }
 
+static void tiers_learn(otm_engine* E, int32_t idle) {
+  if (E->tiers_always) return;
+  for (int g = 0; g < TIER_GROUPS; ++g) {
+    const int32_t bit = 1 << g;
+    if (E->tier_woken & bit) continue;
+    E->tier_quiet[g] = (idle & bit) ? E->tier_quiet[g] + 1 : 0;
+    if (E->tier_quiet[g] >= TIER_QUIET) E->tier_dormant |= bit;
+  }
+}
+static void tiers_wake(otm_engine* E, int32_t groups) {
+  if (groups & TIER_TRANS_ONLINE) groups |= TIER_ROUTE_ONLINE;
+  E->tier_woken |= groups;
+  E->tier_dormant &= ~groups;
+}
+
 int engine_match(otm_engine* E, const DevBatch& b, hipStream_t s, std::string* err) {
   if (!s) s = E->stream;
+  if (!E->tiers_read) {
+    E->tiers_read = true;
+    const char* v = std::getenv("OTM_TIERS_ALWAYS");
+    E->tiers_always = v && *v && *v != '0';
+  }
   const int64_t NP = b.n_points;
   struct OomGuard {
     otm_engine* E;
@@ -785,20 +815,28 @@
     TRY(engine_match_once(E, b, s, err, from));
     TRY(E->h_status.ensure(1, err));
     BatchStatus* dst = &E->snap.p->status;
-    launch_status(E->abort_flag.p, E->trans_off.p + NP, E->counters_i32.p, dst, s);
-    HIPCHK(hipMemcpyAsync(E->h_status.p, dst, sizeof(BatchStatus), hipMemcpyDeviceToHost, s));
+    launch_status(E->abort_flag.p, E->trans_off.p + NP, E->counters_i32.p, &E->snap.p->stage[0][0], dst,
+                  E->h_status.p, s);
+    E->last_dispatches += 1;
     HIPCHK(wait_batch(E, s, NP));
-    const BatchStatus st = *E->h_status.p;
+    BatchStatus st = *E->h_status.p;
     const int32_t ab = st.abort;
     const int64_t ttotal = st.ttotal;
     E->last_trans = ttotal;
     E->last_attempts = attempt + 1;
-    if (!ab) break;
+    if (!ab) {
+      tiers_learn(E, st.tier_idle);
+      break;
+    }
     if (attempt == 16) {
       *err = "batch capacities could not be sized";
       return OTM_EDEVICE;
     }
     if (ttotal > E->trans_cap) E->trans_cap = ttotal + ttotal / 4 + 4096;
+    const int32_t woke = st.tier_wake & TIER_ALL;
+    if (woke) tiers_wake(E, woke);
+    const bool woke_cand_only = woke == TIER_CAND_BIG && !st.pool_over;
+    if (woke_cand_only && E->cand_log2 == 0 && !E->cand_final) st.grow |= GROW_CAND;
     if (st.grow & GROW_HUGE) {
       const int32_t next = E->huge_log2 ? E->huge_log2 + 2 : 19;
       const int32_t prev = E->huge_log2;
@@ -833,10 +871,12 @@
     if (st.pool_over)
       E->pool_cap = (int32_t)std::min<size_t>((size_t)st.pool_used * 2 + 1024, (size_t)INT32_MAX / 2);
     const char* nr = std::getenv("OTM_NO_RESUME");
-    const bool whole = ttotal > E->trans_cap || st.pool_over || !(st.grow & (GROW_HUGE | GROW_CAND)) ||
+    const bool whole = st.pool_over ||
+                       !((st.grow & (GROW_HUGE | GROW_CAND)) || woke_cand_only) || (woke && !woke_cand_only) ||
                        (nr && *nr && *nr != '0');
     from = whole ? RESUME_ALL
-                 : (st.grow & GROW_CAND) ? RESUME_CAND_BIG : (st.route_huge ? RESUME_ROUTE_HUGE : RESUME_TRANS_HUGE);
+                 : ((st.grow & GROW_CAND) || woke_cand_only) ? RESUME_CAND_BIG
+                 : (st.route_huge ? RESUME_ROUTE_HUGE : RESUME_TRANS_HUGE);
     if (from != RESUME_ALL) {
       const SnapId snap = from == RESUME_CAND_BIG ? SNAP_AFTER_CAND
                                                   : (from == RESUME_TRANS_HUGE ? SNAP_AFTER_TRANS : SNAP_AFTER_ROUTE);
@@ -845,6 +885,7 @@
                             hipMemcpyDeviceToDevice, s));
       HIPCHK(hipMemsetAsync(ctr + CTR_GROW_HUGE, 0, 4, s));
       HIPCHK(hipMemsetAsync(ctr + CTR_GROW_CAND, 0, 4, s));
+      HIPCHK(hipMemsetAsync(ctr + CTR_TIER_WAKE, 0, 4, s));
       HIPCHK(hipMemsetAsync(E->abort_flag.p, 0, 4, s));
       E->last_resumes += 1;
     }
diff --git a/reporter_amd/csrc/engine.h b/reporter_amd/csrc/engine.h
--- a/reporter_amd/csrc/engine.h
+++ b/reporter_amd/csrc/engine.h
@@ -157,6 +157,10 @@
   int32_t huge_final = 0, cand_final = 0;
   int32_t last_attempts = 0;
   int32_t last_resumes = 0;
+  int32_t tier_dormant = 0, tier_woken = 0;
+  int32_t tier_quiet[otm::TIER_GROUPS] = {};
+  bool tiers_read = false, tiers_always = false;
+  int32_t last_dispatches = 0;
   otm::DevBuf<uint16_t> ord_tile;
   otm::DevBuf<int32_t> ord_cnt, ord_cursor, ord_grp, ord_item;
   otm::DevBuf<otm_trace_result> o_traces;
diff --git a/reporter_amd/csrc/kernels.h b/reporter_amd/csrc/kernels.h
--- a/reporter_amd/csrc/kernels.h
+++ b/reporter_amd/csrc/kernels.h
@@ -163,10 +163,21 @@
   CTR_CAND_BIG = 24,
   CTR_GROW_CAND = 25,
   CTR_VIT_WAVE = 26,
+  CTR_TIER_WAKE = 27,
 };
 constexpr int CTR_STAGE_WORDS = 16;
 constexpr int CTR_ZEROED_WORDS = 32;
 constexpr int CTR_WORDS = 64;
+enum TierGroup : int {
+  TIER_CAND_BIG = 1,
+  TIER_TRANS_ONLINE = 2,
+  TIER_ROUTE_ONLINE = 4,
+  TIER_VIT_LISTS = 8,
+  TIER_SEG_LARGE = 16,
+  TIER_ALL = 31,
+};
+constexpr int TIER_GROUPS = 5;
+constexpr int TIER_QUIET = 2;
 enum SnapId : int { SNAP_AFTER_CAND = 0, SNAP_AFTER_TRANS = 1, SNAP_AFTER_ROUTE = 2, SNAP_COUNT = 3 };
 constexpr int ctr_list(CtrSlot c) {
   switch (c) {
@@ -184,7 +195,7 @@
               "per-stage slots lie in the snapshot range");
 static_assert(ctr_per_batch(CTR_VIT_16) && ctr_per_batch(CTR_TRANS_HUGE) && ctr_per_batch(CTR_ROUTE_HUGE) &&
                   ctr_per_batch(CTR_GROW_HUGE) && ctr_per_batch(CTR_CAND_BIG) && ctr_per_batch(CTR_GROW_CAND) &&
-                  ctr_per_batch(CTR_VIT_WAVE),
+                  ctr_per_batch(CTR_VIT_WAVE) && ctr_per_batch(CTR_TIER_WAKE),
               "per-batch slots lie past the snapshot range, within what K1 zeroes");
 
 struct DevWork {
@@ -214,6 +225,7 @@
   int32_t* path_len;
   int32_t* path_pool;
   int32_t pool_cap;
+  int32_t dormant;
   int32_t* trace_err;
   int32_t* spill_list1;
   int32_t* spill_list2;
@@ -318,6 +330,14 @@
 extern const char* const kKernelNames[KN_COUNT];
 struct Marks {
   hipEvent_t* ev = nullptr;
+  int32_t* dispatches = nullptr;
+  void count(int n = 1) const {
+    if (dispatches) *dispatches += n;
+  }
+  void skip(int k, hipStream_t s) const {
+    begin(k, s);
+    end(k, s);
+  }
   void begin(int k, hipStream_t s) const {
     if (ev) (void)hipEventRecord(ev[2 * k], s);
   }
@@ -326,8 +346,8 @@
   }
 };
 
-void launch_columns(const DevGraph& g, const DevBatch& b, const DevParams& p, DevWork& w, hipStream_t s,
-                    const Marks& mk);
+void launch_columns(const DevGraph& g, const DevBatch& b, const DevParams& p, DevWork& w, int64_t* seg_base,
+                    hipStream_t s, const Marks& mk);
 enum Resume { RESUME_ALL = 0, RESUME_CAND_BIG = 1, RESUME_TRANS_HUGE = 2, RESUME_ROUTE_HUGE = 3 };
 void launch_candidates(const DevGraph& g, const DevBatch& b, const DevParams& p, DevWork& w, hipStream_t s,
                        const Marks& mk, int from = RESUME_ALL);
@@ -373,16 +393,19 @@
   int64_t ttotal;
   int32_t pool_used, pool_over;
   int32_t route_huge;
+  int32_t tier_idle;
+  int32_t tier_wake;
+  int32_t pad;
 };
 struct SnapBuf {
   int32_t stage[SNAP_COUNT][CTR_STAGE_WORDS];
   BatchStatus status;
 };
-static_assert(offsetof(SnapBuf, status) == 192 && sizeof(SnapBuf) == 192 + 32, "snapshot buffer layout");
+static_assert(offsetof(SnapBuf, status) == 192 && sizeof(SnapBuf) == 192 + 40, "snapshot buffer layout");
 void launch_expand_compact(const int64_t* trace_off, const int64_t* tbase, const int32_t* dt, const int16_t* acc16,
                            double* time, float* acc, int32_t n_traces, hipStream_t s);
-void launch_status(const int32_t* abort, const int64_t* ttotal, const int32_t* counters, BatchStatus* out,
-                   hipStream_t s);
+void launch_status(const int32_t* abort, const int64_t* ttotal, const int32_t* counters, const int32_t* snap,
+                   BatchStatus* out, BatchStatus* host, hipStream_t s);
 void launch_row_pack(const int32_t* row_cnt, const int64_t* row_off, IdxRow* rows, int32_t n, hipStream_t s);
 void launch_src_pack(const DevGraph& g, const IdxRow* rows, SrcRec* src, hipStream_t s);
 size_t req_sparse_slots(int32_t n, size_t bytes);
diff --git a/reporter_amd/csrc/kernels.hip b/reporter_amd/csrc/kernels.hip
--- a/reporter_amd/csrc/kernels.hip
+++ b/reporter_amd/csrc/kernels.hip
@@ -232,9 +232,17 @@
     if (reset) w.counters_i32[t] = 0;
   }
 }
-template <CtrSlot C>
+template <int G>
+__device__ __forceinline__ void tier_wake(const DevWork& w) {
+  if (G != 0 && (w.dormant & G)) {
+    atomicOr(&w.counters_i32[CTR_TIER_WAKE], G);
+    *w.abort = 1;
+  }
+}
+template <CtrSlot C, int G = 0>
 __device__ __forceinline__ void spill_push(const DevWork& w, int32_t p) {
   const SpillRef s = spill_of<C>(w);
+  tier_wake<G>(w);
   s.list[atomicAdd(s.count, 1)] = p;
 }
 __device__ __forceinline__ bool trans_over_cap(const DevBatch& b, const DevWork& w) {
@@ -303,7 +311,7 @@
   if (active && m.leader == (int)(threadIdx.x & 63)) atomicAdd(&ctr[key], m.count);
 }
 
-__global__ __launch_bounds__(1024) void k_order_plan(const int32_t* tile_cnt, int32_t* cursor, int32_t* grp) {
+__global__ __launch_bounds__(1024) void k_order_plan(int32_t* tile_cnt, int32_t* cursor, int32_t* grp) {
   __shared__ int32_t part[1024];
   __shared__ int32_t cut[ORDER_GROUPS + 1];
   constexpr int PER = ORDER_TILES / 1024;
@@ -335,6 +343,7 @@
     run += v[k];
   }
   __syncthreads();
+  for (int k = 0; k < PER; ++k) tile_cnt[tid * PER + k] = 0;
   if (tid == 0) {
     grp[0] = 0;
     int32_t prev = 0;
@@ -363,7 +372,7 @@
 #define OTM_COL_PTS 256
 #endif
 constexpr int COL_PTS = OTM_COL_PTS;
-__global__ __launch_bounds__(TB) void k_columns(DevGraph g, DevBatch b, DevParams P, DevWork w) {
+__global__ __launch_bounds__(TB) void k_columns(DevGraph g, DevBatch b, DevParams P, DevWork w, int64_t* seg_base) {
   __shared__ float sLat[COL_PTS], sLon[COL_PTS], sGc[COL_PTS];
   __shared__ int32_t sPrev[COL_PTS];
   __shared__ uint8_t sCol[COL_PTS];
@@ -371,6 +380,7 @@
   if (blockIdx.x == 0) {
     if (lane < CTR_ZEROED_WORDS) w.counters_i32[lane] = 0;
     if (lane == 0) *w.abort = 0;
+    if (lane == 0) seg_base[b.n_traces] = 0;
   }
   for (int32_t t = blockIdx.x; t < b.n_traces; t += gridDim.x) {
     const int64_t a = b.trace_off[t], e = b.trace_off[t + 1];
@@ -466,6 +476,7 @@
     }
     if (lane == 0) {
       w.trace_err[t] = 0;
+      seg_base[t] = 0;
       if (w.ctr) {
         cadd(&w.ctr->points, (unsigned long long)n);
         cadd(&w.ctr->columns, (unsigned long long)ncols);
@@ -905,7 +916,7 @@
     if (s_over) {
       if (lane == 0) {
         if (!BIG) {
-          spill_push<CTR_CAND_BIG>(w, (int32_t)p);
+          spill_push<CTR_CAND_BIG, TIER_CAND_BIG>(w, (int32_t)p);
         } else if (w.cand_final) {
           w.ncand[p] = 0;
           atomicCAS(&w.trace_err[w.pt_trace[p]], 0, OTM_TERR_CAND_OVERFLOW);
@@ -1040,14 +1051,25 @@
   w.vmeta[p] = (uint8_t)((w.is_col[p] ? (w.ncand[p] | 0x40) : 0) | (cp >= 0 ? 0x80 : 0));
 }
 
-__global__ void k_status(const int32_t* abort, const int64_t* ttotal, const int32_t* counters, BatchStatus* out) {
+__global__ void k_status(const int32_t* abort, const int64_t* ttotal, const int32_t* counters, const int32_t* snap,
+                         BatchStatus* out, BatchStatus* host) {
   if (threadIdx.x == 0) {
-    out->abort = *abort;
-    out->grow = (counters[CTR_GROW_HUGE] != 0 ? GROW_HUGE : 0) | (counters[CTR_GROW_CAND] != 0 ? GROW_CAND : 0);
-    out->ttotal = *ttotal;
-    out->pool_used = counters[CTR_POOL_USED];
-    out->pool_over = counters[CTR_POOL_OVER];
-    out->route_huge = counters[CTR_ROUTE_HUGE];
+    BatchStatus st;
+    st.abort = *abort;
+    st.grow = (counters[CTR_GROW_HUGE] != 0 ? GROW_HUGE : 0) | (counters[CTR_GROW_CAND] != 0 ? GROW_CAND : 0);
+    st.ttotal = *ttotal;
+    st.pool_used = counters[CTR_POOL_USED];
+    st.pool_over = counters[CTR_POOL_OVER];
+    st.route_huge = counters[CTR_ROUTE_HUGE];
+    st.tier_idle = (counters[CTR_CAND_BIG] == 0 ? TIER_CAND_BIG : 0) |
+                   (snap[CTR_STAGE_WORDS * SNAP_AFTER_TRANS + CTR_INDEX_MISS] == 0 ? TIER_TRANS_ONLINE : 0) |
+                   (snap[CTR_STAGE_WORDS * SNAP_AFTER_ROUTE + CTR_INDEX_MISS] == 0 ? TIER_ROUTE_ONLINE : 0) |
+                   (counters[CTR_VIT_WAVE] == 0 && counters[CTR_VIT_16] == 0 ? TIER_VIT_LISTS : 0) |
+                   (counters[CTR_SEG_LARGE] == 0 ? TIER_SEG_LARGE : 0);
+    st.tier_wake = counters[CTR_TIER_WAKE];
+    st.pad = 0;
+    *out = st;
+    *host = st;
   }
 }
 
@@ -1523,7 +1545,7 @@
       }
     }
     const bool spill = (__ballot(bad) & smask) != 0ull;
-    if (spill && act && sl == 0) spill_push<CTR_INDEX_MISS>(w, (int32_t)p);
+    if (spill && act && sl == 0) spill_push<CTR_INDEX_MISS, TIER_TRANS_ONLINE>(w, (int32_t)p);
     act = act && !spill;
     const int npair_g = act ? Kq * Kp : 0;
     if (sl == 0) {
@@ -1679,7 +1701,7 @@
       sv = idx_find(Xc.slot, Rw, dst_key(g, ej, oj), lab);
     }
     if (sv < 0 || idx_slot_cost(lab) > cq) {
-      spill_push<CTR_INDEX_MISS>(w, (int32_t)p);
+      spill_push<CTR_INDEX_MISS, TIER_ROUTE_ONLINE>(w, (int32_t)p);
       continue;
     }
     int len = 0;
@@ -2316,7 +2338,10 @@
       take = ((__ballot(wide) >> gb) & gmask) == 0ull;
     }
     if (act && !take) {
-      if (j == 0) rej[atomicAdd(rej_n, 1)] = t;
+      if (j == 0) {
+        tier_wake<TIER_VIT_LISTS>(w);
+        rej[atomicAdd(rej_n, 1)] = t;
+      }
       act = false;
     }
     if (!act) n = 0;
@@ -2620,7 +2645,10 @@
       take = ((__ballot(wide) >> gb) & 0xFFFFull) == 0ull;
     }
     if (act && !take) {
-      if (j == 0) rej[atomicAdd(rej_n, 1)] = t;
+      if (j == 0) {
+        tier_wake<TIER_VIT_LISTS>(w);
+        rej[atomicAdd(rej_n, 1)] = t;
+      }
       act = false;
     }
     if (!act) n = 0;
@@ -3336,8 +3364,11 @@
     }
     if (n > PT) {
       if (lane == 0) {
-        if (spill) spill[atomicAdd(spill_n, 1)] = t;
-        else segments_trace<true>(g, w, o, t, n, base, SegSrcGlobal{&g, &b, &w, a});
+        if (spill) {
+          tier_wake<TIER_SEG_LARGE>(w);
+          spill[atomicAdd(spill_n, 1)] = t;
+        } else
+          segments_trace<true>(g, w, o, t, n, base, SegSrcGlobal{&g, &b, &w, a});
       }
       continue;
     }
@@ -3400,8 +3431,11 @@
     SEGP_MARK(2)
     if (nt > TR) {
       if (lane == 0) {
-        if (spill) spill[atomicAdd(spill_n, 1)] = t;
-        else segments_trace<true>(g, w, o, t, n, base, SegSrcGlobal{&g, &b, &w, a});
+        if (spill) {
+          tier_wake<TIER_SEG_LARGE>(w);
+          spill[atomicAdd(spill_n, 1)] = t;
+        } else
+          segments_trace<true>(g, w, o, t, n, base, SegSrcGlobal{&g, &b, &w, a});
       }
       wave_sync();
       continue;
@@ -4835,14 +4869,14 @@
   do {                   \
     mk.begin(k, s);      \
     launch;              \
+    mk.count();          \
     mk.end(k, s);        \
   } while (0)
 
-void launch_columns(const DevGraph& g, const DevBatch& b, const DevParams& p, DevWork& w, hipStream_t s,
-                    const Marks& mk) {
-  if (w.ord.tile_cnt) (void)hipMemsetAsync(w.ord.tile_cnt, 0, ORDER_TILES * 4, s);
+void launch_columns(const DevGraph& g, const DevBatch& b, const DevParams& p, DevWork& w, int64_t* seg_base,
+                    hipStream_t s, const Marks& mk) {
   TIMED(KN_COLUMNS, hipLaunchKernelGGL(k_columns, dim3(grid_for(b.n_traces, 1, WAVE_GRID_CAP)), dim3(TB), 0, s, g,
-                                       b, p, w));
+                                       b, p, w, seg_base));
 }
 static int order_grid(int64_t n, int per_block, int cap) {
   const int64_t per_group = (n + ORDER_GROUPS - 1) / ORDER_GROUPS;
@@ -4858,6 +4892,7 @@
   hipLaunchKernelGGL(k_order_plan, dim3(1), dim3(1024), 0, s, w.ord.tile_cnt, w.ord.cursor, w.ord.grp);
   hipLaunchKernelGGL(k_order_scatter, dim3(grid_for(b.n_points, 256, 8192)), dim3(256), 0, s, b, w, w.ord.tile,
                      w.ord.cursor, w.ord.item);
+  mk.count(2);
   mk.end(KN_ORDER, s);
 }
 
@@ -4875,9 +4910,14 @@
 #ifndef OTM_CAND_WAVE_GRID
 #define OTM_CAND_WAVE_GRID 4096
 #endif
-  if (from < RESUME_CAND_BIG)
+  if (from < RESUME_CAND_BIG) {
     hipLaunchKernelGGL(k_candidates<false>, dim3(OTM_CAND_WAVE_GRID), dim3(TB), 0, s, g, b, p, w);
-  hipLaunchKernelGGL(k_candidates<true>, dim3(CAND_BIG_SLOTS), dim3(TB), 0, s, g, b, p, w);
+    mk.count();
+  }
+  if (!(w.dormant & TIER_CAND_BIG)) {
+    hipLaunchKernelGGL(k_candidates<true>, dim3(CAND_BIG_SLOTS), dim3(TB), 0, s, g, b, p, w);
+    mk.count();
+  }
   mk.end(KN_CAND_WAVE, s);
 }
 void launch_links(const DevBatch& b, const DevParams& p, DevWork& w, hipStream_t s, const Marks& mk) {
@@ -4902,15 +4942,16 @@
   hipLaunchKernelGGL(k_expand_compact, dim3(grid_for(((int64_t)n_traces + 3) / 4, 1, 1 << 20)), dim3(256), 0, s,
                      trace_off, tbase, dt, acc16, time, acc, n_traces);
 }
-void launch_status(const int32_t* abort, const int64_t* ttotal, const int32_t* counters, BatchStatus* out,
-                   hipStream_t s) {
-  hipLaunchKernelGGL(k_status, dim3(1), dim3(64), 0, s, abort, ttotal, counters, out);
+void launch_status(const int32_t* abort, const int64_t* ttotal, const int32_t* counters, const int32_t* snap,
+                   BatchStatus* out, BatchStatus* host, hipStream_t s) {
+  hipLaunchKernelGGL(k_status, dim3(1), dim3(64), 0, s, abort, ttotal, counters, snap, out, host);
 }
 void launch_transitions(const DevGraph& g, const DevBatch& b, const DevParams& p, DevWork& w, hipStream_t s,
                         const Marks& mk, int sub, int from) {
   if (from >= RESUME_TRANS_HUGE) {
     mk.begin(KN_TRANS_GLOBAL, s);
     hipLaunchKernelGGL(k_transitions<2>, dim3(HUGE_SLOTS), dim3(TB), 0, s, g, b, p, w);
+    mk.count();
     mk.end(KN_TRANS_GLOBAL, s);
     return;
   }
@@ -4921,13 +4962,18 @@
     TIMED(KN_TRANS_WIDE, hipLaunchKernelGGL((k_trans_sub<16, true>), dim3(WIDE_GRID), dim3(TB), 0, s, g, b, p, w));
   } else {
     TIMED(KN_TRANS_INDEX, hipLaunchKernelGGL((k_trans_sub<16, false>), dim3(grid), dim3(TB), 0, s, g, b, p, w));
-    mk.begin(KN_TRANS_WIDE, s);
-    mk.end(KN_TRANS_WIDE, s);
+    mk.skip(KN_TRANS_WIDE, s);
+  }
+  if (w.dormant & TIER_TRANS_ONLINE) {
+    mk.skip(KN_TRANS_WAVE, s);
+    mk.skip(KN_TRANS_GLOBAL, s);
+    return;
   }
   TIMED(KN_TRANS_WAVE, hipLaunchKernelGGL(k_transitions<0>, dim3(SPILL_GRID), dim3(TB), 0, s, g, b, p, w));
   mk.begin(KN_TRANS_GLOBAL, s);
   hipLaunchKernelGGL(k_transitions<1>, dim3(BIG_SLOTS), dim3(TB), 0, s, g, b, p, w);
   hipLaunchKernelGGL(k_transitions<2>, dim3(HUGE_SLOTS), dim3(TB), 0, s, g, b, p, w);
+  mk.count(2);
   mk.end(KN_TRANS_GLOBAL, s);
 }
 void launch_viterbi(const DevBatch& b, DevWork& w, hipStream_t s, const Marks& mk) {
@@ -4937,6 +4983,7 @@
   constexpr int rmin = 4096;
   const int form = forced ? forced : (b.n_traces >= gmin ? 8 : (b.n_traces >= rmin ? 4 : 64));
   const SpillRef to_16 = spill_of<CTR_VIT_16>(w), to_wave = spill_of<CTR_VIT_WAVE>(w);
+  const bool lists = !(w.dormant & TIER_VIT_LISTS);
   if (form == 4) {
     const char* we = std::getenv("OTM_VR_WIN");
     const int vt = OTM_VR_U * 16;
@@ -4947,8 +4994,12 @@
     mk.begin(KN_VITERBI, s);
     hipLaunchKernelGGL(k_viterbi_row, dim3(grid_for(b.n_traces, TB / 16, WAVE_GRID_CAP)), dim3(TB), 0, s, b, w,
                        to_wave.list, to_wave.count, win, fast, 1);
-    hipLaunchKernelGGL(k_viterbi, dim3(grid_for(b.n_traces, 1, WAVE_GRID_CAP)), dim3(TB), 0, s, b, w,
-                       (const int32_t*)to_wave.list, (const int32_t*)to_wave.count, 0);
+    mk.count();
+    if (lists) {
+      hipLaunchKernelGGL(k_viterbi, dim3(grid_for(b.n_traces, 1, WAVE_GRID_CAP)), dim3(TB), 0, s, b, w,
+                         (const int32_t*)to_wave.list, (const int32_t*)to_wave.count, 0);
+      mk.count();
+    }
     mk.end(KN_VITERBI, s);
     return;
   }
@@ -4965,14 +5016,22 @@
   if (form == 16) {
     hipLaunchKernelGGL(k_viterbi_g<16>, dim3(grid_for(b.n_traces, TB / 16, WAVE_GRID_CAP)), dim3(TB), 0, s, b, w,
                        (const int32_t*)nullptr, (const int32_t*)nullptr, l16, n16, 1);
+    mk.count();
   } else {
     hipLaunchKernelGGL(k_viterbi_g<8>, dim3(grid_for(b.n_traces, TB / 8, WAVE_GRID_CAP)), dim3(TB), 0, s, b, w,
                        (const int32_t*)nullptr, (const int32_t*)nullptr, l8, n8, 1);
-    hipLaunchKernelGGL(k_viterbi_g<16>, dim3(grid_for(b.n_traces, TB / 16, WAVE_GRID_CAP)), dim3(TB), 0, s, b, w,
-                       (const int32_t*)l8, (const int32_t*)n8, l16, n16, 0);
-  }
-  hipLaunchKernelGGL(k_viterbi, dim3(grid_for(b.n_traces / 64 + 1, 1, 1024)), dim3(TB), 0, s, b, w,
-                     (const int32_t*)l16, (const int32_t*)n16, 0);
+    mk.count();
+    if (lists) {
+      hipLaunchKernelGGL(k_viterbi_g<16>, dim3(grid_for(b.n_traces, TB / 16, WAVE_GRID_CAP)), dim3(TB), 0, s, b, w,
+                         (const int32_t*)l8, (const int32_t*)n8, l16, n16, 0);
+      mk.count();
+    }
+  }
+  if (lists) {
+    hipLaunchKernelGGL(k_viterbi, dim3(grid_for(b.n_traces / 64 + 1, 1, 1024)), dim3(TB), 0, s, b, w,
+                       (const int32_t*)l16, (const int32_t*)n16, 0);
+    mk.count();
+  }
   mk.end(KN_VITERBI, s);
 }
 void launch_route(const DevGraph& g, const DevBatch& b, const DevParams& p, DevWork& w, hipStream_t s,
@@ -4980,15 +5039,22 @@
   if (from >= RESUME_ROUTE_HUGE) {
     mk.begin(KN_ROUTE_GLOBAL, s);
     hipLaunchKernelGGL(k_route<2>, dim3(HUGE_SLOTS), dim3(TB), 0, s, g, b, p, w);
+    mk.count();
     mk.end(KN_ROUTE_GLOBAL, s);
     return;
   }
   TIMED(KN_ROUTE_INDEX, hipLaunchKernelGGL(k_route_index, dim3(order_grid(b.n_points, 256, 1 << 30)), dim3(256), 0,
                                            s, g, b, p, w));
+  if (w.dormant & TIER_ROUTE_ONLINE) {
+    mk.skip(KN_ROUTE_WAVE, s);
+    mk.skip(KN_ROUTE_GLOBAL, s);
+    return;
+  }
   TIMED(KN_ROUTE_WAVE, hipLaunchKernelGGL(k_route<0>, dim3(SPILL_GRID), dim3(TB), 0, s, g, b, p, w));
   mk.begin(KN_ROUTE_GLOBAL, s);
   hipLaunchKernelGGL(k_route<1>, dim3(BIG_SLOTS), dim3(TB), 0, s, g, b, p, w);
   hipLaunchKernelGGL(k_route<2>, dim3(HUGE_SLOTS), dim3(TB), 0, s, g, b, p, w);
+  mk.count(2);
   mk.end(KN_ROUTE_GLOBAL, s);
 }
 void launch_segments(const DevGraph& g, const DevBatch& b, DevWork& w, DevOut& o, hipStream_t s, const Marks& mk) {
@@ -4999,8 +5065,12 @@
   mk.begin(KN_SEG_WRITE, s);
   hipLaunchKernelGGL((k_segments<SEGP_PTS_S, SEGP_TRAV_S>), grid, dim3(TB), 0, s, g, b, w, o, (const int32_t*)nullptr,
                      (const int32_t*)nullptr, lst, cnt);
-  hipLaunchKernelGGL((k_segments<SEGP_PTS, SEGP_TRAV>), dim3(grid_for(b.n_traces, 1, 2048)), dim3(TB), 0, s, g, b, w,
-                     o, (const int32_t*)lst, (const int32_t*)cnt, (int32_t*)nullptr, (int32_t*)nullptr);
+  mk.count();
+  if (!(w.dormant & TIER_SEG_LARGE)) {
+    hipLaunchKernelGGL((k_segments<SEGP_PTS, SEGP_TRAV>), dim3(grid_for(b.n_traces, 1, 2048)), dim3(TB), 0, s, g, b,
+                       w, o, (const int32_t*)lst, (const int32_t*)cnt, (int32_t*)nullptr, (int32_t*)nullptr);
+    mk.count();
+  }
   mk.end(KN_SEG_WRITE, s);
 }
 void launch_queue(const DevBatch& b, DevWork& w, DevOut& o, float kph, hipStream_t s) {
diff --git a/reporter_amd/engine.py b/reporter_amd/engine.py
--- a/reporter_amd/engine.py
+++ b/reporter_amd/engine.py
@@ -508,6 +508,14 @@
         _check(lib().otm_get_spill_stats(self.h, C.byref(st)))
         return {n: getattr(st, n) for n, _ in _lib.SpillStats._fields_ if n != "pad"}
 
+    TIERS = {"cand_big": 1, "trans_online": 2, "route_online": 4, "vit_lists": 8, "seg_large": 16}
+
+    def tiers(self):
+        mask, disp = C.c_int32(), C.c_int32()
+        _check(lib().otm_get_tiers(self.h, C.byref(mask), C.byref(disp)))
+        return {"dormant": {n for n, b in self.TIERS.items() if mask.value & b}, "mask": mask.value,
+                "dispatches": disp.value}
+
     _DEBUG = {"ncand": (0, np.int32), "cand_edge": (1, np.int32), "cand_off": (2, np.float32),
               "cand_emis": (3, np.float32), "trans_off": (4, np.int64), "trans": (5, np.float32),
               "state": (6, np.int32), "col_prev": (7, np.int32), "route_dist": (8, np.float32),
```

Result: faster. 1.787 billion, median of 6 (+3.1%).
